# tj12323/GeoPurify

Hardware: AMD Instinct MI355X
Metric: scenes/sec (ScanNet-val shape) + pooled-feature GB/s vs HBM peak (higher is better)
Workload: dtype f32 (student convolutions and pooling: f16 hi/lo split operands, 3 MFMAs per product, fp32 accumulate)

## Files before the change

geopurify_amd/_lib.py:

```python
import ctypes
import os
from ctypes import POINTER, c_char_p, c_double, c_float, c_int32, c_int64, c_size_t, c_uint32, c_void_p

_HERE = os.path.dirname(os.path.abspath(__file__))
LIB_PATH = os.environ.get("GP_LIB") or os.path.join(_HERE, "libgeopurify_hip.so")

_P = c_void_p
GP_KNN_MAX_K = 127

SIGNATURES = {
    "gp_version": (c_int32, []),
    "gp_last_error": (c_char_p, []),
    "gp_debug_set": (c_int32, [c_int32, c_int32]),
    "gp_debug_ptr": (c_int32, [c_int32, _P, c_size_t]),
    "gp_voxelize_workspace_bytes": (c_size_t, [c_int64]),
    "gp_voxelize_f64": (c_int32, [_P, c_int64, POINTER(c_double), _P, _P, _P, _P, _P, _P, _P, c_size_t, _P]),
    "gp_fnv_hash_f64": (c_int32, [_P, c_int64, _P, _P]),
    "gp_project_points_f64": (c_int32, [_P, c_int64, POINTER(c_double), c_double, c_double, c_double,
                                        c_double, _P, c_int32, c_int32, c_int32, c_double, _P, _P, _P]),
    "gp_render_depth_f64": (c_int32, [_P, c_int64, POINTER(c_double), c_double, c_double, c_double, c_double,
                                      c_int32, c_int32, c_int32, _P, _P]),
    "gp_minmax_i32": (c_int32, [_P, c_int64, _P, _P]),
    "gp_morton_order_workspace_bytes": (c_size_t, [c_int64]),
    "gp_morton_order": (c_int32, [_P, c_int64, _P, _P, _P, c_size_t, _P]),
    "gp_grid_bytes": (c_size_t, [c_int64, POINTER(c_int32)]),
    "gp_grid_build": (c_int32, [_P, c_int64, POINTER(c_int32), POINTER(c_int32), _P, c_size_t, _P]),
    "gp_scatter_mean_csr": (c_int32, [_P, c_int64, c_int32, _P, _P, c_int64, _P, _P, c_int64, c_int32, _P]),
    "gp_gather_rows": (c_int32, [_P, c_int64, c_int32, _P, c_int64, _P, _P, c_int64, _P]),
    "gp_kernel_map_build": (c_int32, [_P, _P, c_int64, _P, _P]),
    "gp_coords_order_batched_workspace_bytes": (c_size_t, [c_int64]),
    "gp_coords_order_batched": (c_int32, [_P, c_int64, _P, _P, _P, _P, _P, c_size_t, _P]),
    "gp_kernel_map_sorted": (c_int32, [_P, c_int64, _P, _P]),
    "gp_quantize_batched_workspace_bytes": (c_size_t, [c_int64]),
    "gp_quantize_batched": (c_int32, [_P, c_int64, _P, _P, _P, _P, _P, _P, _P, c_size_t, _P]),
    "gp_segment_labels": (c_int32, [_P, c_int64, _P, _P, _P, c_int64, c_int64, c_int32, _P, _P]),
    "gp_sparse_conv": (c_int32, [_P, c_int64, _P, c_int64, _P, c_int32, c_int32, c_int32, _P, _P, _P,
                                 c_int64, c_int32, _P, c_int64, _P]),
    "gp_conv_pairs_workspace_bytes": (c_size_t, [c_int64, c_int32]),
    "gp_conv_pairs_build": (c_int32, [_P, c_int64, c_int32, c_int32, _P, _P, _P, _P, _P, _P, _P, c_size_t, _P]),
    "gp_conv_chunk_plan_workspace_bytes": (c_size_t, [c_int64, c_int32]),
    "gp_conv_chunk_plan": (c_int32, [_P, c_int64, c_int32, c_int32, c_int32, c_int32, c_int32, _P, _P, _P, c_size_t, _P]),
    "gp_conv_weights_split": (c_int32, [_P, c_int32, c_int32, c_int32, c_float, _P, _P, _P]),
    "gp_split_f16": (c_int32, [_P, c_int64, c_int32, c_int64, _P, _P, c_int64, _P]),
    "gp_sparse_conv_f16x3": (c_int32, [_P, c_int64, _P, _P, c_int64, _P, _P, _P, _P, _P, c_int32, c_int64, c_int64, c_int32, _P, _P,
                                       c_int32, c_int32, _P, _P, _P, _P, c_int64, c_int32, _P, c_int64, _P, _P,
                                       c_int64, c_int32, POINTER(c_int32), POINTER(c_int32), POINTER(c_int32), _P, _P,
                                       _P, _P, c_int64, _P, c_int32, c_int32, _P]),
    "gp_conv_weights_split_blocked": (c_int32, [_P, c_int32, c_int32, c_int32, c_float, _P, _P, c_int32, _P]),
    "gp_pow2_scale": (c_int32, [_P, c_int64, c_int32, c_int64, _P, _P, c_size_t, _P]),
    "gp_split_f16_scaled": (c_int32, [_P, c_int64, c_int32, c_int64, _P, _P, c_int64, _P, _P, _P, _P]),
    "gp_rcb_order": (c_int32, [_P, c_int64, c_int32, c_int32, _P, _P, _P]),
    "gp_rows_renumber_i32": (c_int32, [_P, c_int64, c_int32, _P, _P, _P, _P]),
    "gp_l2norm_rows": (c_int32, [_P, c_int64, c_int32, c_int64, _P]),
    "gp_embed_head_f16x3": (c_int32, [_P, _P, c_int64, _P, _P, _P, c_int64, c_int32, c_int32, c_float, c_int32, _P, c_int64, _P, _P, c_float, _P, _P]),
    "gp_knn_workspace_bytes": (c_size_t, [c_int64]),
    "gp_knn_lattice": (c_int32, [_P, _P, _P, c_int64, c_int32, _P, _P, c_size_t, _P]),
    "gp_knn_batched_workspace_bytes": (c_size_t, [c_int64]),
    "gp_knn_batched": (c_int32, [_P, _P, c_int64, c_int32, _P, _P, _P, c_size_t, _P]),
    "gp_affinity_softmax": (c_int32, [_P, c_int64, c_int32, _P, c_int32, c_int64, c_float, _P, _P]),
    "gp_affinity_softmax_scatter": (c_int32, [_P, c_int64, c_int32, _P, c_int32, c_int64, c_float, _P, _P, _P, _P, _P]),
    "gp_pool_ell": (c_int32, [_P, c_int64, _P, _P, c_int32, c_int64, c_int32, _P, c_int64, _P]),
    "gp_pool_transpose_workspace_bytes": (c_size_t, [c_int64, c_int32]),
    "gp_pool_transpose_build": (c_int32, [_P, c_int64, c_int32, _P, _P, _P, c_size_t, _P]),
    "gp_pool_ell_transpose": (c_int32, [_P, c_int64, _P, _P, _P, c_int32, c_int64, c_int32, _P, c_int64, _P]),
    "gp_pool_ell_wgrad": (c_int32, [_P, c_int64, _P, c_int64, _P, c_int32, c_int64, c_int32, _P, c_int32, _P]),
    "gp_affinity_softmax_backward_workspace_bytes": (c_size_t, [c_int64, c_int32]),
    "gp_affinity_softmax_backward": (c_int32, [_P, c_int64, c_int32, _P, _P, _P, c_int32, c_int64, c_float, _P, _P, _P, c_int64, _P,
                                               c_size_t, _P]),
    "gp_l2norm_rows_backward": (c_int32, [_P, c_int64, _P, c_int64, c_int32, c_int64, _P, c_int64, _P]),
    "gp_pool_tiles_workspace_bytes": (c_size_t, [c_int64, c_int32]),
    "gp_pool_tiles_count": (c_int32, [_P, c_int64, c_int32, c_int32, _P, _P, c_size_t, _P]),
    "gp_pool_tiles_fill": (c_int32, [_P, _P, c_int64, c_int32, c_int32, _P, _P, _P, _P]),
    "gp_pool_tiles_apply": (c_int32, [_P, c_int64, _P, _P, _P, c_int32, c_int64, c_int32, _P, c_int64, _P]),
    "gp_pool_mfma_workspace_bytes": (c_size_t, [c_int64, c_int32]),
    "gp_pool_mfma_count": (c_int32, [_P, c_int64, c_int32, c_int32, c_int32, _P, _P, _P, c_size_t, _P]),
    "gp_pool_mfma_fill": (c_int32, [_P, _P, c_int64, c_int32, c_int32, _P, _P, c_int64, _P, _P, _P, _P]),
    "gp_pool_mfma_apply": (c_int32, [_P, _P, c_int64, _P, _P, _P, _P, c_int64, c_int32, c_int32, _P, _P, c_int64, _P, c_int64, _P, _P]),
    "gp_pool_mfma_apply_persistent": (c_int32, [_P, _P, c_int64, _P, _P, _P, _P, c_int64, c_int32, c_int32, c_int32, _P, _P, c_int64,
                                                _P, c_int64, c_int64, _P, _P, _P]),
    "gp_pool_cs_workspace_bytes": (c_size_t, [c_int64, c_int32]),
    "gp_pool_cs_count": (c_int32, [_P, c_int64, c_int32, c_int32, _P, _P, _P, _P, c_size_t, _P]),
    "gp_pool_cs_fill": (c_int32, [_P, _P, c_int64, c_int32, c_int32, _P, c_int64, c_int32, _P, _P, _P, _P, _P]),
    "gp_pool_cs_structure": (c_int32, [_P, c_int64, c_int32, c_int32, _P, c_int64, c_int32, _P, _P, _P, _P, _P, _P]),
    "gp_pool_cs_structure_valid": (c_int32, [_P, c_int64, c_int32, c_int32, _P, c_int64, c_int32, _P, _P, _P, _P]),
    "gp_affinity_cs_fragments": (c_int32, [_P, _P, c_int64, c_int32, c_int32, c_float, _P, _P, _P, _P, c_int32, _P, _P, _P]),
    "gp_pool_cs_apply": (c_int32, [_P, _P, c_int64, _P, _P, _P, _P, _P, c_int64, c_int32, c_int32, _P, _P, c_int64, _P, c_int64, _P, _P]),
    "gp_pool_cs_deps": (c_int32, [_P, _P, c_int64, c_int32, _P, _P, _P]),
    "gp_pool_cs_chain_flag_words": (c_size_t, [c_int64, c_int32]),
    "gp_pool_cs_chain_flag_words_d": (c_size_t, [c_int64, c_int32, c_int32]),
    "gp_pool_cs_apply_chain": (c_int32, [_P, _P, _P, _P, c_int64, _P, _P, _P, _P, _P, c_int64, c_int32, c_int32, c_int32, _P, c_int64, _P, _P, _P,
                                         c_uint32, _P]),
    "gp_lift_dense_accum": (c_int32, [_P, c_int32, c_int32, c_int32, _P, _P, _P, c_int64, _P, c_int64, _P, _P]),
    "gp_lift_dense_bilinear_accum": (c_int32, [_P, c_int32, c_int32, c_int32, c_int32, c_int32, _P, _P, _P, c_int64, _P,
                                               c_int64, _P, _P]),
    "gp_lift_dense_finish": (c_int32, [_P, c_int64, c_int32, _P, c_int64, _P, _P]),
    "gp_lift_masks_workspace_bytes": (c_size_t, [c_int32, c_int32, c_int32]),
    "gp_lift_masks_view": (c_int32, [_P, c_int32, c_int32, c_int32, _P, _P, _P, _P, _P, c_int32, c_int32,
                                     _P, _P, c_int64, _P, _P, _P, c_size_t, _P]),
    "gp_pv_count": (c_int32, [_P, c_int64, _P, _P]),
    "gp_scan_workspace_bytes": (c_size_t, [c_int64]),
    "gp_exclusive_scan_i64": (c_int32, [_P, c_int64, _P, _P, c_size_t, _P]),
    "gp_pv_fill": (c_int32, [_P, _P, c_int64, c_int32, _P, _P, _P, _P, _P]),
    "gp_segment_tables": (c_int32, [_P, c_int32, c_int32, _P, c_int32, c_float, _P, _P, _P]),
    "gp_fuse_views_top3": (c_int32, [_P, _P, _P, c_int64, _P, _P, c_int32, c_int32, c_int32, _P, c_int64, _P, _P]),
    "gp_nn1_workspace_bytes": (c_size_t, [c_int64, c_int64]),
    "gp_nn1_f64": (c_int32, [_P, c_int64, _P, c_int64, _P, _P, c_size_t, _P]),
    "gp_nn1_masked_workspace_bytes": (c_size_t, [c_int64]),
    "gp_nn1_masked_f64": (c_int32, [_P, c_int64, _P, _P, _P, _P, c_size_t, _P]),
    "gp_visible_lists_workspace_bytes": (c_size_t, [c_int64]),
    "gp_visible_lists": (c_int32, [_P, c_int64, _P, _P, _P, _P, _P, c_size_t, _P]),
    "gp_views_visible_lists_workspace_bytes": (c_size_t, [c_int64, c_int32]),
    "gp_views_visible_lists": (c_int32, [_P, c_int64, _P, _P, c_int32, c_int32, c_int32, c_int32, c_double, c_int64, c_int64,
                                         _P, _P, _P, _P, _P, _P, _P, c_size_t, _P]),
    "gp_lift_masks_views_workspace_bytes": (c_size_t, [c_int32, c_int32, c_int32, c_int32, c_int64, c_int64, c_int64]),
    "gp_lift_masks_views": (c_int32, [_P, c_int32, c_int32, c_int32, c_int32, _P, _P, _P, _P, _P, c_int32, c_int32, _P, c_int64,
                                      _P, _P, _P, _P, _P, _P, c_int32, c_int64, c_int64, _P, _P, _P, _P, _P, c_size_t, _P]),
    "gp_classify_argmax": (c_int32, [_P, c_int64, c_int32, c_int64, _P, c_int32, c_float, _P, _P, _P]),
    "gp_gather_rows_classify": (c_int32, [_P, c_int64, c_int32, _P, c_int64, _P, _P, c_int64, _P, c_int32, c_float, _P, _P, _P]),
    "gp_rows_argmax": (c_int32, [_P, c_int64, c_int32, c_int64, _P, c_int64, c_int32, _P, _P, _P]),
    "gp_col_stats_workspace_bytes": (c_size_t, [c_int64, c_int32]),
    "gp_col_stats": (c_int32, [_P, c_int64, c_int64, c_int32, _P, _P, _P, c_size_t, _P]),
    "gp_bn_train_apply": (c_int32, [_P, c_int64, c_int64, c_int32, _P, _P, _P, _P, c_float, _P, c_int64, c_int32, _P, c_int64,
                                    _P, _P, c_int64, c_float, _P, _P, _P]),
    "gp_bn_train_backward_workspace_bytes": (c_size_t, [c_int64, c_int32]),
    "gp_bn_train_backward": (c_int32, [_P, c_int64, _P, c_int64, _P, c_int64, _P, _P, c_float, _P, _P, c_int64, c_int32, _P, c_int64,
                                       _P, c_int64, _P, _P, _P, _P, _P, c_int64, _P, c_size_t, _P]),
    "gp_col_sums_f64": (c_int32, [_P, c_int64, c_int64, c_int32, _P, _P, _P, c_size_t, _P]),
    "gp_bn_bwd_sums_f64": (c_int32, [_P, c_int64, _P, c_int64, _P, c_int64, _P, _P, c_float, _P, _P, c_int64, c_int32, _P, _P, c_size_t, _P]),
    "gp_bn_bwd_apply": (c_int32, [_P, c_int64, _P, c_int64, _P, c_int64, _P, _P, c_float, _P, _P, _P, c_int64, c_int64, c_int32, _P, c_int64,
                                  _P, c_int64, _P, _P]),
    "gp_infonce_workspace_bytes": (c_size_t, [c_int64, c_int32]),
    "gp_infonce_fwd_bwd": (c_int32, [_P, c_int64, c_int64, c_int32, _P, c_int64, _P, c_int64, c_int32, c_float, _P, _P, c_int64,
                                     _P, c_size_t, _P]),
    "gp_infonce_weighted_fwd_bwd": (c_int32, [_P, c_int64, c_int64, c_int32, _P, c_int64, _P, c_int64, c_int32, c_float, _P, _P, _P, _P, c_int64,
                                              _P, c_size_t, _P]),
    "gp_conv_wgrad_workspace_bytes": (c_size_t, [c_int64, c_int32, c_int32]),
    "gp_conv_wgrad_f16x3": (c_int32, [_P, _P, c_int64, _P, _P, c_int64, _P, _P, _P, c_int64, _P, c_int32, c_int32, c_int32, c_int32,
                                      _P, _P, _P, c_size_t, _P]),
    "gp_adamw_step": (c_int32, [_P, _P, _P, _P, c_int64, c_float, c_float, c_float, c_float, c_float, c_int64, _P]),
    "gp_knn_points_f32": (c_int32, [_P, c_int64, _P, c_int64, c_int32, _P, _P, _P]),
    "gp_sampler_select": (c_int32, [_P, c_int64, c_int64, c_int64, _P, c_int32, _P, _P, _P]),
    "gp_sim_segments_f16x3": (c_int32, [_P, _P, c_int64, c_int32, _P, _P, _P, _P, c_int64, c_int64, _P, _P]),
    "gp_sampler_select_segments": (c_int32, [_P, _P, _P, _P, c_int64, c_int64, _P, c_int32, _P, _P, _P]),
    "gp_sampler_micro_segments": (c_int32, [_P, _P, _P, _P, _P, c_int64, c_int32, _P, c_int64, c_int32, _P, _P]),
    "gp_normalize_split_f16": (c_int32, [_P, c_int64, c_int32, c_int64, c_int64, c_float, _P, _P, c_int64, _P]),
    "gp_iou_hist_i64": (c_int32, [_P, _P, c_int64, c_int32, POINTER(c_int64), c_int32, _P, _P]),
    "gp_nn1_batched_workspace_bytes": (c_size_t, [c_int64]),
    "gp_nn1_batched": (c_int32, [_P, _P, _P, _P, c_int64, c_int32, _P, _P, _P, c_size_t, _P]),
    "gp_iou_hist_batched_i64": (c_int32, [_P, _P, c_int64, _P, _P, c_int64, c_int32, c_int32, POINTER(c_int64), c_int32, _P, _P]),
    "gp_sparse_conv_tiles": (c_int32, [POINTER(c_int32)]),
    "gp_segment_loss_col_step": (c_int32, []),
    "gp_segment_loss_unit_rows": (c_int32, [_P, c_int64, c_int32, c_int64, _P, c_int64, c_int32, _P, _P]),
    "gp_segment_loss_items_workspace_bytes": (c_size_t, [c_int64, c_int64]),
    "gp_segment_loss_items": (c_int32, [_P, _P, c_int64, _P, _P, c_int64, c_int32, POINTER(c_int64), c_int32, c_int32, _P, _P, _P, _P, _P, _P,
                                        _P, c_size_t, _P]),
    "gp_segment_loss_rows": (c_int32, [_P, c_int64, c_int64, c_int32, c_int32, _P, _P, _P, _P, _P, _P, _P, c_int64, _P, _P, _P]),
    "gp_segment_loss_reduce_workspace_bytes": (c_size_t, [c_int64, c_int32]),
    "gp_segment_loss_reduce": (c_int32, [_P, _P, c_int64, _P, c_int32, c_int32, _P, _P, _P, c_size_t, _P]),
    "gp_fused_decode_workspace_bytes": (c_size_t, [c_int64, c_int64]),
    "gp_fused_decode": (c_int32, [_P, c_int64, _P, _P, c_int64, c_int64, _P, c_int64, c_int32, _P, _P, _P, _P, c_size_t, _P]),
    "gp_lift_batched_col_chunk": (c_int32, []),
    "gp_lift_batched_transpose": (c_int32, [_P, c_int32, c_int32, c_int64, _P, _P]),
    "gp_lift_batched_workspace_bytes": (c_size_t, [c_int64, c_int32]),
    "gp_lift_batched": (c_int32, [_P, c_int64, _P, c_int32, c_int32, c_int32, _P, _P, _P, _P, c_int32, c_int32, c_int32, c_int32, c_int32,
                                  c_double, c_int64, c_int64, c_int32, _P, c_int64, _P, _P, _P, _P, _P, _P, _P, c_size_t, _P]),
    "gp_lift_masks_batched_lists_workspace_bytes": (c_size_t, [c_int64, c_int32]),
    "gp_lift_masks_batched_lists": (c_int32, [_P, c_int64, _P, _P, _P, _P, c_int32, c_int32, c_int32, c_int32, c_double, c_int64, c_int64,
                                              c_int64, _P, _P, _P, _P, _P, _P, _P, _P, _P, c_size_t, _P]),
    "gp_lift_masks_batched_workspace_bytes": (c_size_t, [c_int64, c_int32, c_int32, c_int32, c_int32, c_int32, c_int32, c_int64, c_int32,
                                                         c_int64]),
    "gp_lift_masks_batched": (c_int32, [_P, c_int64, _P, c_int32, _P, c_int32, c_int32, c_int32, _P, _P, _P, _P, _P, c_int32, c_int32,
                                        _P, _P, _P, _P, _P, _P, c_int64, c_int32, c_int64, _P, _P, c_int32, c_int32, c_int32,
                                        _P, c_int64, _P, _P, _P, _P, _P, _P, c_size_t, _P]),
}

_lib = None


class GeoPurifyHipError(RuntimeError):
    pass


def load(path=None):
    global _lib
    if _lib is not None:
        return _lib
    import torch
    p = path or LIB_PATH
    if not os.path.exists(p):
        raise GeoPurifyHipError(
            f"{p} not found: build it with `python -c 'import __graft_entry__ as g; g.build()'` "
            "(or `make -C geopurify_amd/csrc`).  There is no CPU fallback.")
    lib = ctypes.CDLL(p)
    missing = []
    for name, (res, args) in SIGNATURES.items():
        try:
            fn = getattr(lib, name)
        except AttributeError:
            missing.append(name)
            continue
        fn.restype = res
        fn.argtypes = args
    if missing:
        raise GeoPurifyHipError(f"{p} does not export {missing}; rebuild the library")
    _lib = lib
    return lib


def check(rc, what):
    if rc != 0:
        msg = load().gp_last_error()
        raise GeoPurifyHipError(f"{what} failed (rc={rc}): {msg.decode() if msg else ''}")


def exported_symbols():
    return list(SIGNATURES.keys())
```

geopurify_amd/csrc/knn.hip:

```cpp
#include "gp_grid.h"

namespace {

constexpr int KNN_MAXSEL = 128;
constexpr int KNN_MAXTIE = 256;

template <int R>
struct KnnCfg {
    static constexpr int B = (8 * R + 1) * (8 * R + 1);
    static constexpr int HB = (B + 63) / 64 * 64;
};

template <int R, int WAVES>
__global__ void __launch_bounds__(WAVES * 64)
knn_ring_kernel(const void *grid, const int32_t *__restrict__ coords, const int32_t *__restrict__ ids, int64_t nv,
                int k, int32_t *__restrict__ nbr, const int32_t *__restrict__ qlist,
                const int32_t *__restrict__ qcount, int32_t *__restrict__ fail_list, int32_t *__restrict__ fail_count) {
    constexpr int B = KnnCfg<R>::B, HB = KnnCfg<R>::HB;
    __shared__ int s_hist[WAVES][HB];
    __shared__ unsigned long long s_selkey[WAVES][KNN_MAXSEL];
    __shared__ int s_selrow[WAVES][KNN_MAXSEL];
    __shared__ int s_tieid[WAVES][KNN_MAXTIE];
    __shared__ int s_tierow[WAVES][KNN_MAXTIE];
    __shared__ int s_cnt[WAVES][2];
    __shared__ int s_cstart[WAVES][(2 * R + 1) * (2 * R + 1) * (2 * R + 1)], s_coff[WAVES][(2 * R + 1) * (2 * R + 1) * (2 * R + 1) + 1];

    const int wv = threadIdx.x >> 6, lane = threadIdx.x & 63;
    int64_t widx = (int64_t)blockIdx.x * WAVES + wv;
    int64_t total = qlist ? (int64_t)*qcount : nv;
    if (widx >= total) return;
    const int qi = __builtin_amdgcn_readfirstlane(qlist ? qlist[widx] : (int)widx);
    GpGridView g(grid);
    const int qx = coords[(int64_t)qi * 3], qy = coords[(int64_t)qi * 3 + 1], qz = coords[(int64_t)qi * 3 + 2];
    const int cx0 = (qx - g.h->origin[0]) >> 3, cy0 = (qy - g.h->origin[1]) >> 3, cz0 = (qz - g.h->origin[2]) >> 3;
    int *hist = s_hist[wv];
    for (int b = lane; b < HB; b += 64) hist[b] = 0;
    if (lane < 2) s_cnt[wv][lane] = 0;
    constexpr int SIDE = 2 * R + 1, NC = SIDE * SIDE * SIDE;
    int *cstart = s_cstart[wv], *coff = s_coff[wv];
    int total_c = 0;
    for (int c0 = 0; c0 < NC; c0 += 64) {
        const int c = c0 + lane;
        int start = 0, cnt = 0;
        if (c < NC) {
            const int dx = c % SIDE - R, dy = (c / SIDE) % SIDE - R, dz = c / (SIDE * SIDE) - R;
            const int slot = g.cell_slot(cx0 + dx, cy0 + dy, cz0 + dz);
            if (slot >= 0) { start = g.recs[slot].start; cnt = g.recs[slot].count; }
        }
        int incl = cnt;
#pragma unroll
        for (int o = 1; o < 64; o <<= 1) {
            int t = __shfl_up(incl, o, 64);
            if (lane >= o) incl += t;
        }
        if (c < NC) { cstart[c] = start; coff[c] = total_c + incl - cnt; }
        total_c += __shfl(incl, 63, 64);
    }
    if (lane == 0) coff[NC] = total_c;
    gp_wave_sync();
    auto row_of = [&](int j) {
        int lo = 0, hi = NC - 1;
        while (lo < hi) {
            const int mid = (lo + hi + 1) >> 1;
            if (coff[mid] <= j) lo = mid; else hi = mid - 1;
        }
        return cstart[lo] + (j - coff[lo]);
    };

    for (int j0 = 0; j0 < total_c; j0 += 128) {
        const int ja = j0 + lane, jb = j0 + 64 + lane;
        const bool va = ja < total_c, vb = jb < total_c;
        const int64_t ra = va ? row_of(ja) : 0, rb = vb ? row_of(jb) : 0;
        const int ax = coords[ra * 3], ay = coords[ra * 3 + 1], az = coords[ra * 3 + 2];
        const int bx = coords[rb * 3], by = coords[rb * 3 + 1], bz = coords[rb * 3 + 2];
        const int da = (ax - qx) * (ax - qx) + (ay - qy) * (ay - qy) + (az - qz) * (az - qz);
        const int db = (bx - qx) * (bx - qx) + (by - qy) * (by - qy) + (bz - qz) * (bz - qz);
        if (va && da < B) atomicAdd(&hist[da], 1);
        if (vb && db < B) atomicAdd(&hist[db], 1);
    }
    gp_wave_sync();

    constexpr int CH = HB / 64;
    int loc = 0;
#pragma unroll
    for (int c = 0; c < CH; ++c) loc += hist[lane * CH + c];
    int incl = loc;
#pragma unroll
    for (int o = 1; o < 64; o <<= 1) {
        int t = __shfl_up(incl, o, 64);
        if (lane >= o) incl += t;
    }
    int tot = __shfl(incl, 63, 64);
    const int need = k + 1;
    bool fail = tot < need;
    int T = 0, c_lt = 0;
    if (!fail) {
        int excl = incl - loc;
        unsigned long long m = __ballot(incl >= need);
        int owner = __ffsll((long long)m) - 1;
        int myT = 0, mylt = 0;
        if (lane == owner) {
            int run = excl;
            for (int c = 0; c < CH; ++c) {
                int h = hist[lane * CH + c];
                if (run + h >= need) { myT = lane * CH + c; mylt = run; break; }
                run += h;
            }
        }
        T = __shfl(myT, owner, 64);
        c_lt = __shfl(mylt, owner, 64);
        if (hist[T] > KNN_MAXTIE) fail = true;
    }
    if (fail) {
        if (lane == 0) {
            int p = atomicAdd(fail_count, 1);
            fail_list[p] = qi;
        }
        return;
    }

    for (int j0 = 0; j0 < total_c; j0 += 64) {
        const int j = j0 + lane;
        if (j < total_c) {
            const int64_t r = row_of(j);
            int ex = coords[r * 3] - qx, ey = coords[r * 3 + 1] - qy, ez = coords[r * 3 + 2] - qz;
            int d2 = ex * ex + ey * ey + ez * ez;
            if (d2 < T) {
                int id = ids ? ids[r] : (int)r;
                int p = atomicAdd(&s_cnt[wv][0], 1);
                s_selkey[wv][p] = ((unsigned long long)(unsigned)d2 << 32) | (unsigned)id;
                s_selrow[wv][p] = (int)r;
            } else if (d2 == T) {
                int id = ids ? ids[r] : (int)r;
                int p = atomicAdd(&s_cnt[wv][1], 1);
                s_tieid[wv][p] = id;
                s_tierow[wv][p] = (int)r;
            }
        }
    }
    gp_wave_sync();
    const int m_tie = s_cnt[wv][1];
    const int take = need - c_lt;
    for (int t = lane; t < m_tie; t += 64) {
        int id = s_tieid[wv][t];
        int rank = 0;
        for (int u = 0; u < m_tie; ++u) rank += (s_tieid[wv][u] < id);
        if (rank < take) {
            s_selkey[wv][c_lt + rank] = ((unsigned long long)(unsigned)T << 32) | (unsigned)id;
            s_selrow[wv][c_lt + rank] = s_tierow[wv][t];
        }
    }
    gp_wave_sync();

    for (int t = lane; t < need; t += 64) {
        unsigned long long key = s_selkey[wv][t];
        int rank = 0;
        for (int u = 0; u < need; ++u) rank += (s_selkey[wv][u] < key);
        if (rank > 0) nbr[(int64_t)qi * k + rank - 1] = s_selrow[wv][t];
    }
}

__global__ void __launch_bounds__(256)
knn_exhaustive_kernel(const int32_t *__restrict__ coords, const int32_t *__restrict__ ids, int64_t nv, int k,
                      int32_t *__restrict__ nbr, const int32_t *__restrict__ qlist, const int32_t *__restrict__ qcount) {
    __shared__ int s_red[4];
    __shared__ unsigned long long s_selkey[KNN_MAXSEL];
    __shared__ int s_selrow[KNN_MAXSEL];
    __shared__ int s_n;
    const int total = *qcount;
    for (int w = blockIdx.x; w < total; w += gridDim.x) {
        const int qi = qlist[w];
        const int qx = coords[(int64_t)qi * 3], qy = coords[(int64_t)qi * 3 + 1], qz = coords[(int64_t)qi * 3 + 2];
        const int need = k + 1;
        auto keyof = [&](int64_t r) {
            long long ex = coords[r * 3] - qx, ey = coords[r * 3 + 1] - qy, ez = coords[r * 3 + 2] - qz;
            unsigned long long d2 = (unsigned long long)(ex * ex + ey * ey + ez * ez);
            unsigned id = (unsigned)(ids ? ids[r] : (int)r);
            return (d2 << 32) | id;
        };
        unsigned long long lo = 0, hi = ~0ull;
        while (lo < hi) {
            unsigned long long mid = lo + ((hi - lo) >> 1);
            int c = 0;
            for (int64_t r = threadIdx.x; r < nv; r += 256) c += (keyof(r) <= mid);
            c = gp_wave_sum_i(c);
            __syncthreads();
            if ((threadIdx.x & 63) == 0) s_red[threadIdx.x >> 6] = c;
            __syncthreads();
            int tot = s_red[0] + s_red[1] + s_red[2] + s_red[3];
            if (tot >= need) hi = mid; else lo = mid + 1;
        }
        if (threadIdx.x == 0) s_n = 0;
        __syncthreads();
        for (int64_t r = threadIdx.x; r < nv; r += 256) {
            unsigned long long key = keyof(r);
            if (key <= lo) {
                int p = atomicAdd(&s_n, 1);
                if (p < KNN_MAXSEL) { s_selkey[p] = key; s_selrow[p] = (int)r; }
            }
        }
        __syncthreads();
        for (int t = threadIdx.x; t < need; t += 256) {
            unsigned long long key = s_selkey[t];
            int rank = 0;
            for (int u = 0; u < need; ++u) rank += (s_selkey[u] < key);
            if (rank > 0) nbr[(int64_t)qi * k + rank - 1] = s_selrow[t];
        }
        __syncthreads();
    }
}

__global__ void zero2_kernel(int32_t *a, int32_t *b) {
    if (threadIdx.x == 0) { *a = 0; *b = 0; }
}

}

extern "C" size_t gp_knn_workspace_bytes(int64_t nv) {
    GpCarver cv(nullptr, 0);
    cv.take<int32_t>(64);
    cv.take<int32_t>(nv);
    cv.take<int32_t>(nv);
    return cv.off;
}

extern "C" int gp_knn_lattice(const void *grid, const int32_t *coords, const int32_t *ids, int64_t nv, int32_t k,
                              int32_t *nbr, void *workspace, size_t workspace_bytes, void *stream_) {
    GP_CHECK_ARG(grid && coords && nbr && workspace, "gp_knn_lattice: null argument");
    GP_CHECK_ARG(k >= 1 && k <= GP_KNN_MAX_K, "gp_knn_lattice: k=%d not in 1..%d", k, GP_KNN_MAX_K);
    GP_CHECK_ARG(nv > k, "gp_knn_lattice: need more than k voxels (nv=%lld, k=%d)", (long long)nv, k);
    GpCarver cv(workspace, workspace_bytes);
    int32_t *counts = cv.take<int32_t>(64);
    int32_t *list_a = cv.take<int32_t>(nv);
    int32_t *list_b = cv.take<int32_t>(nv);
    if (!cv.ok()) { gp_set_error("gp_knn_lattice: workspace too small (%zu < %zu)", workspace_bytes, cv.off); return GP_ENOMEM; }
    hipStream_t s = gp_stream(stream_);
    zero2_kernel<<<1, 64, 0, s>>>(counts, counts + 1);
    constexpr int W1 = 4, W3 = 2;
    knn_ring_kernel<1, W1><<<(int)((nv + W1 - 1) / W1), W1 * 64, 0, s>>>(grid, coords, ids, nv, k, nbr, nullptr, nullptr,
                                                                      list_a, counts);
    knn_ring_kernel<3, W3><<<(int)((nv + W3 - 1) / W3), W3 * 64, 0, s>>>(grid, coords, ids, nv, k, nbr, list_a, counts,
                                                                      list_b, counts + 1);
    knn_exhaustive_kernel<<<1024, 256, 0, s>>>(coords, ids, nv, k, nbr, list_b, counts + 1);
    GP_CHECK_LAUNCH();
    return GP_OK;
}
```

geopurify_amd/csrc/lift.hip:

```cpp
#include <cstring>
#include <rocprim/device/device_scan.hpp>

#include "gp_common.h"
#include "gp_project.h"

namespace {

__global__ void lift_dense_accum_kernel(const float *__restrict__ feat2d, int d, int H, int W,
                                        const int64_t *__restrict__ pt, const int64_t *__restrict__ x,
                                        const int64_t *__restrict__ y, int64_t n_v, float *__restrict__ sum,
                                        int64_t ld_sum, float *__restrict__ cnt) {
    int64_t i = (blockIdx.x * (int64_t)blockDim.x + threadIdx.x) >> 6;
    if (i >= n_v) return;
    int lane = gp_lane();
    int64_t p = pt[i];
    int64_t pix = x[i] * W + y[i];
    int64_t plane = (int64_t)H * W;
    for (int c = lane; c < d; c += 64) sum[p * ld_sum + c] += feat2d[c * plane + pix];
    if (lane == 0) cnt[p] += 1.0f;
}

__global__ void lift_dense_bilinear_accum_kernel(const float *__restrict__ feat, int d, int h, int w, float scale_h,
                                                 float scale_w, const int64_t *__restrict__ pt,
                                                 const int64_t *__restrict__ x, const int64_t *__restrict__ y, int64_t n_v,
// ... 25 lines not shown
    if (c == 0.f) c = 1e-6f;
    for (int k = lane; k < d; k += 64) sum[p * ld_sum + k] = sum[p * ld_sum + k] / c;
    if (lane == 0) seen[p] = c > 1e-5f ? 1 : 0;
}

__global__ void transpose_kernel(const float *__restrict__ src, int rows, int cols, float *__restrict__ dst) {
    __shared__ float tile[64][65];
    int bx = blockIdx.x * 64, by = blockIdx.y * 64;
    int tx = threadIdx.x & 63, ty = threadIdx.x >> 6;
    for (int r = ty; r < 64; r += 4) {
        int row = by + r, col = bx + tx;
        tile[r][tx] = (row < rows && col < cols) ? src[(int64_t)row * cols + col] : 0.f;
    }
    __syncthreads();
    for (int r = ty; r < 64; r += 4) {
        int orow = bx + r, ocol = by + tx;
        if (orow < cols && ocol < rows) dst[(int64_t)orow * rows + ocol] = tile[tx][r];
    }
}

__device__ __forceinline__ void lift_masks_point(const float *__restrict__ mt , int Q, int h, int w,
                                                 const float *__restrict__ scores, const int32_t *__restrict__ tx0,
                                                 const float *__restrict__ twx, const int32_t *__restrict__ ty0,
                                                 const float *__restrict__ twy, int out_h, int out_w, int row, int col, int lane,
                                                 int &seg_out, float &logit_out) {
    bool inb = (unsigned)row < (unsigned)out_h && (unsigned)col < (unsigned)out_w;
    float best = -1.f, best_logit = 0.f;
    int best_q = -1;
    if (inb) {
        int x0 = tx0[col], y0 = ty0[row];
        float wx[4], wy[4];
#pragma unroll
        for (int t = 0; t < 4; ++t) { wx[t] = twx[col * 4 + t]; wy[t] = twy[row * 4 + t]; }
        for (int q = lane; q < Q; q += 64) {
            float sc = scores[q];
            float hr[4];
#pragma unroll
            for (int j = 0; j < 4; ++j) {
                int yy = min(y0 + j, h - 1);
                const float *r = mt + ((int64_t)yy * w) * Q + q;
                float t = __fmul_rn(r[(int64_t)min(x0, w - 1) * Q], wx[0]);
#pragma unroll
                for (int a = 1; a < 4; ++a) t = fmaf(r[(int64_t)min(x0 + a, w - 1) * Q], wx[a], t);
                hr[j] = t;
            }
            float v = __fmul_rn(hr[0], wy[0]);
#pragma unroll
            for (int j = 1; j < 4; ++j) v = fmaf(hr[j], wy[j], v);
            if (sc > 0.f) {
                float sg = 1.f / (1.f + expf(-v));
                float pr = __fmul_rn(sc, sg);
                if (pr > best) { best = pr; best_q = q; best_logit = v; }
            }
        }
    }
#pragma unroll
    for (int o = 32; o > 0; o >>= 1) {
        float ob = __shfl_xor(best, o, 64);
        int oq = __shfl_xor(best_q, o, 64);
        float ol = __shfl_xor(best_logit, o, 64);
        bool take = (oq >= 0) && (best_q < 0 || ob > best || (ob == best && oq < best_q));
        if (take) { best = ob; best_q = oq; best_logit = ol; }
    }
    float sg = 1.f / (1.f + expf(-best_logit));
    seg_out = (best_q >= 0 && sg >= 0.5f) ? best_q : -1;
    logit_out = best_logit;
}
__global__ void lift_masks_kernel(const float *__restrict__ mt , int Q, int h, int w,
                                  const float *__restrict__ scores, const int32_t *__restrict__ tx0,
                                  const float *__restrict__ twx, const int32_t *__restrict__ ty0,
                                  const float *__restrict__ twy, int out_h, int out_w,
                                  const int64_t *__restrict__ px, const int64_t *__restrict__ py, int64_t n_v,
                                  int32_t *__restrict__ seg, float *__restrict__ seg_logit) {
    int64_t i = (blockIdx.x * (int64_t)blockDim.x + threadIdx.x) >> 6;
    if (i >= n_v) return;
    int lane = gp_lane();
    int sg;
    float lg;
    lift_masks_point(mt, Q, h, w, scores, tx0, twx, ty0, twy, out_h, out_w, (int)px[i], (int)py[i], lane, sg, lg);
    if (lane == 0) {
        seg[i] = sg;
        if (seg_logit) seg_logit[i] = lg;
    }
}

}

#include "gp_lift_masks.h"

namespace {

__global__ void pv_mask_kernel(const int64_t *__restrict__ ent_pt, const int32_t *__restrict__ ent_view, const uint8_t *__restrict__ keep,
                               int64_t total, unsigned long long *__restrict__ vmask) {
    int64_t e = blockIdx.x * (int64_t)blockDim.x + threadIdx.x;
    if (e >= total) return;
    const int v = ent_view[e];
    if (keep[v]) atomicOr(&vmask[ent_pt[e] * 2 + (v >> 6)], 1ull << (v & 63));
}
__global__ void pv_cnt_kernel(const unsigned long long *__restrict__ vmask, int64_t n, int64_t *__restrict__ cnt ) {
    int64_t p = blockIdx.x * (int64_t)blockDim.x + threadIdx.x;
    if (p < n) cnt[p] = __popcll(vmask[2 * p]) + __popcll(vmask[2 * p + 1]);
    else if (p == n) cnt[p] = 0;
}
__global__ void pv_fill_views_kernel(const int64_t *__restrict__ ent_pt, const int32_t *__restrict__ ent_view,
                                     const uint8_t *__restrict__ keep, const int32_t *__restrict__ seg, int64_t total,
                                     const unsigned long long *__restrict__ vmask, const int64_t *__restrict__ start,
                                     int32_t *__restrict__ pv_view, int32_t *__restrict__ pv_seg) {
    int64_t e = blockIdx.x * (int64_t)blockDim.x + threadIdx.x;
    if (e >= total) return;
    const int v = ent_view[e];
    if (!keep[v]) return;
    const int64_t p = ent_pt[e];
    const unsigned long long m0 = vmask[2 * p], m1 = vmask[2 * p + 1];
    const int rank = v < 64 ? __popcll(m0 & ((1ull << v) - 1ull)) : __popcll(m0) + __popcll(m1 & ((1ull << (v - 64)) - 1ull));
    const int64_t s_ = start[p] + rank;
    pv_view[s_] = v;
    pv_seg[s_] = seg[e];
}

__global__ void segment_tables_kernel(const float *__restrict__ emb, int Q, int d, const float *__restrict__ text,
                                      int C, float scale, float *__restrict__ fseg, float *__restrict__ lseg) {
    int q = (blockIdx.x * blockDim.x + threadIdx.x) >> 6;
    if (q >= Q) return;
    int lane = gp_lane();
    float ss = 0.f;
    for (int c = lane; c < d; c += 64) { float v = emb[(int64_t)q * d + c]; ss += v * v; }
    ss = gp_wave_sum(ss);
    float nrm = fmaxf(sqrtf(ss), 1e-12f);
    for (int c = lane; c < d; c += 64) fseg[(int64_t)q * d + c] = emb[(int64_t)q * d + c] / nrm;
    for (int k = 0; k < C; ++k) {
        float dot = 0.f;
        for (int c = lane; c < d; c += 64) dot += (emb[(int64_t)q * d + c] / nrm) * text[(int64_t)k * d + c];
        dot = gp_wave_sum(dot);
        if (lane == 0) lseg[(int64_t)q * C + k] = scale * dot;
    }
}

__global__ void pv_count_kernel(const int64_t *__restrict__ pt, int64_t n_v, int64_t *__restrict__ cnt) {
    int64_t i = blockIdx.x * (int64_t)blockDim.x + threadIdx.x;
    if (i < n_v) cnt[pt[i]] += 1;
}
__global__ void pv_fill_kernel(const int64_t *__restrict__ pt, const int32_t *__restrict__ seg, int64_t n_v, int view,
                               const int64_t *__restrict__ start, int32_t *__restrict__ cursor,
                               int32_t *__restrict__ pv_view, int32_t *__restrict__ pv_seg) {
    int64_t i = blockIdx.x * (int64_t)blockDim.x + threadIdx.x;
    if (i >= n_v) return;
    int64_t p = pt[i];
    int64_t s = start[p] + cursor[p];
    cursor[p] += 1;
    pv_view[s] = view;
    pv_seg[s] = seg[i];
}

__global__ void fuse_top3_kernel(const int64_t *__restrict__ start, const int32_t *__restrict__ pv_view,
                                 const int32_t *__restrict__ pv_seg, int64_t n, const float *__restrict__ fseg,
                                 const float *__restrict__ lseg, int Q, int d, int C, float *__restrict__ out,
                                 int64_t ld_out, uint8_t *__restrict__ seen) {
    int64_t p = (blockIdx.x * (int64_t)blockDim.x + threadIdx.x) >> 6;
    if (p >= n) return;
    int lane = gp_lane();
    int64_t b = start[p], e = start[p + 1];
    int M = (int)(e - b);
    if (lane == 0 && seen) seen[p] = M > 0 ? 1 : 0;
    if (M == 0) {
        for (int c = lane * 4; c < d; c += 256) *reinterpret_cast<float4 *>(out + p * ld_out + c) = make_float4(0, 0, 0, 0);
        return;
    }
    const bool in_regs = M <= 64;
    int my_sg = -1, my_v = 0;
    if (in_regs && lane < M) { my_sg = pv_seg[b + lane]; my_v = pv_view[b + lane]; }
    float bestv = -INFINITY;
    int bestc = 0x7fffffff;
    for (int c0 = 0; c0 < C; c0 += 64) {
        const int c = c0 + lane;
        float sum = 0.f;
        if (in_regs) {
            for (int j0 = 0; j0 < M; j0 += 4) {
                float t[4];
#pragma unroll
                for (int u = 0; u < 4; ++u) {
                    const int j = j0 + u;
                    const int sg = __shfl(my_sg, j < M ? j : 0, 64), vw = __shfl(my_v, j < M ? j : 0, 64);
                    t[u] = (j < M && sg >= 0 && c < C) ? lseg[((int64_t)vw * Q + sg) * C + c] : 0.f;
                }
#pragma unroll
                for (int u = 0; u < 4; ++u)
                    if (j0 + u < M) sum += t[u];
            }
        } else if (c < C) {
            for (int64_t j = b; j < e; ++j) { int sg = pv_seg[j]; sum += sg >= 0 ? lseg[((int64_t)pv_view[j] * Q + sg) * C + c] : 0.f; }
        }
        if (c < C) {
            sum = sum / (float)M;
            if (sum > bestv) { bestv = sum; bestc = c; }
        }
    }
#pragma unroll
    for (int o = 32; o > 0; o >>= 1) {
        float ov = __shfl_xor(bestv, o, 64);
        int oc = __shfl_xor(bestc, o, 64);
        if (ov > bestv || (ov == bestv && oc < bestc)) { bestv = ov; bestc = oc; }
    }
    float s0 = -INFINITY, s1 = -INFINITY, s2 = -INFINITY;
    int64_t j0 = -1, j1 = -1, j2 = -1;
    if (in_regs) {
        const float my_s = (lane < M && my_sg >= 0) ? lseg[((int64_t)my_v * Q + my_sg) * C + bestc] : 0.f;
        for (int jj = 0; jj < M; ++jj) {
            const float sc = __shfl(my_s, jj, 64);
            const int64_t j = b + jj;
            if (sc > s0) { s2 = s1; j2 = j1; s1 = s0; j1 = j0; s0 = sc; j0 = j; }
            else if (sc > s1) { s2 = s1; j2 = j1; s1 = sc; j1 = j; }
            else if (sc > s2) { s2 = sc; j2 = j; }
        }
    } else {
        for (int64_t j = b; j < e; ++j) {
            int sg = pv_seg[j];
            float sc = sg >= 0 ? lseg[((int64_t)pv_view[j] * Q + sg) * C + bestc] : 0.f;
            if (sc > s0) { s2 = s1; j2 = j1; s1 = s0; j1 = j0; s0 = sc; j0 = j; }
            else if (sc > s1) { s2 = s1; j2 = j1; s1 = sc; j1 = j; }
            else if (sc > s2) { s2 = sc; j2 = j; }
        }
    }
    float e0 = 1.f, e1 = (j1 >= 0) ? expf(s1 - s0) : 0.f, e2 = (j2 >= 0) ? expf(s2 - s0) : 0.f;
    float den = e0 + e1 + e2;
    float w0 = e0 / den, w1 = e1 / den, w2 = e2 / den;
    if (pv_seg[j0] < 0) w0 = 0.f;
    if (j1 >= 0 && pv_seg[j1] < 0) { w1 = 0.f; }
    if (j2 >= 0 && pv_seg[j2] < 0) { w2 = 0.f; }
    auto frow = [&](int64_t j) { int sg = pv_seg[j] < 0 ? 0 : pv_seg[j]; return fseg + ((int64_t)pv_view[j] * Q + sg) * d; };
    const float *f0 = frow(j0);
    const float *f1 = j1 >= 0 ? frow(j1) : f0;
    const float *f2 = j2 >= 0 ? frow(j2) : f0;
    for (int c = lane * 4; c < d; c += 256) {
        float4 a = *reinterpret_cast<const float4 *>(f0 + c);
        float4 r = make_float4(a.x * w0, a.y * w0, a.z * w0, a.w * w0);
        if (j1 >= 0) {
            float4 t = *reinterpret_cast<const float4 *>(f1 + c);
            r.x += t.x * w1; r.y += t.y * w1; r.z += t.z * w1; r.w += t.w * w1;
        }
        if (j2 >= 0) {
            float4 t = *reinterpret_cast<const float4 *>(f2 + c);
            r.x += t.x * w2; r.y += t.y * w2; r.z += t.z * w2; r.w += t.w * w2;
        }
        *reinterpret_cast<float4 *>(out + p * ld_out + c) = r;
    }
}

}

extern "C" int gp_lift_dense_accum(const float *feat2d, int32_t d, int32_t height, int32_t width, const int64_t *pt,
                                   const int64_t *x, const int64_t *y, int64_t n_v, float *sum, int64_t ld_sum,
                                   float *cnt, void *stream_) {
    GP_CHECK_ARG(feat2d && pt && x && y && sum && cnt, "gp_lift_dense_accum: null argument");
    if (n_v == 0) return GP_OK;
    lift_dense_accum_kernel<<<(int)((n_v * 64 + 255) / 256), 256, 0, gp_stream(stream_)>>>(feat2d, d, height, width, pt,
                                                                                            x, y, n_v, sum, ld_sum, cnt);
    GP_CHECK_LAUNCH();
    return GP_OK;
}

extern "C" int gp_lift_dense_bilinear_accum(const float *feat, int32_t d, int32_t h, int32_t w, int32_t out_h, int32_t out_w,
                                            const int64_t *pt, const int64_t *x, const int64_t *y, int64_t n_v, float *sum,
                                            int64_t ld_sum, float *cnt, void *stream_) {
    GP_CHECK_ARG(feat && pt && x && y && sum && cnt, "gp_lift_dense_bilinear_accum: null argument");
    GP_CHECK_ARG(d > 0 && h > 0 && w > 0 && out_h > 0 && out_w > 0, "gp_lift_dense_bilinear_accum: bad shape");
    if (n_v == 0) return GP_OK;
    const float sh = out_h > 1 ? (float)(h - 1) / (float)(out_h - 1) : 0.f;
    const float sw = out_w > 1 ? (float)(w - 1) / (float)(out_w - 1) : 0.f;
    lift_dense_bilinear_accum_kernel<<<(int)((n_v * 64 + 255) / 256), 256, 0, gp_stream(stream_)>>>(feat, d, h, w, sh, sw, pt, x, y,
                                                                                                     n_v, sum, ld_sum, cnt);
    GP_CHECK_LAUNCH();
    return GP_OK;
}

extern "C" int gp_lift_dense_finish(float *sum, int64_t ld_sum, int32_t d, const float *cnt, int64_t n, uint8_t *seen,
                                    void *stream_) {
    GP_CHECK_ARG(sum && cnt && seen && n > 0, "gp_lift_dense_finish: null/empty argument");
    lift_dense_finish_kernel<<<(int)((n * 64 + 255) / 256), 256, 0, gp_stream(stream_)>>>(sum, ld_sum, d, cnt, n, seen);
    GP_CHECK_LAUNCH();
    return GP_OK;
}

extern "C" size_t gp_lift_masks_workspace_bytes(int32_t q, int32_t h, int32_t w) {
    return gp_align_up((size_t)q * h * w * sizeof(float), 256);
}

extern "C" int gp_lift_masks_view(const float *pred_masks, int32_t q, int32_t h, int32_t w, const float *scores,
                                  const int32_t *tap_x0, const float *tap_wx, const int32_t *tap_y0,
                                  const float *tap_wy, int32_t out_h, int32_t out_w, const int64_t *x,
                                  const int64_t *y, int64_t n_v, int32_t *seg, float *seg_logit, void *workspace,
                                  size_t workspace_bytes, void *stream_) {
    GP_CHECK_ARG(pred_masks && scores && tap_x0 && tap_wx && tap_y0 && tap_wy && x && y && seg && workspace,
                 "gp_lift_masks_view: null argument");
    GP_CHECK_ARG(q > 0 && h > 0 && w > 0, "gp_lift_masks_view: bad mask shape");
    if (workspace_bytes < gp_lift_masks_workspace_bytes(q, h, w)) { gp_set_error("gp_lift_masks_view: workspace too small"); return GP_ENOMEM; }
    if (n_v == 0) return GP_OK;
    hipStream_t s = gp_stream(stream_);
    float *mt = static_cast<float *>(workspace);
    int hw = h * w;
    dim3 tg((hw + 63) / 64, (q + 63) / 64);
    transpose_kernel<<<tg, 256, 0, s>>>(pred_masks, q, hw, mt);
    lift_masks_kernel<<<(int)((n_v * 64 + 255) / 256), 256, 0, s>>>(mt, q, h, w, scores, tap_x0, tap_wx, tap_y0, tap_wy,
                                                                    out_h, out_w, x, y, n_v, seg, seg_logit);
    GP_CHECK_LAUNCH();
    return GP_OK;
}

static size_t lv_scan32_tmp(int64_t n) {
    size_t t = 0;
    (void)rocprim::exclusive_scan(nullptr, t, (int32_t *)nullptr, (int32_t *)nullptr, (int32_t)0, (size_t)n, rocprim::plus<int32_t>(), 0);
    return t;
}
static size_t lv_scan64_tmp(int64_t n) {
    size_t t = 0;
    (void)rocprim::exclusive_scan(nullptr, t, (int64_t *)nullptr, (int64_t *)nullptr, (int64_t)0, (size_t)n, rocprim::plus<int64_t>(), 0);
    return t;
}
struct LvWork {
    float *mt; int32_t *cov, *rs, *rent, *qent; float *rxyz; double *part_d; int32_t *part_i; unsigned long long *vmask; int4 *tab;
    int64_t *cnt; char *tmp; size_t tmp_bytes;
    int32_t *order; float *sscore;
};
static size_t lv_carve(void *ws, size_t bytes, int32_t nsrc, int32_t q, int32_t h, int32_t w, int64_t total, int64_t n, int64_t fill_cap,
                       LvWork &k) {
    GpCarver cv(ws, bytes);
    k.mt = cv.take<float>((size_t)nsrc * q * h * w);
    k.order = cv.take<int32_t>((size_t)nsrc * q);
    k.sscore = cv.take<float>((size_t)nsrc * q);
    k.cov = cv.take<int32_t>(total + 1);
    k.rs = cv.take<int32_t>(total + 1);
    k.rent = cv.take<int32_t>(total);
    k.qent = cv.take<int32_t>(total);
    k.rxyz = cv.take<float>(total * 3);
    k.part_d = cv.take<double>((size_t)FV_CHUNKS * fill_cap);
    k.part_i = cv.take<int32_t>((size_t)FV_CHUNKS * fill_cap);
    k.vmask = cv.take<unsigned long long>(n * 2);
    k.cnt = cv.take<int64_t>(n + 1);
    k.tab = cv.take<int4>(130);
    size_t a = lv_scan32_tmp(total + 1), b = lv_scan64_tmp(n + 1);
    k.tmp_bytes = a > b ? a : b;
    k.tmp = cv.take<char>(k.tmp_bytes);
    return cv.off;
}
extern "C" size_t gp_lift_masks_views_workspace_bytes(int32_t nsrc, int32_t q, int32_t h, int32_t w, int64_t total, int64_t n,
                                                      int64_t fill_cap) {
    if (nsrc <= 0 || q <= 0 || h <= 0 || w <= 0 || total <= 0 || n <= 0 || fill_cap < 0 || fill_cap > total) return 0;
    LvWork k;
    return lv_carve(nullptr, 0, nsrc, q, h, w, total, n, fill_cap ? fill_cap : total, k);
}
extern "C" int gp_lift_masks_views(const float *pred_masks, int32_t nsrc, int32_t q, int32_t h, int32_t w, const float *scores,
                                   const int32_t *tap_x0, const float *tap_wx, const int32_t *tap_y0, const float *tap_wy,
                                   int32_t out_h, int32_t out_w, const float *xyz, int64_t n, const int64_t *ent_pt,
                                   const int64_t *ent_x, const int64_t *ent_y, const int32_t *ent_view, const int64_t *view_off,
                                   const uint8_t *keep, int32_t nviews, int64_t total, int64_t fill_cap, int32_t *seg,
                                   int64_t *pv_start, int32_t *pv_view, int32_t *pv_seg, void *workspace, size_t workspace_bytes,
                                   void *stream_) {
    GP_CHECK_ARG(pred_masks && scores && tap_x0 && tap_wx && tap_y0 && tap_wy && xyz && ent_pt && ent_x && ent_y && ent_view && view_off &&
                     keep && seg && pv_start && pv_view && pv_seg && workspace,
                 "gp_lift_masks_views: null argument");
    GP_CHECK_ARG(q > 0 && h > 0 && w > 0 && n > 0 && total > 0, "gp_lift_masks_views: empty shape");
    GP_CHECK_ARG(q <= 1024, "gp_lift_masks_views: %d queries (the score sort holds 1024)", q);
    GP_CHECK_ARG(nviews > 0 && nviews <= 128 && nviews <= nsrc, "gp_lift_masks_views: %d views (1..128, <= %d mask sets)", nviews, nsrc);
    GP_CHECK_ARG(total < (int64_t)INT32_MAX, "gp_lift_masks_views: too many entries");
    GP_CHECK_ARG(fill_cap >= 0 && fill_cap <= total, "gp_lift_masks_views: fill_cap=%lld outside 0..total", (long long)fill_cap);
    if (fill_cap == 0) fill_cap = total;
    LvWork k;
    if (lv_carve(workspace, workspace_bytes, nsrc, q, h, w, total, n, fill_cap, k) > workspace_bytes) {
        gp_set_error("gp_lift_masks_views: workspace too small");
        return GP_ENOMEM;
    }
    hipStream_t s = gp_stream(stream_);
    const int hw = h * w;
    lv_sort_scores_kernel<<<nviews, 256, 0, s>>>(scores, q, k.order, k.sscore);
    transpose_views_kernel<<<dim3((hw + 63) / 64, (q + 63) / 64, nviews), 256, 0, s>>>(pred_masks, q, hw, k.mt, k.order);
    lift_masks_views_kernel<<<(unsigned)((total * 64 + 255) / 256), 256, 0, s>>>(k.mt, q, h, w, k.sscore, k.order, tap_x0, tap_wx, tap_y0,
                                                                               tap_wy, out_h, out_w, ent_x, ent_y, ent_view, keep, total, seg);
    const unsigned eb = (unsigned)((total + 1 + 255) / 256);
    fill_flags_kernel<<<eb, 256, 0, s>>>(seg, total, k.cov);
    size_t tb = k.tmp_bytes;
    GP_CHECK_HIP(rocprim::exclusive_scan(k.tmp, tb, k.cov, k.rs, (int32_t)0, (size_t)(total + 1), rocprim::plus<int32_t>(), s));
    fill_compact_kernel<<<eb, 256, 0, s>>>(xyz, ent_pt, seg, k.rs, total, k.rxyz, k.rent, k.qent);
    const unsigned qb = (unsigned)(total / 256 + nviews + 1);
    fill_table_kernel<<<1, 64, 0, s>>>(view_off, k.rs, nviews, k.tab);
    fill_part_kernel<<<dim3(qb, FV_CHUNKS), 256, 0, s>>>(xyz, ent_pt, k.tab, nviews, k.rxyz, k.qent, k.part_d, k.part_i, fill_cap,
                                                         k.rent, seg);
    fill_reduce_kernel<<<qb, 256, 0, s>>>(k.tab, nviews, k.part_d, k.part_i, fill_cap, k.rent, k.qent, seg);
    GP_CHECK_HIP(hipMemsetAsync(k.vmask, 0, (size_t)n * 2 * sizeof(unsigned long long), s));
    pv_mask_kernel<<<eb, 256, 0, s>>>(ent_pt, ent_view, keep, total, k.vmask);
    pv_cnt_kernel<<<(unsigned)((n + 1 + 255) / 256), 256, 0, s>>>(k.vmask, n, k.cnt);
    tb = k.tmp_bytes;
    GP_CHECK_HIP(rocprim::exclusive_scan(k.tmp, tb, k.cnt, pv_start, (int64_t)0, (size_t)(n + 1), rocprim::plus<int64_t>(), s));
    pv_fill_views_kernel<<<eb, 256, 0, s>>>(ent_pt, ent_view, keep, seg, total, k.vmask, pv_start, pv_view, pv_seg);
    GP_CHECK_LAUNCH();
    return GP_OK;
}

extern "C" int gp_segment_tables(const float *mask_embed, int32_t q, int32_t d, const float *text_norm, int32_t c,
                                 float logit_scale, float *f_seg, float *logit_seg, void *stream_) {
    GP_CHECK_ARG(mask_embed && text_norm && f_seg && logit_seg && q > 0 && d > 0 && c > 0, "gp_segment_tables: null/empty argument");
    segment_tables_kernel<<<(q * 64 + 255) / 256, 256, 0, gp_stream(stream_)>>>(mask_embed, q, d, text_norm, c, logit_scale,
                                                                              f_seg, logit_seg);
    GP_CHECK_LAUNCH();
    return GP_OK;
}

extern "C" int gp_pv_count(const int64_t *pt, int64_t n_v, int64_t *cnt, void *stream_) {
    GP_CHECK_ARG(pt && cnt, "gp_pv_count: null argument");
    if (n_v == 0) return GP_OK;
    pv_count_kernel<<<(int)((n_v + 255) / 256), 256, 0, gp_stream(stream_)>>>(pt, n_v, cnt);
    GP_CHECK_LAUNCH();
    return GP_OK;
}

extern "C" size_t gp_scan_workspace_bytes(int64_t n) {
    size_t t = 0;
    (void)rocprim::exclusive_scan(nullptr, t, (int64_t *)nullptr, (int64_t *)nullptr, (int64_t)0, (size_t)n, rocprim::plus<int64_t>(), 0);
    return gp_align_up(t, 256);
}

extern "C" int gp_exclusive_scan_i64(const int64_t *in, int64_t n, int64_t *out, void *workspace, size_t workspace_bytes,
                                     void *stream_) {
    GP_CHECK_ARG(in && out && n > 0, "gp_exclusive_scan_i64: null/empty argument");
    size_t t = workspace_bytes;
    GP_CHECK_HIP(rocprim::exclusive_scan(workspace, t, in, out, (int64_t)0, (size_t)n, rocprim::plus<int64_t>(), gp_stream(stream_)));
    return GP_OK;
}

extern "C" int gp_pv_fill(const int64_t *pt, const int32_t *seg, int64_t n_v, int32_t view, const int64_t *pv_start,
                          int32_t *cursor, int32_t *pv_view, int32_t *pv_seg, void *stream_) {
    GP_CHECK_ARG(pt && seg && pv_start && cursor && pv_view && pv_seg, "gp_pv_fill: null argument");
    if (n_v == 0) return GP_OK;
    pv_fill_kernel<<<(int)((n_v + 255) / 256), 256, 0, gp_stream(stream_)>>>(pt, seg, n_v, view, pv_start, cursor, pv_view, pv_seg);
    GP_CHECK_LAUNCH();
    return GP_OK;
}

extern "C" int gp_fuse_views_top3(const int64_t *pv_start, const int32_t *pv_view, const int32_t *pv_seg, int64_t n,
                                  const float *f_seg, const float *logit_seg, int32_t q, int32_t d, int32_t c,
                                  float *out, int64_t ld_out, uint8_t *seen, void *stream_) {
    GP_CHECK_ARG(pv_start && pv_view && pv_seg && f_seg && logit_seg && out && n > 0, "gp_fuse_views_top3: null/empty argument");
    GP_CHECK_ARG(d % 4 == 0 && ld_out % 4 == 0, "gp_fuse_views_top3: d and ld_out must be multiples of 4");
    fuse_top3_kernel<<<(int)((n * 64 + 255) / 256), 256, 0, gp_stream(stream_)>>>(pv_start, pv_view, pv_seg, n, f_seg,
                                                                                logit_seg, q, d, c, out, ld_out, seen);
    GP_CHECK_LAUNCH();
    return GP_OK;
}
```

geopurify_amd/ops.py:

```python
import ctypes

import numpy as np
import torch

from . import _lib
from ._lib import check


def _ptr(t):
    return ctypes.c_void_p(t.data_ptr()) if t is not None else None


def _stream():
    return ctypes.c_void_p(torch.cuda.current_stream().cuda_stream)


def _ws(nbytes, device):
    return torch.empty(max(int(nbytes), 256), dtype=torch.uint8, device=device)


def _chk(t, dtype, name):
    if t.dtype != dtype or not t.is_cuda or not t.is_contiguous():
        raise ValueError(f"{name}: expected contiguous CUDA {dtype}, got {t.dtype} cuda={t.is_cuda} contig={t.is_contiguous()}")
    return t
# ... 68 lines not shown


def minmax_i32(coords):
    lib = _lib.load()
    _chk(coords, torch.int32, "coords")
    mm = torch.empty(6, dtype=torch.int32, device=coords.device)
    check(lib.gp_minmax_i32(_ptr(coords), coords.shape[0], _ptr(mm), _stream()), "gp_minmax_i32")
    return mm


def morton_order(coords_i32):
    lib = _lib.load()
    _chk(coords_i32, torch.int32, "coords")
    nv = coords_i32.shape[0]
    dev = coords_i32.device
    ws = _ws(lib.gp_morton_order_workspace_bytes(nv), dev)
    perm = torch.empty(nv, dtype=torch.int32, device=dev)
    rank = torch.empty(nv, dtype=torch.int32, device=dev)
    check(lib.gp_morton_order(_ptr(coords_i32), nv, _ptr(perm), _ptr(rank), _ptr(ws), ws.numel(), _stream()),
          "gp_morton_order")
    return perm, rank


class Grid:

    def __init__(self, buf, origin, extent, nv):
        self.buf, self.origin, self.extent, self.nv = buf, origin, extent, nv

    def status(self):
        return int(self.buf[36:40].view(torch.int32).item())


def grid_build(coords_sorted, origin=None, extent=None):
    lib = _lib.load()
    _chk(coords_sorted, torch.int32, "coords")
    nv = coords_sorted.shape[0]
    if origin is None or extent is None:
        lo = coords_sorted.amin(0)
        hi = coords_sorted.amax(0)
        lohi = torch.stack([lo, hi]).cpu().tolist()
        origin = lohi[0]
        extent = [lohi[1][a] - lohi[0][a] + 1 for a in range(3)]
    o = (ctypes.c_int32 * 3)(*[int(v) for v in origin])
    e = (ctypes.c_int32 * 3)(*[int(v) for v in extent])
    nbytes = lib.gp_grid_bytes(nv, e)
    if nbytes == 0:
        raise _lib.GeoPurifyHipError("gp_grid_bytes: invalid extent")
    buf = _ws(nbytes, coords_sorted.device)
    check(lib.gp_grid_build(_ptr(coords_sorted), nv, o, e, _ptr(buf), buf.numel(), _stream()), "gp_grid_build")
    return Grid(buf, list(origin), list(extent), nv)


def kernel_map_build(grid, coords_sorted):
    lib = _lib.load()
    nv = coords_sorted.shape[0]
    nm = torch.empty((27, nv), dtype=torch.int32, device=coords_sorted.device)
    check(lib.gp_kernel_map_build(_ptr(grid.buf), _ptr(coords_sorted), nv, _ptr(nm), _stream()), "gp_kernel_map_build")
    return nm


def coords_order_batched(coords_b):
    lib = _lib.load()
    _chk(coords_b, torch.int32, "coords")
    if coords_b.dim() != 2 or coords_b.shape[1] != 4:
        raise ValueError(f"coords_order_batched: expected [nv, 4], got {list(coords_b.shape)}")
    nv = coords_b.shape[0]
    dev = coords_b.device
    ws = _ws(lib.gp_coords_order_batched_workspace_bytes(nv), dev)
    perm = torch.empty(nv, dtype=torch.int32, device=dev)
    rank = torch.empty(nv, dtype=torch.int32, device=dev)
    keys = torch.empty(nv, dtype=torch.int64, device=dev)
    status = torch.empty(3, dtype=torch.int32, device=dev)
    check(lib.gp_coords_order_batched(_ptr(coords_b), nv, _ptr(perm), _ptr(rank), _ptr(keys), _ptr(status), _ptr(ws), ws.numel(),
                                      _stream()), "gp_coords_order_batched")
    return perm, rank, keys, status


def kernel_map_sorted(keys_sorted):
    lib = _lib.load()
    _chk(keys_sorted, torch.int64, "keys")
    nv = keys_sorted.shape[0]
    nm = torch.empty((27, nv), dtype=torch.int32, device=keys_sorted.device)
    check(lib.gp_kernel_map_sorted(_ptr(keys_sorted), nv, _ptr(nm), _stream()), "gp_kernel_map_sorted")
    return nm


class QuantizedIndex:

    def __init__(self, n, nv, coordinates, unique_index, inverse, order, seg_start, bad_batch, bad_axes):
        self.n, self.nv, self.coordinates, self.unique_index, self.inverse = n, nv, coordinates, unique_index, inverse
        self.order, self.seg_start, self.bad_batch, self.bad_axes = order, seg_start, bad_batch, bad_axes
        self.counts = seg_start[1:] - seg_start[:-1]


QUANTIZE_OUTPUTS = {"vox_coords": (torch.int32, lambda n: (n, 4)), "unique_index": (torch.int64, lambda n: (n,)),
                    "inverse": (torch.int64, lambda n: (n,)), "order": (torch.int64, lambda n: (n,)),
                    "seg_start": (torch.int64, lambda n: (n + 1,)), "status": (torch.int32, lambda n: (3,))}


def quantize_batched(coords_b, buffers=None):
    lib = _lib.load()
    _chk(coords_b, torch.int32, "coords")
    if coords_b.dim() != 2 or coords_b.shape[1] != 4:
        raise ValueError(f"quantize_batched: expected [n, 4], got {list(coords_b.shape)}")
    n = coords_b.shape[0]
    if not 0 < n < 2 ** 31:
        raise ValueError(f"quantize_batched: n={n} out of range (1 .. 2^31 - 1)")
    dev = coords_b.device
    b = {}
    for name, (dtype, shape) in QUANTIZE_OUTPUTS.items():
        t = (buffers or {}).get(name)
        if t is None:
            t = torch.empty(shape(n), dtype=dtype, device=dev)
        elif _chk(t, dtype, name).shape != shape(n) or t.device != dev:
            raise ValueError(f"quantize_batched: buffer {name} must be {list(shape(n))} on {dev}, got {list(t.shape)} on {t.device}")
        b[name] = t
    ws = _ws(lib.gp_quantize_batched_workspace_bytes(n), dev)
    check(lib.gp_quantize_batched(_ptr(coords_b), n, _ptr(b["vox_coords"]), _ptr(b["unique_index"]), _ptr(b["inverse"]),
                                  _ptr(b["order"]), _ptr(b["seg_start"]), _ptr(b["status"]), _ptr(ws), ws.numel(), _stream()),
          "gp_quantize_batched")
    nv, bad_batch, bad_axes = readback(b["status"])
    return QuantizedIndex(n, nv, b["vox_coords"][:nv], b["unique_index"][:nv], b["inverse"], b["order"], b["seg_start"][:nv + 1],
                     bad_batch, bad_axes)


SEGMENT_LABEL_RULES = {"first": 0, "differ": 1, "count": 2}


def segment_labels(labels, q, ignore_label, rule, out=None):
    lib = _lib.load()
    if rule not in SEGMENT_LABEL_RULES:
        raise ValueError(f"segment_labels: rule={rule!r}, expected one of {sorted(SEGMENT_LABEL_RULES)}")
    _chk(labels, torch.int64, "labels")
    if labels.dim() != 1 or labels.shape[0] != q.n:
        raise ValueError(f"segment_labels: expected labels [{q.n}], got {list(labels.shape)}")
    if labels.device != q.order.device:
        raise ValueError(f"segment_labels: labels on {labels.device}, the quantisation on {q.order.device}")
    if out is None:
        out = torch.empty(q.nv, dtype=torch.int64, device=labels.device)
    elif _chk(out, torch.int64, "out").shape != (q.nv,) or out.device != labels.device:
        raise ValueError(f"segment_labels: expected out [{q.nv}], got {list(out.shape)}")
    check(lib.gp_segment_labels(_ptr(labels), q.n, _ptr(q.order), _ptr(q.seg_start), _ptr(q.unique_index), q.nv, int(ignore_label),
                                SEGMENT_LABEL_RULES[rule], _ptr(out), _stream()), "gp_segment_labels")
    return out


def scatter_mean_csr(src, d, order, seg_start, nv, out, col0=0, row_map=None):
    lib = _lib.load()
    _chk(src, torch.float32, "src")
    check(lib.gp_scatter_mean_csr(_ptr(src), src.stride(0), int(d), _ptr(order), _ptr(seg_start), int(nv),
                                  _ptr(row_map), _ptr(out), out.stride(0), int(col0), _stream()),
          "gp_scatter_mean_csr")
    return out


def gather_rows(src, d, index, out=None, row_map=None):
    lib = _lib.load()
    n = index.shape[0]
    if out is None:
        out = torch.empty((n, d), dtype=torch.float32, device=src.device)
    check(lib.gp_gather_rows(_ptr(src), src.stride(0), int(d), _ptr(index), n, _ptr(row_map), _ptr(out),
                             out.stride(0), _stream()), "gp_gather_rows")
    return out


def gather_rows_classify(src, d, index, text_norm, logit_scale, row_map=None):
    lib = _lib.load()
    n = index.shape[0]
    out = torch.empty((n, d), dtype=torch.float32, device=src.device)
    pred = torch.empty(n, dtype=torch.int64, device=src.device)
    zero = torch.empty(n, dtype=torch.uint8, device=src.device)
    check(lib.gp_gather_rows_classify(_ptr(src), src.stride(0), int(d), _ptr(index), n, _ptr(row_map), _ptr(out), out.stride(0),
                                      _ptr(text_norm), int(text_norm.shape[0]), float(logit_scale), _ptr(pred), _ptr(zero), _stream()),
          "gp_gather_rows_classify")
    return out, pred, zero


def can_gather_rows_classify(d, num_classes):
    return d % 64 == 0 and d <= 1024 and num_classes * d * 4 <= 64 * 1024


def pool_cs_width_ok(d):
    return d % 256 == 0 and 256 <= d <= 1024


def sparse_conv(x, nbr_map, w, scale=None, shift=None, residual=None, relu=False, out=None):
    lib = _lib.load()
    nv = x.shape[0]
    if w.dim() == 3:
        kv, cin, cout = w.shape
    else:
        kv, (cin, cout) = 1, w.shape
    _chk(w, torch.float32, "w")
    if out is None:
        out = torch.empty((nv, cout), dtype=torch.float32, device=x.device)
    check(lib.gp_sparse_conv(_ptr(x), x.stride(0), _ptr(nbr_map) if kv > 1 else None, nv, _ptr(w), int(kv),
                             int(cin), int(cout), _ptr(scale), _ptr(shift), _ptr(residual),
                             residual.stride(0) if residual is not None else 0, int(bool(relu)), _ptr(out),
                             out.stride(0), _stream()), "gp_sparse_conv")
    return out


class ConvPairs:

    def __init__(self, pair_in, pair_pos, seg_off, tile_start, nseg, num_pairs, nv):
        self.pair_in, self.pair_pos, self.pair_off, self.tile_start = pair_in, pair_pos, seg_off, tile_start
        self.nseg, self.num_pairs, self.nv = nseg, num_pairs, nv
        self.partial = None
        self.num_chunks, self.chunk_row_off, self.chunk_tile_off, self.chunk_pair_off = 0, None, None, None

    def _set_chunks(self, rows, tiles, pairs):
        n = len(rows) - 1
        self.num_chunks = n
        self.chunk_row_off = (ctypes.c_int32 * (n + 1))(*rows)
        self.chunk_tile_off = (ctypes.c_int32 * (n + 1))(*tiles)
        self.chunk_pair_off = (ctypes.c_int32 * (n + 1))(*pairs)
        self.max_chunk_pairs = max(pairs[i + 1] - pairs[i] for i in range(n))

    def regroup(self, g):
        g = max(1, min(int(g), max(self.num_chunks, 1)))
        cp = ConvPairs(self.pair_in, self.pair_pos, self.pair_off, self.tile_start, self.nseg, self.num_pairs, self.nv)
        cp.tile_desc = self.tile_desc
        n = self.num_chunks
        idx = list(range(0, n, g)) + [n]
        ro, po, to = list(self.chunk_row_off), list(self.chunk_pair_off), list(self.chunk_tile_off)
        cp._set_chunks([ro[i] for i in idx], [to[i] for i in idx], [po[i] for i in idx])
        return cp


CONV_TARGET_TILES = None


def conv_pairs_build(nbr_map, chunk_rows="balanced", col_tiles=2):
    lib = _lib.load()
    kv, nv = nbr_map.shape
    dev = nbr_map.device
    if isinstance(chunk_rows, str):
        if chunk_rows != "balanced":
            raise ValueError(f"conv_pairs_build: chunk_rows={chunk_rows!r}")
    if isinstance(chunk_rows, str):
        granule = 256
        max_chunks = (nv + granule - 1) // granule
        plan = torch.empty(max_chunks + 2, dtype=torch.int32, device=dev)
        ws = _ws(lib.gp_conv_chunk_plan_workspace_bytes(nv, granule), dev)
        target = CONV_TARGET_TILES or 3 * torch.cuda.get_device_properties(dev).multi_processor_count - 16
        check(lib.gp_conv_chunk_plan(_ptr(nbr_map), nv, kv, granule, int(col_tiles), int(target), max_chunks, _ptr(plan),
                                     _ptr(plan[max_chunks + 1:]), _ptr(ws), ws.numel(), _stream()), "gp_conv_chunk_plan")
        host = readback(plan)
        nchunks = host[max_chunks + 1]
        rows = host[:nchunks + 1]
        row_off = plan[:nchunks + 1]
    else:
        ch = nv if chunk_rows is None else max(int(chunk_rows), 256)
        rows = list(range(0, nv, ch)) + [nv]
        nchunks = len(rows) - 1
        row_off = torch.tensor(rows, dtype=torch.int32, device=dev)
    nseg = nchunks * kv
    ws = _ws(lib.gp_conv_pairs_workspace_bytes(nv, kv), dev)
    pair_in = torch.empty(kv * nv, dtype=torch.int32, device=dev)
    pair_pos = torch.empty((kv, nv), dtype=torch.int32, device=dev)
    seg_off = torch.empty(nseg + 1, dtype=torch.int32, device=dev)
    tile_start = torch.empty(nseg + 1, dtype=torch.int32, device=dev)
    tile_desc = torch.empty(((kv * nv) // 256 + nseg + 1, 4), dtype=torch.int32, device=dev)
    check(lib.gp_conv_pairs_build(_ptr(nbr_map), nv, kv, nchunks, _ptr(row_off), _ptr(pair_in), _ptr(pair_pos), _ptr(seg_off),
                                  _ptr(tile_start), _ptr(tile_desc), _ptr(ws), ws.numel(), _stream()), "gp_conv_pairs_build")
    bounds = readback(torch.stack([seg_off[::kv], tile_start[::kv]]))
    num_pairs = bounds[0][-1]
    cp = ConvPairs(pair_in, pair_pos, seg_off, tile_start, nseg, num_pairs, nv)
    cp.tile_desc = tile_desc
    cp._set_chunks(rows, bounds[1], bounds[0])
    return cp


def conv_weights_split(w, scale_pow2, blocked=None, transpose_flip=False):
    lib = _lib.load()
    kv, cin, cout = w.shape
    if transpose_flip:
        if cout % 32 == 0 and cin % 256 == 0 and blocked is not False:
            hi = torch.empty((kv, cin // 256, cout // 32, 256, 32), dtype=torch.float16, device=w.device)
            lo = torch.empty_like(hi)
            check(lib.gp_conv_weights_split_blocked(_ptr(w), kv, cout, cin, float(scale_pow2), _ptr(hi), _ptr(lo), 1, _stream()),
                  "gp_conv_weights_split_blocked")
            return hi, lo
        return conv_weights_split(w.flip(0).transpose(1, 2).contiguous(), scale_pow2, blocked)
    if blocked is None:
        blocked = cin % 32 == 0 and cout % 256 == 0
    if blocked:
        hi = torch.empty((kv, cout // 256, cin // 32, 256, 32), dtype=torch.float16, device=w.device)
        lo = torch.empty_like(hi)
        check(lib.gp_conv_weights_split_blocked(_ptr(w), kv, cin, cout, float(scale_pow2), _ptr(hi), _ptr(lo), 0, _stream()),
              "gp_conv_weights_split_blocked")
        return hi, lo
    hi = torch.empty((kv, cout, cin), dtype=torch.float16, device=w.device)
    lo = torch.empty((kv, cout, cin), dtype=torch.float16, device=w.device)
    check(lib.gp_conv_weights_split(_ptr(w), kv, cin, cout, float(scale_pow2), _ptr(hi), _ptr(lo), _stream()),
          "gp_conv_weights_split")
    return hi, lo


def conv_weights_shape(w_hi):
    if w_hi.dim() == 5:
        return int(w_hi.shape[0]), int(w_hi.shape[1]) * 256, int(w_hi.shape[2]) * 32
    return tuple(int(v) for v in w_hi.shape)


def split_f16(x, d=None, scale=None, per_row=False, interleaved=False, dst_row=None, extra_zero_rows=0):
    lib = _lib.load()
    d = x.shape[1] if d is None else d
    if interleaved:
        assert per_row and d % 32 == 0, "interleaved rows are the row-scaled operand of the convolution"
        rows = torch.empty((x.shape[0], 2 * d), dtype=torch.float16, device=x.device)
        rinv = torch.empty(x.shape[0], dtype=torch.float32, device=x.device)
        check(lib.gp_split_f16_scaled(_ptr(x), x.stride(0), int(d), x.shape[0], _ptr(rows), None, rows.stride(0), None, _ptr(rinv),
                                      _ptr(dst_row), _stream()), "gp_split_f16_scaled")
        return rows, None, rinv
    hi = torch.empty((x.shape[0] + extra_zero_rows, d), dtype=torch.float16, device=x.device)
    lo = torch.empty((x.shape[0] + extra_zero_rows, d), dtype=torch.float16, device=x.device)
    if extra_zero_rows:
        hi[x.shape[0]:].zero_()
        lo[x.shape[0]:].zero_()
    if scale is None and not per_row:
        if dst_row is not None:
            raise ValueError("split_f16: dst_row needs a scaled form (scale= or per_row=True)")
        check(lib.gp_split_f16(_ptr(x), x.stride(0), int(d), x.shape[0], _ptr(hi), _ptr(lo), hi.stride(0), _stream()),
              "gp_split_f16")
        return hi, lo
    rinv = torch.empty(x.shape[0], dtype=torch.float32, device=x.device) if per_row else None
    check(lib.gp_split_f16_scaled(_ptr(x), x.stride(0), int(d), x.shape[0], _ptr(hi), _ptr(lo), hi.stride(0), _ptr(scale),
                                  _ptr(rinv), _ptr(dst_row), _stream()), "gp_split_f16_scaled")
    return (hi, lo, rinv) if per_row else (hi, lo)


def rcb_order(coords_sorted, chunk_rows=1024, leaf_rows=128):
    lib = _lib.load()
    _chk(coords_sorted, torch.int32, "coords")
    nv = coords_sorted.shape[0]
    sigma = torch.empty(nv, dtype=torch.int32, device=coords_sorted.device)
    rho = torch.empty(nv, dtype=torch.int32, device=coords_sorted.device)
    check(lib.gp_rcb_order(_ptr(coords_sorted), nv, int(chunk_rows), int(leaf_rows), _ptr(sigma), _ptr(rho), _stream()), "gp_rcb_order")
    return sigma, rho


def rows_renumber(nbr, sigma, rho):
    lib = _lib.load()
    nv, k = nbr.shape
    out = torch.empty_like(nbr)
    check(lib.gp_rows_renumber_i32(_ptr(nbr), nv, int(k), _ptr(sigma), _ptr(rho), _ptr(out), _stream()), "gp_rows_renumber_i32")
    return out


def pow2_scale(x, d=None):
    lib = _lib.load()
    d = x.shape[1] if d is None else d
    out = torch.empty(2, dtype=torch.float32, device=x.device)
    ws = _ws(256, x.device)
    check(lib.gp_pow2_scale(_ptr(x), x.stride(0), int(d), x.shape[0], _ptr(out), _ptr(ws), ws.numel(), _stream()), "gp_pow2_scale")
    return out


def sparse_conv_f16x3(x, pairs, w_hi, w_lo, scale=None, shift=None, residual=None, relu=False, out=None,
                      x_split=None, out_split=None, x_row_inv=None, out_row_inv=None, want_f32=True, fp32_partials=False, dense_single_offset=False,
                      reference_walk=False):
    lib = _lib.load()
    res_planes = residual if isinstance(residual, (tuple, list)) else None
    if res_planes is not None:
        residual = None
    rh, rl, ri = (tuple(res_planes) + (None,))[:3] if res_planes is not None else (None, None, None)
    kv, cout, cin = conv_weights_shape(w_hi)
    w_blocked = int(w_hi.dim() == 5)
    nv = pairs.nv
    dev = w_hi.device
    if dense_single_offset:
        partial = torch.empty(64, dtype=torch.float32, device=dev)
    else:
        if pairs.partial is None or pairs.partial.shape[1] < cout or pairs.partial.shape[0] < max(pairs.max_chunk_pairs, 1):
            pairs.partial = torch.empty((max(pairs.max_chunk_pairs, 1), cout), dtype=torch.float32, device=dev)
        partial = pairs.partial
    if out is None and (want_f32 or out_split is None):
        out = torch.empty((nv, cout), dtype=torch.float32, device=dev)
    xh, xl = x_split if x_split is not None else (None, None)
    yh, yl = out_split if out_split is not None else (None, None)
    plane_flags = (1 if (xh is not None and xl is None) else 0) | (2 if (yh is not None and yl is None) else 0) | \
                  (4 if (rh is not None and rl is None) else 0) | (8 if fp32_partials else 0) | (16 if dense_single_offset else 0) | (32 if reference_walk else 0)
    check(lib.gp_sparse_conv_f16x3(_ptr(x), x.stride(0) if x is not None else 0, _ptr(xh), _ptr(xl),
                                   xh.stride(0) if xh is not None else 0, _ptr(pairs.pair_in), _ptr(pairs.pair_pos),
                                   _ptr(pairs.pair_off), _ptr(pairs.tile_start), _ptr(pairs.tile_desc), pairs.nseg, pairs.num_pairs, nv, kv, _ptr(w_hi), _ptr(w_lo), cin, cout,
                                   _ptr(partial), _ptr(scale), _ptr(shift), _ptr(residual),
                                   residual.stride(0) if residual is not None else 0, int(bool(relu)), _ptr(out),
                                   out.stride(0) if out is not None else 0, _ptr(yh), _ptr(yl), yh.stride(0) if yh is not None else 0,
                                   int(pairs.num_chunks), pairs.chunk_row_off, pairs.chunk_tile_off, pairs.chunk_pair_off,
                                   _ptr(x_row_inv), _ptr(out_row_inv), _ptr(rh), _ptr(rl), rh.stride(0) if rh is not None else 0, _ptr(ri),
                                   w_blocked, plane_flags, _stream()),
          "gp_sparse_conv_f16x3")
    return out


def interleave_planes(hi, lo):
    n, c = hi.shape
    return torch.stack([hi.reshape(n, c // 32, 32), lo.reshape(n, c // 32, 32)], dim=2).reshape(n, 2 * c).contiguous()


def deinterleave_planes(t):
    n, c2 = t.shape
    v = t.reshape(n, c2 // 64, 2, 32)
    return v[:, :, 0].reshape(n, c2 // 2).contiguous(), v[:, :, 1].reshape(n, c2 // 2).contiguous()


def l2norm_rows_(x, d=None):
    lib = _lib.load()
    d = x.shape[1] if d is None else d
    check(lib.gp_l2norm_rows(_ptr(x), x.stride(0), int(d), x.shape[0], _stream()), "gp_l2norm_rows")
    return x


def embed_head_f16x3(x_split, w_hi, w_lo, out_scale, x_row_inv=None, normalize=True, out=None, planes=False, want_f32=True, plane_rows=None):
    lib = _lib.load()
    hi, lo = x_split
    cout, cin = w_hi.shape[-2:]
    nv = hi.shape[0]
    _chk(hi, torch.float16, "x_hi"), _chk(lo, torch.float16, "x_lo")
    if hi.stride(0) != lo.stride(0) or hi.shape[1] < cin:
        raise ValueError("embed_head_f16x3: the hi / lo planes must share a row stride and hold cin channels")
    if out is None and (want_f32 or not planes):
        out = torch.empty((nv, cout), dtype=torch.float32, device=hi.device)
    eh = el = None
    if planes:
        eh = torch.empty((nv, cout), dtype=torch.float16, device=hi.device)
        el = torch.empty((nv, cout), dtype=torch.float16, device=hi.device)
    check(lib.gp_embed_head_f16x3(_ptr(hi), _ptr(lo), hi.stride(0), _ptr(x_row_inv), _ptr(w_hi), _ptr(w_lo), nv, int(cin), int(cout),
                                  float(out_scale), int(bool(normalize)), _ptr(out), out.stride(0) if out is not None else 0, _ptr(eh), _ptr(el),
                                  AFFINITY_PLANE_SCALE, _ptr(plane_rows) if planes else None, _stream()), "gp_embed_head_f16x3")
    return (out, (eh, el)) if planes else out


def knn_lattice(grid, coords_sorted, ids, k):
    lib = _lib.load()
    nv = coords_sorted.shape[0]
    dev = coords_sorted.device
    ws = _ws(lib.gp_knn_workspace_bytes(nv), dev)
    nbr = torch.empty((nv, k), dtype=torch.int32, device=dev)
    check(lib.gp_knn_lattice(_ptr(grid.buf), _ptr(coords_sorted), _ptr(ids), nv, int(k), _ptr(nbr), _ptr(ws),
                             ws.numel(), _stream()), "gp_knn_lattice")
    return nbr


def knn_batched(keys_sorted, ids, k, nbr=None, status=None, workspace=None):
    lib = _lib.load()
    _chk(keys_sorted, torch.int64, "keys")
    _chk(ids, torch.int32, "ids")
    nv, k = keys_sorted.shape[0], int(k)
    if keys_sorted.dim() != 1 or ids.shape != (nv,):
        raise ValueError(f"knn_batched: expected keys [nv] and ids [nv], got {list(keys_sorted.shape)} and {list(ids.shape)}")
    dev = keys_sorted.device
    if nbr is None:
        nbr = torch.empty((nv, max(k, 0)), dtype=torch.int32, device=dev)
    elif _chk(nbr, torch.int32, "nbr").shape != (nv, k):
        raise ValueError(f"knn_batched: expected nbr [{nv}, {k}], got {list(nbr.shape)}")
    if status is None:
        status = torch.empty(4, dtype=torch.int32, device=dev)
    elif _chk(status, torch.int32, "status").shape != (4,):
        raise ValueError(f"knn_batched: expected status [4], got {list(status.shape)}")
    ws = _ws(lib.gp_knn_batched_workspace_bytes(nv), dev) if workspace is None else _chk(workspace, torch.uint8, "workspace")
    check(lib.gp_knn_batched(_ptr(keys_sorted), _ptr(ids), nv, k, _ptr(nbr), _ptr(status), _ptr(ws), ws.numel(), _stream()),
          "gp_knn_batched")
    return nbr, status


def affinity_softmax(e, nbr, sharpen=20.0, d=None, into=None):
    lib = _lib.load()
    nv, k = nbr.shape
    d = e.shape[1] if d is None else d
    w = torch.empty((nv, k), dtype=torch.float32, device=e.device)
    if into is not None:
        if into.dst is None or into.nv != nv or tuple(into.dst.shape) != (nv, k):
            raise ValueError("affinity_softmax: `into` needs a PoolCs structure built from these neighbour lists")
        check(lib.gp_affinity_softmax_scatter(_ptr(e), e.stride(0), int(d), _ptr(nbr), int(k), nv, float(sharpen), _ptr(w),
                                              _ptr(into.dst), _ptr(into.wa_hi), _ptr(into.wa_lo), _stream()),
              "gp_affinity_softmax_scatter")
        into.filled = True
        return w
    check(lib.gp_affinity_softmax(_ptr(e), e.stride(0), int(d), _ptr(nbr), int(k), nv, float(sharpen), _ptr(w),
                                  _stream()), "gp_affinity_softmax")
    return w


_E_SCALE = {}
AFFINITY_PLANE_SCALE = 1024.0


def affinity_cs_fragments(e, sharpen, op, planes=None):
    lib = _lib.load()
    if op.valid is None:
        raise ValueError("affinity_cs_fragments: the operator needs pool_cs_plan(structure='valid')")
    if planes is not None:
        eh, el = planes
    else:
        key = str(e.device)
        if key not in _E_SCALE:
            _E_SCALE[key] = torch.tensor([AFFINITY_PLANE_SCALE], dtype=torch.float32, device=e.device)
        eh, el = split_f16(e, 128, scale=_E_SCALE[key])
    check(lib.gp_affinity_cs_fragments(_ptr(eh), _ptr(el), op.nv, 128, int(op.k), float(sharpen), _ptr(op.bu_off), _ptr(op.bu_row),
                                       _ptr(op.bu_mask), _ptr(op.valid), int(op.block_rows), _ptr(op.wa_hi), _ptr(op.wa_lo), _stream()),
          "gp_affinity_cs_fragments")
    op.filled = True
    return op


def pool_ell(x, nbr, w, d, out):
    lib = _lib.load()
    nv, k = nbr.shape
    check(lib.gp_pool_ell(_ptr(x), x.stride(0), _ptr(nbr), _ptr(w), int(k), nv, int(d), _ptr(out), out.stride(0),
                          _stream()), "gp_pool_ell")
    return out


def _flat_nk(t, dtype, nv, k, name):
    if _chk(t, dtype, name).shape != (nv, k):
        raise ValueError(f"{name}: expected [{nv}, {k}], got {list(t.shape)}")
    return t


def _rows(t, name, n=None, d=None):
    if t.dtype != torch.float32 or not t.is_cuda or t.dim() != 2 or t.stride(1) != 1:
        raise ValueError(f"{name}: expected CUDA fp32 rows with unit column stride, got {t.dtype} {list(t.shape)} strides {t.stride()}")
    if (n is not None and t.shape[0] != n) or (d is not None and t.shape[1] != d):
        raise ValueError(f"{name}: expected [{n}, {d}], got {list(t.shape)}")
    return t


def pool_transpose_build(nbr, tr_off=None, tr_slot=None, workspace=None):
    lib = _lib.load()
    _chk(nbr, torch.int32, "nbr")
    if nbr.dim() != 2:
        raise ValueError(f"pool_transpose_build: expected nbr [nv, k], got {list(nbr.shape)}")
    nv, k = nbr.shape
    dev = nbr.device
    if tr_off is None:
        tr_off = torch.empty(nv + 1, dtype=torch.int64, device=dev)
    elif _chk(tr_off, torch.int64, "tr_off").shape != (nv + 1,):
        raise ValueError(f"pool_transpose_build: expected tr_off [{nv + 1}], got {list(tr_off.shape)}")
    if tr_slot is None:
        tr_slot = torch.empty(nv * k, dtype=torch.int32, device=dev)
    elif _chk(tr_slot, torch.int32, "tr_slot").shape != (nv * k,):
        raise ValueError(f"pool_transpose_build: expected tr_slot [{nv * k}], got {list(tr_slot.shape)}")
    ws = _ws(lib.gp_pool_transpose_workspace_bytes(nv, int(k)), dev) if workspace is None else _chk(workspace, torch.uint8, "workspace")
    check(lib.gp_pool_transpose_build(_ptr(nbr), nv, int(k), _ptr(tr_off), _ptr(tr_slot), _ptr(ws), ws.numel(), _stream()),
          "gp_pool_transpose_build")
    return tr_off, tr_slot


def pool_ell_transpose(g, tr_off, tr_slot, w, k, out):
    lib = _lib.load()
    nv, d = _rows(g, "g").shape
    _rows(out, "out", nv, d)
    _chk(tr_off, torch.int64, "tr_off"), _chk(tr_slot, torch.int32, "tr_slot"), _chk(w, torch.float32, "w")
    if tr_off.shape != (nv + 1,) or tr_slot.numel() != w.numel():
        raise ValueError(f"pool_ell_transpose: expected tr_off [{nv + 1}] and one slot per weight, got {list(tr_off.shape)} / "
                         f"{tr_slot.numel()} / {w.numel()}")
    check(lib.gp_pool_ell_transpose(_ptr(g), g.stride(0), _ptr(tr_off), _ptr(tr_slot), _ptr(w), int(k), nv, int(d), _ptr(out),
                                    out.stride(0), _stream()), "gp_pool_ell_transpose")
    return out


def pool_ell_wgrad(g, x_prev, nbr, dw, accumulate):
    lib = _lib.load()
    nv, d = _rows(g, "g").shape
    _rows(x_prev, "x_prev", nv, d)
    _chk(nbr, torch.int32, "nbr")
    k = nbr.shape[1] if nbr.dim() == 2 else -1
    _flat_nk(nbr, torch.int32, nv, k, "nbr"), _flat_nk(dw, torch.float32, nv, k, "dw")
    check(lib.gp_pool_ell_wgrad(_ptr(g), g.stride(0), _ptr(x_prev), x_prev.stride(0), _ptr(nbr), int(k), nv, int(d), _ptr(dw),
                                int(bool(accumulate)), _stream()), "gp_pool_ell_wgrad")
    return dw


def affinity_softmax_backward(e_unit, nbr, w, dw, sharpen, tr_off, tr_slot, out=None, workspace=None):
    lib = _lib.load()
    nv, d = _rows(e_unit, "e_unit").shape
    _chk(nbr, torch.int32, "nbr")
    k = nbr.shape[1] if nbr.dim() == 2 else -1
    _flat_nk(nbr, torch.int32, nv, k, "nbr"), _flat_nk(w, torch.float32, nv, k, "w"), _flat_nk(dw, torch.float32, nv, k, "dw")
    _chk(tr_off, torch.int64, "tr_off"), _chk(tr_slot, torch.int32, "tr_slot")
    if tr_off.shape != (nv + 1,) or tr_slot.numel() != nv * k:
        raise ValueError(f"affinity_softmax_backward: expected tr_off [{nv + 1}] and tr_slot [{nv * k}], got {list(tr_off.shape)} / "
                         f"{list(tr_slot.shape)}")
    out = torch.empty((nv, d), dtype=torch.float32, device=e_unit.device) if out is None else _rows(out, "out", nv, d)
    ws = (_ws(lib.gp_affinity_softmax_backward_workspace_bytes(nv, int(k)), e_unit.device) if workspace is None
          else _chk(workspace, torch.uint8, "workspace"))
    check(lib.gp_affinity_softmax_backward(_ptr(e_unit), e_unit.stride(0), int(d), _ptr(nbr), _ptr(w), _ptr(dw), int(k), nv, float(sharpen),
                                           _ptr(tr_off), _ptr(tr_slot), _ptr(out), out.stride(0), _ptr(ws), ws.numel(), _stream()),
          "gp_affinity_softmax_backward")
    return out


def l2norm_rows_backward(e_raw, de_unit, out=None):
# ... 151 lines not shown
    xh, xl = x_split
    assert xh.stride(0) == xl.stride(0)
    yh, yl = out_split if out_split is not None else (None, None)
    check(lib.gp_pool_cs_apply(_ptr(xh), _ptr(xl), xh.stride(0), _ptr(op.bu_off), _ptr(op.bu_row), _ptr(op.bu_mask), _ptr(op.wa_hi),
                               _ptr(op.wa_lo), op.nv, int(d), int(op.block_rows), _ptr(yh), _ptr(yl), yh.stride(0) if yh is not None else 0,
                               _ptr(out_f32), out_f32.stride(0) if out_f32 is not None else 0, _ptr(out_scale), _stream()),
          "gp_pool_cs_apply")
    return out_f32 if out_f32 is not None else out_split


def pool_cs_deps(op, d=512):
    lib = _lib.load()
    words = _pool_cs_flag_words(op, d)
    dev = op.bu_row.device
    nb = op.bu_off.numel() - 1
    op.dep = torch.empty(nb * 64, dtype=torch.int32, device=dev)
    scratch = torch.empty(nb, dtype=torch.int32, device=dev)
    check(lib.gp_pool_cs_deps(_ptr(op.bu_off), _ptr(op.bu_row), op.nv, int(op.block_rows), _ptr(op.dep), _ptr(scratch), _stream()),
          "gp_pool_cs_deps")
    op.flags = torch.zeros(words, dtype=torch.int32, device=dev)
    op.epoch = 0
    return op


def _pool_cs_flag_words(op, d):
    words = _lib.load().gp_pool_cs_chain_flag_words_d(op.nv, int(op.block_rows), int(d))
    if words == 0:
        raise ValueError(f"pool_cs: d={d} (the column-sliced kernels take d = 256, 512, 768 or 1024)")
    return words


def pool_cs_apply_chain(x_split, pong, op, d, applications, out_f32, out_scale=None):
    lib = _lib.load()
    if getattr(op, "dep", None) is None:
        pool_cs_deps(op, d)
    elif op.flags is None or op.flags.numel() < _pool_cs_flag_words(op, d):
        op.flags = torch.zeros(_pool_cs_flag_words(op, d), dtype=torch.int32, device=op.bu_row.device)
        op.epoch = 0
    xh, xl = x_split
    ph, pl_ = pong
    assert xh.stride(0) == xl.stride(0) == ph.stride(0) == pl_.stride(0)
    check(lib.gp_pool_cs_apply_chain(_ptr(xh), _ptr(xl), _ptr(ph), _ptr(pl_), xh.stride(0), _ptr(op.bu_off), _ptr(op.bu_row),
                                     _ptr(op.bu_mask), _ptr(op.wa_hi), _ptr(op.wa_lo), op.nv, int(d), int(op.block_rows),
                                     int(applications), _ptr(out_f32), out_f32.stride(0), _ptr(out_scale), _ptr(op.dep), _ptr(op.flags),
                                     op.epoch & 0xFFFFFFFF, _stream()), "gp_pool_cs_apply_chain")
    op.epoch += int(applications)
    op.chain_done = torch.cuda.Event()
    op.chain_done.record(torch.cuda.current_stream(xh.device))
    return out_f32


def pool_cs_chain_check(op):
    if getattr(op, "flags", None) is None:
        return
    ev = getattr(op, "chain_done", None)
    if ev is not None:
        ev.synchronize()
    if int(op.flags[0].item()) != 0:
        raise _lib.GeoPurifyHipError("gp_pool_cs_apply_chain: a workgroup waited 2 s for a dependency; the pooled features are invalid")


def pool_mfma_apply_persistent(x_split, op, d, out_split=None, out_f32=None, out_scale=None, dynamic=True):
    lib = _lib.load()
    xh, xl = x_split
    assert xh.stride(0) == xl.stride(0)
    yh, yl = out_split if out_split is not None else (None, None)
    rows = (yh if yh is not None else out_f32).shape[0]
    check(lib.gp_pool_mfma_apply_persistent(_ptr(xh), _ptr(xl), xh.stride(0), _ptr(op.bu_off), _ptr(op.bu_row), _ptr(op.wa_hi),
                                            _ptr(op.wa_lo), op.nv, int(d), int(op.block_rows), int(op.min_steps), _ptr(yh), _ptr(yl),
                                            yh.stride(0) if yh is not None else 0, _ptr(out_f32),
                                            out_f32.stride(0) if out_f32 is not None else 0, int(rows), _ptr(out_scale),
                                            _ptr(op.queue) if dynamic else None, _stream()),
          "gp_pool_mfma_apply_persistent")
    return out_f32 if out_f32 is not None else out_split


def lift_dense_accum(feat2d, pt, x, y, sum_, cnt):
    lib = _lib.load()
    d, H, W = feat2d.shape
    check(lib.gp_lift_dense_accum(_ptr(feat2d), d, H, W, _ptr(pt), _ptr(x), _ptr(y), pt.shape[0], _ptr(sum_),
                                  sum_.stride(0), _ptr(cnt), _stream()), "gp_lift_dense_accum")


def lift_dense_bilinear_accum(feat_lo, out_h, out_w, pt, x, y, sum_, cnt):
    lib = _lib.load()
    d, h, w = feat_lo.shape
    check(lib.gp_lift_dense_bilinear_accum(_ptr(feat_lo), d, h, w, int(out_h), int(out_w), _ptr(pt), _ptr(x), _ptr(y),
                                           pt.shape[0], _ptr(sum_), sum_.stride(0), _ptr(cnt), _stream()),
          "gp_lift_dense_bilinear_accum")


def lift_dense_finish(sum_, d, cnt):
    lib = _lib.load()
    n = sum_.shape[0]
    seen = torch.empty(n, dtype=torch.uint8, device=sum_.device)
    check(lib.gp_lift_dense_finish(_ptr(sum_), sum_.stride(0), int(d), _ptr(cnt), n, _ptr(seen), _stream()),
          "gp_lift_dense_finish")
    return seen


def lift_masks_view(pred_masks, scores, taps, out_hw, x, y, want_logit=False, workspace=None):
    lib = _lib.load()
    Q, h, w = pred_masks.shape
    n_v = x.shape[0]
    dev = pred_masks.device
    need = lib.gp_lift_masks_workspace_bytes(Q, h, w)
    if workspace is None or workspace.numel() < need:
        workspace = _ws(need, dev)
    seg = torch.empty(n_v, dtype=torch.int32, device=dev)
    lg = torch.empty(n_v, dtype=torch.float32, device=dev) if want_logit else None
    tx0, twx, ty0, twy = taps
    check(lib.gp_lift_masks_view(_ptr(pred_masks), Q, h, w, _ptr(scores), _ptr(tx0), _ptr(twx), _ptr(ty0), _ptr(twy),
                                 int(out_hw[0]), int(out_hw[1]), _ptr(x), _ptr(y), n_v, _ptr(seg), _ptr(lg),
                                 _ptr(workspace), workspace.numel(), _stream()), "gp_lift_masks_view")
    return (seg, lg) if want_logit else seg


def segment_tables(mask_embed, text_norm, logit_scale, f_seg, logit_seg):
    lib = _lib.load()
    Q, d = mask_embed.shape
    C = text_norm.shape[0]
    check(lib.gp_segment_tables(_ptr(mask_embed), Q, d, _ptr(text_norm), C, float(logit_scale), _ptr(f_seg),
                                _ptr(logit_seg), _stream()), "gp_segment_tables")


def pv_count(pt, cnt):
    lib = _lib.load()
    check(lib.gp_pv_count(_ptr(pt), pt.shape[0], _ptr(cnt), _stream()), "gp_pv_count")


def exclusive_scan_i64(x):
    lib = _lib.load()
    n = x.shape[0]
    out = torch.empty_like(x)
    ws = _ws(lib.gp_scan_workspace_bytes(n), x.device)
    check(lib.gp_exclusive_scan_i64(_ptr(x), n, _ptr(out), _ptr(ws), ws.numel(), _stream()), "gp_exclusive_scan_i64")
    return out


def pv_fill(pt, seg, view, pv_start, cursor, pv_view, pv_seg):
    lib = _lib.load()
    check(lib.gp_pv_fill(_ptr(pt), _ptr(seg), pt.shape[0], int(view), _ptr(pv_start), _ptr(cursor), _ptr(pv_view),
                         _ptr(pv_seg), _stream()), "gp_pv_fill")


def fuse_views_top3(pv_start, pv_view, pv_seg, n, f_seg, logit_seg, out):
    lib = _lib.load()
    V, Q, d = f_seg.shape
    C = logit_seg.shape[2]
    seen = torch.empty(n, dtype=torch.uint8, device=out.device)
    check(lib.gp_fuse_views_top3(_ptr(pv_start), _ptr(pv_view), _ptr(pv_seg), int(n), _ptr(f_seg), _ptr(logit_seg),
                                 Q, d, C, _ptr(out), out.stride(0), _ptr(seen), _stream()), "gp_fuse_views_top3")
    return seen


def nn1(ref_xyz, query_xyz):
    lib = _lib.load()
    _chk(ref_xyz, torch.float32, "ref_xyz")
    _chk(query_xyz, torch.float32, "query_xyz")
    nr, nq = ref_xyz.shape[0], query_xyz.shape[0]
    nn = torch.empty(nq, dtype=torch.int64, device=ref_xyz.device)
    if nq == 0:
        return nn
    ws = _ws(lib.gp_nn1_workspace_bytes(nr, nq), ref_xyz.device)
    check(lib.gp_nn1_f64(_ptr(ref_xyz), nr, _ptr(query_xyz), nq, _ptr(nn), _ptr(ws), ws.numel(), _stream()), "gp_nn1_f64")
    return nn


def nn1_masked(xyz, ref_mask, query_mask, workspace=None):
    lib = _lib.load()
    _chk(xyz, torch.float32, "xyz")
    n = xyz.shape[0]
    nn = torch.empty(n, dtype=torch.int64, device=xyz.device)
    need = lib.gp_nn1_masked_workspace_bytes(n)
    if workspace is None or workspace.numel() < need:
        workspace = _ws(need, xyz.device)
    check(lib.gp_nn1_masked_f64(_ptr(xyz), n, _ptr(ref_mask), _ptr(query_mask), _ptr(nn), _ptr(workspace),
                                workspace.numel(), _stream()), "gp_nn1_masked_f64")
    return nn


def visible_lists(mapping, pt, x, y, count_dev, workspace=None):
    lib = _lib.load()
    n = mapping.shape[0]
    need = lib.gp_visible_lists_workspace_bytes(n)
    if workspace is None or workspace.numel() < need:
        workspace = _ws(need, mapping.device)
    check(lib.gp_visible_lists(_ptr(mapping), n, _ptr(pt), _ptr(x), _ptr(y), _ptr(count_dev), _ptr(workspace),
                               workspace.numel(), _stream()), "gp_visible_lists")


def views_visible_lists(coords, params, depth_all, width, height, cut_bound, vis_thres, min_visible, val_keep):
    lib = _lib.load()
    _chk(coords, torch.float64, "coords")
    _chk(params, torch.float64, "params")
    n, nv = coords.shape[0], params.shape[0]
    dev = coords.device
    if depth_all is not None:
        _chk(depth_all, torch.float64, "depth_all")
        assert depth_all.shape == (nv, height, width)
    ent = {"pt": torch.empty(nv * n, dtype=torch.int64, device=dev), "x": torch.empty(nv * n, dtype=torch.int64, device=dev),
           "y": torch.empty(nv * n, dtype=torch.int64, device=dev), "view": torch.empty(nv * n, dtype=torch.int32, device=dev),
           "view_off": torch.empty(nv + 1, dtype=torch.int64, device=dev), "keep": torch.empty(nv, dtype=torch.uint8, device=dev)}
    ws = _ws(lib.gp_views_visible_lists_workspace_bytes(n, nv), dev)
    check(lib.gp_views_visible_lists(_ptr(coords), n, _ptr(params), _ptr(depth_all), nv, int(width), int(height), int(cut_bound),
                                     float(vis_thres), int(min_visible), int(val_keep), _ptr(ent["pt"]), _ptr(ent["x"]), _ptr(ent["y"]),
                                     _ptr(ent["view"]), _ptr(ent["view_off"]), _ptr(ent["keep"]), _ptr(ws), ws.numel(), _stream()),
          "gp_views_visible_lists")
    return ent


def lift_masks_views(pred_masks, scores, taps, out_hw, xyz, ent, total, nviews, fill_cap=None):
    lib = _lib.load()
    _chk(pred_masks, torch.float32, "pred_masks")
    _chk(scores, torch.float32, "scores")
    _chk(xyz, torch.float32, "xyz")
    nsrc, Q, h, w = pred_masks.shape
    n = xyz.shape[0]
    dev = xyz.device
    seg = torch.empty(total, dtype=torch.int32, device=dev)
    start = torch.empty(n + 1, dtype=torch.int64, device=dev)
    pvv = torch.empty(total, dtype=torch.int32, device=dev)
    pvs = torch.empty(total, dtype=torch.int32, device=dev)
    if fill_cap is None:
        fill_cap = min(int(total), max(int(total) // 4, 65536))
    ws = _ws(lib.gp_lift_masks_views_workspace_bytes(nsrc, Q, h, w, total, n, int(fill_cap)), dev)
    tx0, twx, ty0, twy = taps
    check(lib.gp_lift_masks_views(_ptr(pred_masks), nsrc, Q, h, w, _ptr(scores), _ptr(tx0), _ptr(twx), _ptr(ty0), _ptr(twy),
                                  int(out_hw[0]), int(out_hw[1]), _ptr(xyz), n, _ptr(ent["pt"]), _ptr(ent["x"]), _ptr(ent["y"]),
                                  _ptr(ent["view"]), _ptr(ent["view_off"]), _ptr(ent["keep"]), int(nviews), int(total), int(fill_cap), _ptr(seg),
                                  _ptr(start), _ptr(pvv), _ptr(pvs), _ptr(ws), ws.numel(), _stream()), "gp_lift_masks_views")
    return seg, start, pvv, pvs


def classify_argmax(feat, text_norm, logit_scale, d=None):
    lib = _lib.load()
    n = feat.shape[0]
    d = feat.shape[1] if d is None else d
    C = text_norm.shape[0]
    pred = torch.empty(n, dtype=torch.int64, device=feat.device)
    zero = torch.empty(n, dtype=torch.uint8, device=feat.device)
    check(lib.gp_classify_argmax(_ptr(feat), feat.stride(0), int(d), n, _ptr(text_norm), C, float(logit_scale),
                                 _ptr(pred), _ptr(zero), _stream()), "gp_classify_argmax")
    return pred, zero


def classify_argmax_gemm(feat, text_norm, d=None):
    lib = _lib.load()
    n = feat.shape[0]
    d = feat.shape[1] if d is None else d
    C = text_norm.shape[0]
    cpad = (C + 127) // 128 * 128
    w = torch.zeros((d, cpad), dtype=torch.float32, device=feat.device)
    w[:, :C] = text_norm.t()
    logits = sparse_conv(feat, None, w)
    pred = torch.empty(n, dtype=torch.int64, device=feat.device)
    zero = torch.empty(n, dtype=torch.uint8, device=feat.device)
    check(lib.gp_rows_argmax(_ptr(logits), logits.stride(0), C, n, _ptr(feat), feat.stride(0), int(d), _ptr(pred),
                             _ptr(zero), _stream()), "gp_rows_argmax")
    return pred, zero


def iou_hist(pred, target, num_classes, ignore_ids, counts):
    lib = _lib.load()
    ig = (ctypes.c_int64 * max(len(ignore_ids), 1))(*[int(v) for v in ignore_ids])
    check(lib.gp_iou_hist_i64(_ptr(pred), _ptr(target), pred.shape[0], int(num_classes), ig, len(ignore_ids),
                              _ptr(counts), _stream()), "gp_iou_hist_i64")
    return counts


def nn1_batched(keys_sorted, ids, ref_mask, query_mask, axes=7, nn=None, status=None, workspace=None):
    lib = _lib.load()
    _chk(keys_sorted, torch.int64, "keys")
    nv = keys_sorted.shape[0]
    if keys_sorted.dim() != 1:
        raise ValueError(f"nn1_batched: expected keys [nv], got {list(keys_sorted.shape)}")
    for t, dtype, name in ((ids, torch.int32, "ids"), (ref_mask, torch.uint8, "ref_mask"), (query_mask, torch.uint8, "query_mask")):
        if t is not None and _chk(t, dtype, name).shape != (nv,):
            raise ValueError(f"nn1_batched: expected {name} [{nv}], got {list(t.shape)}")
    dev = keys_sorted.device
    if nn is None:
        nn = torch.empty(nv, dtype=torch.int32, device=dev)
    elif _chk(nn, torch.int32, "nn").shape != (nv,):
        raise ValueError(f"nn1_batched: expected nn [{nv}], got {list(nn.shape)}")
    if status is None:
        status = torch.empty(4, dtype=torch.int32, device=dev)
    elif _chk(status, torch.int32, "status").shape != (4,):
        raise ValueError(f"nn1_batched: expected status [4], got {list(status.shape)}")
    ws = _ws(lib.gp_nn1_batched_workspace_bytes(nv), dev) if workspace is None else _chk(workspace, torch.uint8, "workspace")
    check(lib.gp_nn1_batched(_ptr(keys_sorted), _ptr(ids), _ptr(ref_mask), _ptr(query_mask), nv, int(axes), _ptr(nn), _ptr(status),
                             _ptr(ws), ws.numel(), _stream()), "gp_nn1_batched")
    return nn, status


def iou_hist_batched(pred, coords, target, num_batches, num_classes, ignore_ids, counts, index=None):
    lib = _lib.load()
    _chk(pred, torch.int64, "pred")
    _chk(coords, torch.int32, "coords")
    _chk(target, torch.int64, "target")
    _chk(counts, torch.int64, "counts")
    rows, n = pred.shape[0], target.shape[0]
    if pred.dim() != 1 or coords.shape != (rows, 4) or target.dim() != 1:
        raise ValueError(f"iou_hist_batched: expected pred [rows], coords [rows, 4], target [n], got {list(pred.shape)}, "
                         f"{list(coords.shape)}, {list(target.shape)}")
    if index is not None and _chk(index, torch.int64, "index").shape != (n,):
        raise ValueError(f"iou_hist_batched: expected index [{n}], got {list(index.shape)}")
# ... 603 lines not shown
```

geopurify_amd/pipeline.py:

```python
from dataclasses import dataclass, field
from typing import List, Optional

import numpy as np
import torch

from . import ops
from .bicubic import aa_bicubic_taps

GEO_DIM = 6
CONV_PAD = 32


def _pad_to(v, m):
    return (v + m - 1) // m * m


class StudentWeights:

    def __init__(self, state_dict, device, eps=1e-5, mode="f16x3", residual_from_planes=True, interleaved_rows=True, blocked_weights=True,
                 head="f16x3"):
        sd = {k: v.detach() for k, v in state_dict.items()}
        self.mode = mode
        self.residual_from_planes = bool(residual_from_planes)
        self.interleaved_rows = bool(interleaved_rows)
        self.blocked_weights = bool(blocked_weights)
        w0 = sd["input_layer.0.kernel"].float()
        self.cin = w0.shape[1]
        self.cin_pad = _pad_to(self.cin, CONV_PAD)
        self.hidden = w0.shape[2]
        w0p = torch.zeros((27, self.cin_pad, self.hidden), dtype=torch.float32)
        w0p[:, :self.cin] = w0
        self.layers = []
        self._add_layer(w0p, self._fold(sd, "input_layer.1", eps), device)
        self.num_blocks = 0
        while f"res_blocks.{self.num_blocks}.conv1.kernel" in sd:
            i = self.num_blocks
            self._add_layer(sd[f"res_blocks.{i}.conv1.kernel"].float(), self._fold(sd, f"res_blocks.{i}.norm1", eps), device)
            self._add_layer(sd[f"res_blocks.{i}.conv2.kernel"].float(), self._fold(sd, f"res_blocks.{i}.norm2", eps), device)
            self.num_blocks += 1
        self.w_out = sd["output_layer.kernel"].float().to(device).contiguous()
        self.embed = self.w_out.shape[1]
        self.head = None
        if (mode == "f16x3" and self.embed == 128 and self.hidden % 64 == 0 and all(l[0] == "f16x3" for l in self.layers)
                and head != "f32"):
            amax = float(self.w_out.abs().max().item())
            p2 = 2.0 ** int(np.floor(np.log2(16384.0 / amax))) if amax > 0 else 1.0
            hi, lo = ops.conv_weights_split(self.w_out.reshape(1, self.hidden, self.embed), p2, blocked=False)
            self.head = (hi, lo, 1.0 / p2)

    @staticmethod
    def _fold(sd, prefix, eps):
        s = sd[prefix + ".bn.weight"].float() / torch.sqrt(sd[prefix + ".bn.running_var"].float() + eps)
        b = sd[prefix + ".bn.bias"].float() - sd[prefix + ".bn.running_mean"].float() * s
        return s, b

    def _add_layer(self, w, bn, device):
        w = w.to(device).contiguous()
        scale, shift = bn[0].to(device).contiguous(), bn[1].to(device).contiguous()
        use_fast = self.mode == "f16x3" and w.shape[2] % 256 == 0
        if use_fast:
            amax = float(w.abs().max().item())
            p2 = 2.0 ** int(np.floor(np.log2(16384.0 / amax))) if amax > 0 else 1.0
            hi, lo = ops.conv_weights_split(w, p2, blocked=None if self.blocked_weights else False)
            self.layers.append(("f16x3", (hi, lo), (scale / p2).contiguous(), shift))
        else:
            self.layers.append(("f32", w, scale, shift))

    def _conv(self, li, x, ctx, residual=None, x_split=None, want_split=False, want_f32=True, il=False):
        kind, w, scale, shift = self.layers[li]
        if kind == "f16x3":
            out_split = None
            if want_split:
                nv, cout = ctx["pairs"].nv, ops.conv_weights_shape(w[0])[1]
                dev = w[0].device
                if il:
                    out_split = (torch.empty((nv, 2 * cout), dtype=torch.float16, device=dev), None, torch.empty(nv, dtype=torch.float32, device=dev))
                else:
                    out_split = (torch.empty((nv, cout), dtype=torch.float16, device=dev), torch.empty((nv, cout), dtype=torch.float16, device=dev),
                                 torch.empty(nv, dtype=torch.float32, device=dev))
            y = ops.sparse_conv_f16x3(x, ctx["pairs"], w[0], w[1], scale, shift, residual=residual, relu=True,
                                      x_split=x_split[:2] if x_split is not None else None,
                                      out_split=out_split[:2] if out_split is not None else None,
                                      x_row_inv=x_split[2] if x_split is not None else None,
                                      out_row_inv=out_split[2] if out_split is not None else None, want_f32=want_f32)
            return y, out_split
        return ops.sparse_conv(x, ctx["nbr_map"], w, scale, shift, residual=residual, relu=True), None

    @property
    def fast(self):
        return all(l[0] == "f16x3" for l in self.layers)

    def split_input(self, x):
        if not self.fast:
            return None
        return ops.split_f16(x, self.cin_pad, per_row=True, interleaved=self.residual_from_planes and self.interleaved_rows)

    def forward(self, x, nbr_map, pairs=None, x_split=None, mark=None, planes=False, plane_rows=None, raw=False):
        if raw and planes:
            raise ValueError("StudentWeights.forward: raw=True returns fp32 rows, not planes")
        ctx = {"nbr_map": nbr_map, "pairs": pairs}
        fast = self.fast
        if pairs is None and any(l[0] == "f16x3" for l in self.layers):
            ctx["pairs"] = ops.conv_pairs_build(nbr_map, col_tiles=max(1, self.hidden // 256))
        xs = (x_split if x_split is not None else self.split_input(x)) if fast else None
        planes_res = fast and self.residual_from_planes
        il = planes_res and self.interleaved_rows
        h, hs = self._conv(0, x, ctx, x_split=xs, want_split=fast, want_f32=not planes_res, il=il)
        for b in range(self.num_blocks):
            t, ts = self._conv(1 + 2 * b, h, ctx, x_split=hs, want_split=fast, want_f32=not fast, il=il)
            last = b == self.num_blocks - 1
            head = last and fast and self.head is not None
            h, hs = self._conv(2 + 2 * b, t, ctx, residual=hs if planes_res else h, x_split=ts, want_split=fast and (not last or head),
                               want_f32=not (head or (planes_res and not last)), il=il and not last)
        self.last_pairs = ctx["pairs"]
        if mark is not None:
            mark("student convolutions")
        if fast and self.head is not None and hs is not None:
            if raw:
                return ops.embed_head_f16x3(hs[:2], self.head[0], self.head[1], self.head[2], x_row_inv=hs[2], normalize=False)
            if planes:
                return ops.embed_head_f16x3(hs[:2], self.head[0], self.head[1], self.head[2], x_row_inv=hs[2], normalize=True,
                                            planes=True, want_f32=False, plane_rows=plane_rows)[1]
            return ops.embed_head_f16x3(hs[:2], self.head[0], self.head[1], self.head[2], x_row_inv=hs[2], normalize=True)
        e = ops.sparse_conv(h, None, self.w_out)
        if raw:
            return e
        e = ops.l2norm_rows_(e)
        if planes:
            return ops.split_f16(e, self.embed, scale=torch.tensor([ops.AFFINITY_PLANE_SCALE], dtype=torch.float32, device=e.device),
                                 dst_row=plane_rows)
        return e

    def flops(self, num_pairs, nv):
        per_pair = self.cin * self.hidden + 2 * self.num_blocks * self.hidden * self.hidden
        return 2.0 * num_pairs * per_pair + 2.0 * nv * self.hidden * self.embed


@dataclass
class ViewLists:
    pt: torch.Tensor
    x: torch.Tensor
    y: torch.Tensor
    src_view: int


@dataclass
class SceneBatch:
    scene_coords: torch.Tensor
    scene_coords_3d: torch.Tensor
    scene_inds_reconstruct: torch.Tensor
    scene_label: torch.Tensor
    scene_gauss_features: torch.Tensor
    views: List[ViewLists] = field(default_factory=list)
    order: Optional[torch.Tensor] = None
    seg_start: Optional[torch.Tensor] = None
    extent: Optional[list] = None
    imgs: Optional[torch.Tensor] = None
    ent: Optional[dict] = None

    def as_tuple(self):
        dev = self.scene_coords.device
        N = self.scene_coords.shape[0]
        e = torch.empty(0, device=dev)
        V = len(self.views)
        ori = torch.cat([torch.cat([torch.full((len(v.pt), 1), float(i), device=dev),
                                    self.scene_coords[v.pt]], 1) for i, v in enumerate(self.views)]) if V else e
        mask = torch.zeros((V, N), dtype=torch.long, device=dev)
        for i, v in enumerate(self.views):
            mask[i, v.pt] = 1
        vid = torch.arange(V, device=dev).repeat_interleave(N)
        mask_2ds = torch.stack([vid, mask.reshape(-1)], 1)
        xl = torch.cat([v.x for v in self.views]) if V else e.long()
        yl = torch.cat([v.y for v in self.views]) if V else e.long()
        imgs = self.imgs if self.imgs is not None else e
        return (self.scene_coords, self.scene_coords_3d, self.scene_inds_reconstruct, self.scene_label, ori,
                e, e, e, e, e, e, imgs, xl, yl, mask_2ds, e, e, e, (None,) * V, self.scene_gauss_features)


def _view_matrices(cfg, views):
    from .synthetic import mapper_intrinsics
    out = []
    for v in views:
        K = mapper_intrinsics(cfg, v.K)
        if cfg.dataset == "scannet":
            w2c = np.asarray(v.pose).T.astype(np.float64)
        else:
            w2c = np.linalg.inv(np.asarray(v.pose))
        out.append((w2c, K))
    return out


def _voxel_extent(vox):
    ci = vox["coords_aug"].to(torch.int32)
    return ops.minmax_i32(ci.contiguous())[3:6].to(torch.int64) + 1


def build_scene_batch(scene, rigid, device="cuda", val_keep=10_000_000, batch_views=True, mark=None):
    from .synthetic import mapper_intrinsics
    cfg = scene.cfg
    dev = torch.device(device)
    coords64 = scene.coords_dev if hasattr(scene, "coords_dev") else torch.from_numpy(scene.coords).to(dev)
    N = coords64.shape[0]
    vox = ops.voxelize(coords64, rigid)
    if mark is not None:
        mark("voxelize")
    W, H = cfg.image_dim
    V = len(scene.views)
    gauss = scene.gauss_dev if hasattr(scene, "gauss_dev") else torch.from_numpy(
        np.concatenate([scene.colors, scene.normals], 1).astype(np.float32)).to(dev)
    labels = scene.labels_dev if hasattr(scene, "labels_dev") else torch.from_numpy(scene.labels).to(dev)
    if batch_views and V and getattr(scene, "depth_all_dev", None) is not None and V * N < 2 ** 31:
        mats = _view_matrices(cfg, scene.views)
        params = np.stack([np.concatenate([m.reshape(16), [K[0, 0], K[1, 1], K[0, 2], K[1, 2]]]) for m, K in mats]).astype(np.float64)
        ent = ops.views_visible_lists(coords64, torch.from_numpy(params).to(dev), scene.depth_all_dev, W, H, cfg.cut_bound,
                                      cfg.vis_thres, cfg.min_visible, val_keep)
        tail = torch.cat([ent["view_off"], _voxel_extent(vox)])
        host = ops.readback(tail)
        views = []
        for i in range(V):
            o, n_v = host[i], host[i + 1] - host[i]
            if n_v == 0 or n_v < cfg.min_visible or n_v > val_keep:
                continue
            views.append(ViewLists(ent["pt"][o:o + n_v], ent["x"][o:o + n_v], ent["y"][o:o + n_v], i))
        ent["total"] = host[V]
        ent["max_nv"] = max([host[i + 1] - host[i] for i in range(V)] + [0])
        ent["sum_nv2"] = float(sum((host[i + 1] - host[i]) ** 2 for i in range(V)))
        ent["num_views"] = V
        if mark is not None:
            mark("project+lists")
        return SceneBatch(coords64.float(), vox["coords_aug"].float(), vox["inds_reconstruct"], labels, gauss, views,
                          vox["order"], vox["seg_start"], host[V + 1:V + 4], ent=ent)
    depth_dev = scene.depth_dev if hasattr(scene, "depth_dev") else [torch.from_numpy(v.depth).to(dev) for v in scene.views]
    pt = torch.empty((V, N), dtype=torch.int64, device=dev)
    xs = torch.empty((V, N), dtype=torch.int64, device=dev)
    ys = torch.empty((V, N), dtype=torch.int64, device=dev)
    counts = torch.zeros(V + 3, dtype=torch.int64, device=dev)
    ws = None
    for i, (w2c, K) in enumerate(_view_matrices(cfg, scene.views)):
        mapping = ops.project_points(coords64, w2c, K[0, 0], K[1, 1], K[0, 2], K[1, 2], depth_dev[i], W, H,
                                     cfg.cut_bound, cfg.vis_thres)
        if ws is None:
            ws = torch.empty(ops._lib.load().gp_visible_lists_workspace_bytes(N), dtype=torch.uint8, device=dev)
        ops.visible_lists(mapping, pt[i], xs[i], ys[i], counts[i:i + 1], ws)
    counts[V:V + 3] = _voxel_extent(vox)
    host = counts.cpu().tolist()
    views = []
    for i in range(V):
        n_v = host[i]
# ... 44 lines not shown
    def __init__(self, feat_maps, text_embed, logit_scale, device="cuda"):
        dev = torch.device(device)
        self.feat = torch.as_tensor(feat_maps).to(dev)
        self.text_embed = torch.as_tensor(text_embed).to(dev)
        self.logit_scale = float(logit_scale)


class LSegFeatureVLM:

    def __init__(self, feat_lo, image_shape, text_embed, logit_scale, device="cuda"):
        dev = torch.device(device)
        self.feat_lo = torch.as_tensor(feat_lo).to(dev).contiguous()
        self.image_shape = tuple(int(v) for v in image_shape)
        self.text_embed = torch.as_tensor(text_embed).to(dev)
        self.logit_scale = float(logit_scale)


POOL_MODES = {"auto": None, "mfma_cs": "cs", "mfma_chain": "chain", "mfma": "mfma", "mfma_persist": "mfma_persist", "tiles": "tiles",
              "ell": "ell"}


def _known_pool_mode(mode):
    if mode not in POOL_MODES:
        raise ValueError(f"pool_mode={mode!r}: one of {', '.join(POOL_MODES)}")
    return mode


def resolve_pool_mode(mode, D, K, num_iters, tile_rows, block_rows):
    family = POOL_MODES[_known_pool_mode(mode)]
    mfma_ok = D == 512 and block_rows * K <= 16384 and num_iters >= 1
    cs_ok = D % 256 == 0 and 256 <= D <= 1024 and 128 * K <= 12288 and num_iters >= 1
    tiles_ok = num_iters > 1 and tile_rows * K <= 1536 and (D % 512 == 0 or (D == 64 and tile_rows in (4, 8)))
    if family is None:
        if (cs_ok or mfma_ok) and num_iters >= 3 and D in (256, 512, 768):
            return "cs" if cs_ok else "mfma"
        return "tiles" if tiles_ok else "ell"
    if family in ("cs", "chain"):
        if not cs_ok:
            raise ValueError(f"pool_mode='{mode}' needs D in (256, 512, 768, 1024) and K <= 96 (D={D}, K={K})")
        return "chain" if family == "chain" and num_iters >= 2 else "cs"
    if family in ("mfma", "mfma_persist") and not mfma_ok:
        raise ValueError(f"pool_mode='mfma' needs D == 512 and block_rows*K <= 16384 (D={D}, K={K})")
    if family == "tiles" and not tiles_ok:
        return "ell"
    return family


class HotPath:

    def __init__(self, student: StudentWeights, mask_shape, K=96, sharpen=20.0, num_iters=19, device="cuda",
                 pool_mode="auto", pool_tile_rows=8, pool_block_rows=64, batch_views=True, pool_structure_ahead=True, affinity_mfma=True,
                 all_views_max_pairs=2e11, pool_row_order="rcb"):
        self.student = student
        self.batch_views = batch_views
        self.all_views_max_pairs = float(all_views_max_pairs)
        self.pool_mode, self.pool_tile_rows, self.pool_block_rows = _known_pool_mode(pool_mode), pool_tile_rows, pool_block_rows
        self.pool_structure_ahead = bool(pool_structure_ahead)
        self.affinity_mfma = bool(affinity_mfma)
        self.pool_row_order = pool_row_order
        self.mask_shape = tuple(mask_shape)
        self.K, self.sharpen, self.num_iters = K, sharpen, num_iters
        self.device = torch.device(device)
        self._taps = {}
        self.stats = {}
        self.stage_mark = None
        self._chain_ops = []
        self.keep_lifted, self.last_lifted = False, None

    def _tap_tables(self, h, w):
        key = (h, w)
        if key not in self._taps:
            H, W = self.mask_shape
            tx0, twx = aa_bicubic_taps(w, W)
            ty0, twy = aa_bicubic_taps(h, H)
            d = self.device
            self._taps[key] = tuple(torch.from_numpy(a).to(d) for a in (tx0, twx, ty0, twy))
        return self._taps[key]

    def lift_masks(self, batch: SceneBatch, vlm):
        dev = self.device
        N = batch.scene_coords.shape[0]
        V = len(batch.views)
        has_img = batch.imgs is not None and batch.imgs.numel() > 0
        batched = ((not has_img or getattr(vlm, "ignores_image", False)) and torch.is_tensor(getattr(vlm, "mask_embed", None))
                   and vlm.mask_embed.dim() == 3 and vlm.mask_embed.is_contiguous())
        outs = None
        if batched:
            text_embed, logit_scale = vlm.text_embed, float(vlm.logit_scale)
            Q, D = vlm.mask_embed.shape[1:]
        else:
            outs = [vlm(v.src_view, image=batch.imgs[v.src_view]) if has_img else vlm(v.src_view) for v in batch.views]
            if V:
                text_embed, logit_scale = outs[0]["text_embed"].to(dev), float(outs[0]["logit_scale"])
                Q, D = outs[0]["mask_embed"].shape
            else:
                text_embed, logit_scale = vlm.text_embed, float(vlm.logit_scale)
                Q, D = 1, text_embed.shape[1]
        text_norm = torch.nn.functional.normalize(text_embed, dim=-1).contiguous()
        C = text_norm.shape[0]
        n_tab = vlm.mask_embed.shape[0] if batched else max(V, 1)
        f_seg = torch.empty((n_tab, Q, D), dtype=torch.float32, device=dev)
        l_seg = torch.empty((n_tab, Q, C), dtype=torch.float32, device=dev)
        if batched:
            ops.segment_tables(vlm.mask_embed.view(n_tab * Q, D), text_norm, logit_scale,
                               f_seg.view(n_tab * Q, D), l_seg.view(n_tab * Q, C))
        scores_all = None
        if batched and getattr(vlm, "pred_logits", None) is not None and vlm.pred_logits.dim() == 3:
            scores_all = torch.softmax(vlm.pred_logits, dim=-1)[..., :-1].max(-1).values.contiguous()
        ent = batch.ent
        pm_all = getattr(vlm, "pred_masks", None)
        all_views = (self.batch_views and batched and scores_all is not None and ent is not None and ent["total"] > 0
                     and ent["num_views"] <= 128 and ent.get("sum_nv2", float(ent["max_nv"]) ** 2 * ent["num_views"]) / 4 <= self.all_views_max_pairs
                     and torch.is_tensor(pm_all) and pm_all.dim() == 4 and pm_all.is_contiguous()
                     and pm_all.shape[0] >= ent["num_views"] and pm_all.shape[1] <= 1024)
        if all_views:
            _, start, pvv, pvs = ops.lift_masks_views(pm_all, scores_all, self._tap_tables(pm_all.shape[2], pm_all.shape[3]),
                                                      self.mask_shape, batch.scene_coords, ent, ent["total"], ent["num_views"])
            return self._fuse_and_fill(batch, start, pvv, pvs, f_seg, l_seg, D, text_norm, logit_scale)
        cnt = torch.zeros(N + 1, dtype=torch.int64, device=dev)
        segs = []
        ws_m = ws_n = None
        for i, v in enumerate(batch.views):
            out = vlm(v.src_view) if batched else outs[i]
            pm = out["pred_masks"].to(dev).contiguous()
            scores = scores_all[v.src_view] if scores_all is not None else \
                torch.softmax(out["pred_logits"].to(dev), dim=-1)[..., :-1].max(-1).values.contiguous()
            if ws_m is None:
                lib = ops._lib.load()
                ws_m = torch.empty(lib.gp_lift_masks_workspace_bytes(*pm.shape), dtype=torch.uint8, device=dev)
                ws_n = torch.empty(lib.gp_nn1_masked_workspace_bytes(N), dtype=torch.uint8, device=dev)
            seg = ops.lift_masks_view(pm, scores, self._tap_tables(pm.shape[1], pm.shape[2]), self.mask_shape,
                                      v.x, v.y, workspace=ws_m)
            xyz = batch.scene_coords[v.pt].contiguous()
            covered = (seg >= 0).to(torch.uint8)
            nn = ops.nn1_masked(xyz, covered, 1 - covered, workspace=ws_n)
            seg = torch.where(nn >= 0, seg[nn.clamp(min=0)], seg)
            if not batched:
                ops.segment_tables(out["mask_embed"].to(dev).contiguous(), text_norm, logit_scale, f_seg[i], l_seg[i])
            ops.pv_count(v.pt, cnt)
            segs.append(seg)
        start = ops.exclusive_scan_i64(cnt)
        total = sum(len(v.pt) for v in batch.views)
        cursor = torch.zeros(N, dtype=torch.int32, device=dev)
        pvv = torch.empty(max(total, 1), dtype=torch.int32, device=dev)
        pvs = torch.empty(max(total, 1), dtype=torch.int32, device=dev)
        for i, v in enumerate(batch.views):
            ops.pv_fill(v.pt, segs[i], v.src_view if batched else i, start, cursor, pvv, pvs)
        return self._fuse_and_fill(batch, start, pvv, pvs, f_seg, l_seg, D, text_norm if V else text_embed, logit_scale)

    def _fuse_and_fill(self, batch, start, pvv, pvs, f_seg, l_seg, D, text, logit_scale):
        dev = self.device
        N = batch.scene_coords.shape[0]
        F = torch.empty((N, D), dtype=torch.float32, device=dev)
        seen = ops.fuse_views_top3(start, pvv, pvs, N, f_seg, l_seg, F)
        nn = ops.nn1_masked(batch.scene_coords, seen, 1 - seen)
        src = torch.where(nn >= 0, nn, torch.arange(N, device=dev))
        F = ops.gather_rows(F, D, src)
        return F, text, logit_scale

    def lift_dense(self, batch: SceneBatch, vlm: DenseFeatureVLM):
        dev = self.device
        N = batch.scene_coords.shape[0]
        D = vlm.feat.shape[1]
        s = torch.zeros((N, D), dtype=torch.float32, device=dev)
        cnt = torch.zeros(N, dtype=torch.float32, device=dev)
        for v in batch.views:
            ops.lift_dense_accum(vlm.feat[v.src_view], v.pt, v.x, v.y, s, cnt)
        seen = ops.lift_dense_finish(s, D, cnt)
        nn = ops.nn1_masked(batch.scene_coords, seen, 1 - seen)
        src = torch.where(nn >= 0, nn, torch.arange(N, device=dev))
        return ops.gather_rows(s, D, src), vlm.text_embed, vlm.logit_scale

    def lift_lseg(self, batch: SceneBatch, vlm: LSegFeatureVLM):
        dev = self.device
        N = batch.scene_coords.shape[0]
        D = vlm.feat_lo.shape[1]
        H, W = vlm.image_shape
        s = torch.zeros((N, D), dtype=torch.float32, device=dev)
        cnt = torch.zeros(N, dtype=torch.float32, device=dev)
        for v in batch.views:
            ops.lift_dense_bilinear_accum(vlm.feat_lo[v.src_view], H, W, v.pt, v.x, v.y, s, cnt)
        seen = ops.lift_dense_finish(s, D, cnt)
        nn = ops.nn1_masked(batch.scene_coords, seen, 1 - seen)
        src = torch.where(nn >= 0, nn, torch.arange(N, device=dev))
        return ops.gather_rows(s, D, src), vlm.text_embed, vlm.logit_scale

    def prepare(self, batch: SceneBatch, F):
        dev = self.device
        N, D = F.shape
        st = self.student
        assert st.cin == D + GEO_DIM, f"student expects {st.cin} input channels, lift gives {D}+{GEO_DIM}"
        coords = batch.scene_coords_3d.floor().to(torch.int32).contiguous()
        Nv = coords.shape[0]
        perm, rank = ops.morton_order(coords)
        cs = coords[perm.long()].contiguous()
        mark = self.stage_mark if self.stage_mark is not None else (lambda name: None)
        mark("morton order")
        if batch.order is None:
            order = torch.sort(batch.scene_inds_reconstruct, stable=True).indices
            segc = torch.zeros(Nv + 1, dtype=torch.int64, device=dev)
            segc[1:] = torch.bincount(batch.scene_inds_reconstruct, minlength=Nv).cumsum(0)
            batch.order, batch.seg_start = order, segc
        X = torch.zeros((Nv, st.cin_pad), dtype=torch.float32, device=dev)
        ops.scatter_mean_csr(F, D, batch.order, batch.seg_start, Nv, X, col0=0, row_map=rank)
        ops.scatter_mean_csr(batch.scene_gauss_features, GEO_DIM, batch.order, batch.seg_start, Nv, X, col0=D,
                             row_map=rank)
        mark("scatter_mean")
        if batch.extent is not None:
            grid = ops.grid_build(cs, [0, 0, 0], batch.extent)
        else:
            grid = ops.grid_build(cs)
        nbr_map = ops.kernel_map_build(grid, cs)
        pairs = ops.conv_pairs_build(nbr_map, col_tiles=max(1, st.hidden // 256)) if any(l[0] == "f16x3" for l in st.layers) else None
        mark("grid+kernel_map")
        nbr = ops.knn_lattice(grid, cs, perm, self.K)
        mark("kNN")
        state = {"X": X, "rank": rank, "nbr_map": nbr_map, "pairs": pairs, "nbr": nbr, "Nv": Nv, "D": D, "pool": None,
                 "xs": st.split_input(X)}
        family = self._pool_family(D)
        if family in ("cs", "chain"):
            sc = ops.pow2_scale(X, D)
            how = self.pool_structure_ahead
            if how and self.affinity_mfma and self.K <= 96 and self.student is not None and self.student.embed == 128:
                how = "valid"
            rho = None
            nbr_op = nbr
            if how == "valid" and self.pool_row_order == "rcb" and Nv > 1024:
                sigma, rho = ops.rcb_order(cs, 1024, 128)
                nbr_op = ops.rows_renumber(nbr, sigma, rho)
                state["rank_pool"] = rho[rank.long()].contiguous()
            state["pool"] = {"op": ops.pool_cs_plan(nbr_op, structure=how), "sc": sc, "rho": rho, "nbr": nbr_op,
                             "x_split": ops.split_f16(X, D, scale=sc[0:1], dst_row=rho),
                             "pong": tuple(torch.empty((Nv, D), dtype=torch.float16, device=dev) for _ in range(2))}
            if family == "chain" and (state["pool"]["op"].dst is not None or state["pool"]["op"].valid is not None):
                ops.pool_cs_deps(state["pool"]["op"], D)
            mark("pool plan+split")
        return state

    def refine(self, batch: SceneBatch, F, after_student=None, prepared=None, classify_text=None):
        p = prepared if prepared is not None else self.prepare(batch, F)
        X, rank, nbr, Nv, D = p["X"], p["rank"], p["nbr"], p["Nv"], p["D"]
        mark = self.stage_mark if self.stage_mark is not None else (lambda name: None)
        op = p["pool"]["op"] if p["pool"] is not None else None
        mfma_aff = op is not None and op.valid is not None
        rho = p["pool"]["rho"] if (p["pool"] is not None and mfma_aff) else None
        E = self.student.forward(X, p["nbr_map"], p["pairs"], x_split=p.get("xs"), mark=self.stage_mark, planes=mfma_aff, plane_rows=rho)
        mark("embed head" if self.stage_mark is not None else "student")
        if after_student is not None:
            after_student()
        if mfma_aff:
            ops.affinity_cs_fragments(None, self.sharpen, op, planes=E)
            w = None
        else:
            w = ops.affinity_softmax(E, nbr, self.sharpen, into=op if op is not None and op.dst is not None else None)
        mark("affinity")
        self._last_E, self._last_E_rho = E, rho
        self._last_pool_inputs = (X, nbr, w, Nv, D)
        self._last_pool_plan = p["pool"]
        out = self._pool(X, nbr, w, Nv, D, plan=p["pool"])
        mark("pooling")
        self._fused_pred = None
        if classify_text is not None and ops.can_gather_rows_classify(D, classify_text[0].shape[0]) and classify_text[0].shape[0] <= 32:
            text_norm = torch.nn.functional.normalize(classify_text[0], dim=-1).contiguous()
            out, pred, zero = ops.gather_rows_classify(out, D, batch.scene_inds_reconstruct, text_norm, classify_text[1],
                                                       row_map=p.get("rank_pool", rank))
            self._fused_pred = (out, classify_text[0], pred, zero)
        else:
            out = ops.gather_rows(out, D, batch.scene_inds_reconstruct, row_map=p.get("rank_pool", rank))
        mark("gather")
        self.stats = {"Nv": Nv, "nbr_map": p["nbr_map"], "pool_bytes_per_iter": Nv * (2 * D * 4 + self.K * 8),
                      "pool_kernel": self._pool_kernel}
        return out

    def _pool_family(self, D):
        return resolve_pool_mode(self.pool_mode, D, self.K, self.num_iters, self.pool_tile_rows, self.pool_block_rows)

    def _pool(self, X, nbr, w, Nv, D, plan=None):
        dev = X.device
        family = self._pool_family(D)
        if w is None and (plan is None or not plan["op"].filled):
            E = self._last_E
            if isinstance(E, tuple):
                E = (E[0].float() + E[1].float()) / ops.AFFINITY_PLANE_SCALE
                if getattr(self, "_last_E_rho", None) is not None:
                    E = E[self._last_E_rho.long()]
            w = ops.affinity_softmax(E.contiguous(), nbr, self.sharpen)
        if self.num_iters == 0:
            out = torch.empty((Nv, D), dtype=torch.float32, device=dev)
            out.copy_(X[:, :D])
            self._pool_kernel = "none"
            return out
        if family in ("cs", "chain"):
            if plan is None:
                sc = ops.pow2_scale(X, D)
                plan = {"op": ops.pool_cs_plan(nbr), "sc": sc, "x_split": ops.split_f16(X, D, scale=sc[0:1]),
                        "pong": tuple(torch.empty((Nv, D), dtype=torch.float16, device=dev) for _ in range(2))}
            op = plan["op"] if plan["op"].filled else ops.pool_cs_fill(plan["op"], nbr, w)
            out = torch.empty((Nv, D), dtype=torch.float32, device=dev)
            sc = plan["sc"]
            sp = [plan["x_split"], plan["pong"]]
            if self.stage_mark is not None:
                self.stage_mark("pool operator fill")
            if family == "chain":
                if op.dep is None:
                    ops.pool_cs_deps(op, D)
                ops.pool_cs_apply_chain(sp[0], sp[1], op, D, self.num_iters, out, out_scale=sc[1:2])
                if op not in self._chain_ops:
                    self._chain_ops.append(op)
                self._pool_kernel = "cs_chain_kernel" if D == 512 else "cs_chain_ns_kernel"
                return out
            src = sp[0]
            for t in range(self.num_iters):
                last = t == self.num_iters - 1
                dst = None if last else sp[(t + 1) % 2]
                ops.pool_cs_apply(src, op, D, out_split=dst, out_f32=out if last else None, out_scale=sc[1:2] if last else None)
                src = dst
            self._pool_kernel = "cs_pool_kernel" if D == 512 else "cs_pool_ns_kernel"
            return out
        if family in ("mfma", "mfma_persist"):
            op = ops.pool_mfma_build(nbr, w, self.pool_block_rows, min_steps=9 if family == "mfma_persist" else 0)
            persistent = family == "mfma_persist" and op.min_steps >= 9 and self.pool_block_rows == 64
            rows = op.rows_padded if persistent else Nv
            out = torch.empty((rows, D), dtype=torch.float32, device=dev)
            sc = ops.pow2_scale(X, D)
            sp = [ops.split_f16(X, D, scale=sc[0:1]), tuple(torch.empty((rows, D), dtype=torch.float16, device=dev) for _ in range(2))]
            if persistent and self.num_iters > 1:
                sp.append(tuple(torch.empty((rows, D), dtype=torch.float16, device=dev) for _ in range(2)))
            apply = ops.pool_mfma_apply_persistent if persistent else ops.pool_mfma_apply
            src = sp[0]
            for t in range(self.num_iters):
                last = t == self.num_iters - 1
                dst = None if last else sp[1 + (t % 2)] if persistent else sp[(t + 1) % 2]
                apply(src, op, D, out_split=dst, out_f32=out if last else None, out_scale=sc[1:2] if last else None)
                src = dst
            self._pool_kernel = "pool_mfma_persist_kernel" if persistent else "pool_mfma_kernel"
            return out[:Nv]
        use_tiles = family == "tiles"
        tiles = ops.pool_tiles_build(nbr, w, self.pool_tile_rows) if use_tiles else None
        bufs = [torch.empty((Nv, D), dtype=torch.float32, device=dev) for _ in range(2)]
        cur = X
        for t in range(self.num_iters):
            if use_tiles:
                ops.pool_tiles_apply(cur, tiles, D, bufs[t % 2])
            else:
                ops.pool_ell(cur, nbr, w, D, bufs[t % 2])
            cur = bufs[t % 2]
        self._pool_kernel = ("pool_tiles64_kernel" if D == 64 else "pool_tiles_kernel") if use_tiles else "pool_ell_kernel"
        return cur

    def evaluate_scene(self, batch: SceneBatch, vlm):
        if isinstance(vlm, LSegFeatureVLM):
            F, text, scale = self.lift_lseg(batch, vlm)
        elif isinstance(vlm, DenseFeatureVLM):
            F, text, scale = self.lift_dense(batch, vlm)
        else:
            F, text, scale = self.lift_masks(batch, vlm)
        if self.keep_lifted:
            self.last_lifted = F
        feats = self.refine(batch, F)
        if self._chain_ops:
            self.pool_chain_check()
        return {"scene_features": feats, "text_features": text, "logit_scale": scale}

    def pool_chain_check(self, block=True):
        keep = []
        while self._chain_ops:
            op = self._chain_ops[0]
            ev = getattr(op, "chain_done", None)
            if not block and ev is not None and not ev.query():
                keep.append(self._chain_ops.pop(0))
                continue
            ops.pool_cs_chain_check(op)
            self._chain_ops.pop(0)
        self._chain_ops = keep
# ... 55 lines not shown
```

include/geopurify_hip.h:

```cpp
#ifndef GEOPURIFY_HIP_H
#define GEOPURIFY_HIP_H

#include <stddef.h>
#include <stdint.h>

#ifdef __cplusplus
extern "C" {
#endif

#define GP_OK 0
#define GP_EINVAL (-22)
#define GP_ENOMEM (-12)
#define GP_EHIP (-5)
#define GP_ERANGE (-34)

#define GP_KNN_MAX_K 127

int gp_version(void);
int gp_debug_set(int32_t key, int32_t value);
int gp_debug_ptr(int32_t key, void *device_buffer, size_t bytes);
const char *gp_last_error(void);

size_t gp_voxelize_workspace_bytes(int64_t n);
int gp_voxelize_f64(const double *coords, int64_t n, const double *rigid_host,
                    double *coords_aug, int64_t *inds, int64_t *inds_reconstruct, int64_t *nv_dev,
                    int64_t *order, int64_t *seg_start,
                    void *workspace, size_t workspace_bytes, void *stream);
int gp_fnv_hash_f64(const double *coords, int64_t n, uint64_t *hash, void *stream);

int gp_project_points_f64(const double *coords, int64_t n, const double *w2c_host,
                          double fx, double fy, double cx, double cy,
                          const double *depth, int32_t width, int32_t height,
                          int32_t cut_bound, double vis_thres,
                          int64_t *mapping, double *weight, void *stream);
int gp_render_depth_f64(const double *coords, int64_t n, const double *w2c_host,
                        double fx, double fy, double cx, double cy, int32_t width, int32_t height,
                        int32_t cut_bound, double *depth, void *stream);

int gp_minmax_i32(const int32_t *coords, int64_t nv, int32_t *mm, void *stream);
size_t gp_morton_order_workspace_bytes(int64_t nv);
int gp_morton_order(const int32_t *coords, int64_t nv, int32_t *perm, int32_t *rank,
                    void *workspace, size_t workspace_bytes, void *stream);
size_t gp_grid_bytes(int64_t nv, const int32_t *extent_host);
int gp_grid_build(const int32_t *coords, int64_t nv, const int32_t *origin_host,
                  const int32_t *extent_host, void *grid, size_t grid_bytes, void *stream);

int gp_scatter_mean_csr(const float *src, int64_t ld_src, int32_t d, const int64_t *order,
                        const int64_t *seg_start, int64_t nv, const int32_t *row_map,
                        float *out, int64_t ld_out, int32_t col0, void *stream);
int gp_gather_rows(const float *src, int64_t ld_src, int32_t d, const int64_t *index, int64_t n,
                   const int32_t *row_map, float *out, int64_t ld_out, void *stream);

int gp_kernel_map_build(const void *grid, const int32_t *coords, int64_t nv, int32_t *nbr_map,
                        void *stream);
size_t gp_coords_order_batched_workspace_bytes(int64_t nv);
int gp_coords_order_batched(const int32_t *coords, int64_t nv, int32_t *perm, int32_t *rank, uint64_t *keys_sorted,
                            int32_t *status, void *workspace, size_t workspace_bytes, void *stream);
size_t gp_quantize_batched_workspace_bytes(int64_t n);
int gp_quantize_batched(const int32_t *coords, int64_t n, int32_t *vox_coords, int64_t *unique_index, int64_t *inverse,
                        int64_t *order, int64_t *seg_start, int32_t *status, void *workspace, size_t workspace_bytes,
                        void *stream);
int gp_segment_labels(const int64_t *labels, int64_t n, const int64_t *order, const int64_t *seg_start,
                      const int64_t *unique_index, int64_t nv, int64_t ignore_label, int32_t rule, int64_t *out, void *stream);
int gp_kernel_map_sorted(const uint64_t *keys_sorted, int64_t nv, int32_t *nbr_map, void *stream);
int gp_sparse_conv(const float *x, int64_t ld_x, const int32_t *nbr_map, int64_t nv,
                   const float *w, int32_t kv, int32_t cin, int32_t cout,
                   const float *scale, const float *shift, const float *residual, int64_t ld_res,
                   int32_t relu, float *y, int64_t ld_y, void *stream);
int gp_sparse_conv_tiles(int32_t *tiles);
size_t gp_conv_pairs_workspace_bytes(int64_t nv, int32_t kv);
int gp_conv_pairs_build(const int32_t *nbr_map, int64_t nv, int32_t kv, int32_t num_chunks, const int32_t *chunk_row_off,
                        int32_t *pair_in, int32_t *pair_pos, int32_t *seg_off, int32_t *tile_start,
                        int32_t *tile_desc ,
                        void *workspace, size_t workspace_bytes, void *stream);
size_t gp_conv_chunk_plan_workspace_bytes(int64_t nv, int32_t granule_rows);
int gp_conv_chunk_plan(const int32_t *nbr_map, int64_t nv, int32_t kv, int32_t granule_rows, int32_t col_tiles,
                       int32_t target_tiles, int32_t max_chunks, int32_t *chunk_row_off, int32_t *n_chunks, void *workspace,
                       size_t workspace_bytes, void *stream);
int gp_conv_weights_split(const float *w, int32_t kv, int32_t cin, int32_t cout, float scale_pow2,
                          void *w_hi, void *w_lo, void *stream);
int gp_split_f16(const float *x, int64_t ld_x, int32_t d, int64_t n, void *hi, void *lo, int64_t ld_h,
                 void *stream);
int gp_pow2_scale(const float *x, int64_t ld_x, int32_t d, int64_t n, float *scale2, void *workspace,
                  size_t workspace_bytes, void *stream);
int gp_split_f16_scaled(const float *x, int64_t ld_x, int32_t d, int64_t n, void *hi, void *lo, int64_t ld_h,
                        const float *scale, float *row_inv_scale, const int32_t *dst_row, void *stream);
int gp_sparse_conv_f16x3(const float *x, int64_t ld_x, const void *x_hi, const void *x_lo, int64_t ld_xh,
                         const int32_t *pair_in, const int32_t *pair_pos,
                         const int32_t *seg_off, const int32_t *tile_start, const int32_t *tile_desc,
                         int32_t nseg, int64_t num_pairs, int64_t nv, int32_t kv,
                         const void *w_hi, const void *w_lo, int32_t cin, int32_t cout, float *partial,
                         const float *scale, const float *shift, const float *residual, int64_t ld_res,
                         int32_t relu, float *y, int64_t ld_y, void *y_hi, void *y_lo, int64_t ld_yh,
                         int32_t num_chunks, const int32_t *chunk_row_off_host, const int32_t *chunk_tile_off_host,
                         const int32_t *chunk_pair_off_host, const float *x_row_inv_scale, float *y_row_inv_scale,
                         const void *res_hi, const void *res_lo, int64_t ld_rh, const float *res_row_inv_scale, int32_t w_blocked,
                         int32_t plane_flags, void *stream);
int gp_conv_weights_split_blocked(const float *w, int32_t kv, int32_t cin, int32_t cout, float scale_pow2,
                                  void *w_hi, void *w_lo, int32_t transpose_flip, void *stream);
int gp_l2norm_rows(float *x, int64_t ld, int32_t d, int64_t n, void *stream);
int gp_embed_head_f16x3(const void *x_hi, const void *x_lo, int64_t ld_x, const float *x_row_inv_scale, const void *w_hi,
                        const void *w_lo, int64_t nv, int32_t cin, int32_t cout, float out_scale, int32_t l2_normalize,
                        float *y, int64_t ld_y, void *e_hi, void *e_lo, float plane_scale,
                        const int32_t *e_dst_row ,
                        void *stream);

int gp_rcb_order(const int32_t *coords, int64_t nv, int32_t chunk_rows, int32_t leaf_rows, int32_t *sigma, int32_t *rho, void *stream);
int gp_rows_renumber_i32(const int32_t *nbr, int64_t nv, int32_t k, const int32_t *sigma, const int32_t *rho, int32_t *out,
                         void *stream);

size_t gp_knn_workspace_bytes(int64_t nv);
int gp_knn_lattice(const void *grid, const int32_t *coords, const int32_t *ids, int64_t nv,
                   int32_t k, int32_t *nbr, void *workspace, size_t workspace_bytes, void *stream);
size_t gp_knn_batched_workspace_bytes(int64_t nv);
int gp_knn_batched(const uint64_t *keys_sorted, const int32_t *ids, int64_t nv, int32_t k, int32_t *nbr, int32_t *status,
                   void *workspace, size_t workspace_bytes, void *stream);

int gp_affinity_softmax(const float *e, int64_t ld_e, int32_t d, const int32_t *nbr, int32_t k,
                        int64_t nv, float sharpen, float *w, void *stream);
int gp_affinity_softmax_scatter(const float *e, int64_t ld_e, int32_t d, const int32_t *nbr, int32_t k, int64_t nv,
                                float sharpen, float *w, const int32_t *dst, void *wa_hi, void *wa_lo, void *stream);

int gp_pool_ell(const float *x, int64_t ld_x, const int32_t *nbr, const float *w, int32_t k,
                int64_t nv, int32_t d, float *y, int64_t ld_y, void *stream);

size_t gp_pool_transpose_workspace_bytes(int64_t nv, int32_t k);
int gp_pool_transpose_build(const int32_t *nbr, int64_t nv, int32_t k, int64_t *tr_off, int32_t *tr_slot, void *workspace,
                            size_t workspace_bytes, void *stream);
int gp_pool_ell_transpose(const float *g, int64_t ld_g, const int64_t *tr_off, const int32_t *tr_slot, const float *w, int32_t k,
                          int64_t nv, int32_t d, float *out, int64_t ld_out, void *stream);
int gp_pool_ell_wgrad(const float *g, int64_t ld_g, const float *x_prev, int64_t ld_x, const int32_t *nbr, int32_t k, int64_t nv,
                      int32_t d, float *dw, int32_t accumulate, void *stream);
size_t gp_affinity_softmax_backward_workspace_bytes(int64_t nv, int32_t k);
int gp_affinity_softmax_backward(const float *e_unit, int64_t ld_e, int32_t d, const int32_t *nbr, const float *w, const float *dw,
                                 int32_t k, int64_t nv, float sharpen, const int64_t *tr_off, const int32_t *tr_slot, float *de_unit,
                                 int64_t ld_de, void *workspace, size_t workspace_bytes, void *stream);
int gp_l2norm_rows_backward(const float *e_raw, int64_t ld_e, const float *de_unit, int64_t ld_du, int32_t d, int64_t n,
                            float *de_raw, int64_t ld_de, void *stream);

size_t gp_pool_tiles_workspace_bytes(int64_t nv, int32_t r);
int gp_pool_tiles_count(const int32_t *nbr, int64_t nv, int32_t k, int32_t r, int64_t *tile_off,
                        void *workspace, size_t workspace_bytes, void *stream);
int gp_pool_tiles_fill(const int32_t *nbr, const float *w, int64_t nv, int32_t k, int32_t r,
                       const int64_t *tile_off, int32_t *u_row, float *u_w, void *stream);
int gp_pool_tiles_apply(const float *x, int64_t ld_x, const int64_t *tile_off, const int32_t *u_row,
                        const float *u_w, int32_t r, int64_t nv, int32_t d, float *y, int64_t ld_y,
                        void *stream);

size_t gp_pool_mfma_workspace_bytes(int64_t nv, int32_t block_rows);
int gp_pool_mfma_count(const int32_t *nbr, int64_t nv, int32_t k, int32_t block_rows, int32_t min_steps,
                       int64_t *bu_off, int32_t *bu_n, void *workspace, size_t workspace_bytes, void *stream);
int gp_pool_mfma_fill(const int32_t *nbr, const float *w, int64_t nv, int32_t k, int32_t block_rows,
                      const int64_t *bu_off, const int32_t *bu_n, int64_t total_rows, int32_t *bu_row,
                      void *wa_hi, void *wa_lo, void *stream);
int gp_pool_mfma_apply(const void *x_hi, const void *x_lo, int64_t ld_x, const int64_t *bu_off,
                       const int32_t *bu_row, const void *wa_hi, const void *wa_lo, int64_t nv, int32_t d,
                       int32_t block_rows, void *y_hi, void *y_lo, int64_t ld_y, float *y_f32,
                       int64_t ld_yf, const float *out_scale, void *stream);
int gp_pool_mfma_apply_persistent(const void *x_hi, const void *x_lo, int64_t ld_x, const int64_t *bu_off,
                                  const int32_t *bu_row, const void *wa_hi, const void *wa_lo, int64_t nv,
                                  int32_t d, int32_t block_rows, int32_t min_steps, void *y_hi, void *y_lo,
                                  int64_t ld_y, float *y_f32, int64_t ld_yf, int64_t y_rows,
                                  const float *out_scale, uint32_t *queue, void *stream);

size_t gp_pool_cs_workspace_bytes(int64_t nv, int32_t rows_per_block);
int gp_pool_cs_count(const int32_t *nbr, int64_t nv, int32_t k, int32_t rows_per_block, int64_t *bu_off, int32_t *bu_n,
                     int64_t *max_union, void *workspace, size_t workspace_bytes, void *stream);
int gp_pool_cs_fill(const int32_t *nbr, const float *w, int64_t nv, int32_t k, int32_t rows_per_block, const int64_t *bu_off,
                    int64_t total_rows, int32_t max_union, int32_t *bu_row, uint32_t *bu_mask, void *wa_hi, void *wa_lo, void *stream);
int gp_pool_cs_structure(const int32_t *nbr, int64_t nv, int32_t k, int32_t rows_per_block, const int64_t *bu_off,
                         int64_t total_rows, int32_t max_union, int32_t *bu_row, uint32_t *bu_mask, void *wa_hi, void *wa_lo,
                         int32_t *dst, void *stream);
int gp_pool_cs_structure_valid(const int32_t *nbr, int64_t nv, int32_t k, int32_t rows_per_block, const int64_t *bu_off,
                               int64_t total_rows, int32_t max_union, int32_t *bu_row, uint32_t *bu_mask, uint32_t *bu_valid,
                               void *stream);
int gp_affinity_cs_fragments(const void *e_hi, const void *e_lo, int64_t nv, int32_t d, int32_t k, float sharpen,
                             const int64_t *bu_off, const int32_t *bu_row, const uint32_t *bu_mask, const uint32_t *bu_valid,
                             int32_t rows_per_block, void *wa_hi, void *wa_lo, void *stream);
int gp_pool_cs_apply(const void *x_hi, const void *x_lo, int64_t ld_x, const int64_t *bu_off, const int32_t *bu_row,
                     const uint32_t *bu_mask, const void *wa_hi, const void *wa_lo, int64_t nv, int32_t d,
                     int32_t rows_per_block, void *y_hi, void *y_lo, int64_t ld_y, float *y_f32, int64_t ld_yf,
                     const float *out_scale, void *stream);
int gp_pool_cs_deps(const int64_t *bu_off, const int32_t *bu_row, int64_t nv, int32_t rows_per_block, int32_t *dep,
                    int32_t *scratch, void *stream);
size_t gp_pool_cs_chain_flag_words(int64_t nv, int32_t rows_per_block);
size_t gp_pool_cs_chain_flag_words_d(int64_t nv, int32_t rows_per_block, int32_t d);
int gp_pool_cs_apply_chain(void *x_hi, void *x_lo, void *p_hi, void *p_lo, int64_t ld, const int64_t *bu_off,
                           const int32_t *bu_row, const uint32_t *bu_mask, const void *wa_hi, const void *wa_lo, int64_t nv,
                           int32_t d, int32_t rows_per_block, int32_t applications, float *y_f32, int64_t ld_yf,
                           const float *out_scale, const int32_t *dep, uint32_t *flags, uint32_t epoch, void *stream);

int gp_lift_dense_accum(const float *feat2d, int32_t d, int32_t height, int32_t width,
                        const int64_t *pt, const int64_t *x, const int64_t *y, int64_t n_v,
                        float *sum, int64_t ld_sum, float *cnt, void *stream);
int gp_lift_dense_bilinear_accum(const float *feat, int32_t d, int32_t h, int32_t w, int32_t out_h, int32_t out_w,
                                 const int64_t *pt, const int64_t *x, const int64_t *y, int64_t n_v,
                                 float *sum, int64_t ld_sum, float *cnt, void *stream);
int gp_lift_dense_finish(float *sum, int64_t ld_sum, int32_t d, const float *cnt, int64_t n,
                         uint8_t *seen, void *stream);
size_t gp_lift_masks_workspace_bytes(int32_t q, int32_t h, int32_t w);
int gp_lift_masks_view(const float *pred_masks, int32_t q, int32_t h, int32_t w,
                       const float *scores, const int32_t *tap_x0, const float *tap_wx,
                       const int32_t *tap_y0, const float *tap_wy, int32_t out_h, int32_t out_w,
                       const int64_t *x, const int64_t *y, int64_t n_v, int32_t *seg,
                       float *seg_logit, void *workspace, size_t workspace_bytes, void *stream);
size_t gp_lift_masks_views_workspace_bytes(int32_t nsrc, int32_t q, int32_t h, int32_t w, int64_t total, int64_t n,
                                           int64_t fill_cap);
int gp_lift_masks_views(const float *pred_masks, int32_t nsrc, int32_t q, int32_t h, int32_t w, const float *scores,
                        const int32_t *tap_x0, const float *tap_wx, const int32_t *tap_y0, const float *tap_wy,
                        int32_t out_h, int32_t out_w, const float *xyz, int64_t n, const int64_t *ent_pt,
                        const int64_t *ent_x, const int64_t *ent_y, const int32_t *ent_view, const int64_t *view_off,
                        const uint8_t *keep, int32_t nviews, int64_t total, int64_t fill_cap, int32_t *seg, int64_t *pv_start,
                        int32_t *pv_view, int32_t *pv_seg, void *workspace, size_t workspace_bytes, void *stream);
int gp_segment_tables(const float *mask_embed, int32_t q, int32_t d, const float *text_norm,
                      int32_t c, float logit_scale, float *f_seg, float *logit_seg, void *stream);
int gp_pv_count(const int64_t *pt, int64_t n_v, int64_t *cnt, void *stream);
size_t gp_scan_workspace_bytes(int64_t n);
int gp_exclusive_scan_i64(const int64_t *in, int64_t n, int64_t *out, void *workspace,
                          size_t workspace_bytes, void *stream);
int gp_pv_fill(const int64_t *pt, const int32_t *seg, int64_t n_v, int32_t view,
               const int64_t *pv_start, int32_t *cursor, int32_t *pv_view, int32_t *pv_seg,
               void *stream);
int gp_fuse_views_top3(const int64_t *pv_start, const int32_t *pv_view, const int32_t *pv_seg,
                       int64_t n, const float *f_seg, const float *logit_seg, int32_t q, int32_t d,
                       int32_t c, float *out, int64_t ld_out, uint8_t *seen, void *stream);
size_t gp_nn1_workspace_bytes(int64_t n_ref, int64_t n_query);
int gp_nn1_f64(const float *ref_xyz, int64_t n_ref, const float *query_xyz, int64_t n_query,
               int64_t *nn, void *workspace, size_t workspace_bytes, void *stream);
size_t gp_nn1_masked_workspace_bytes(int64_t n);
int gp_nn1_masked_f64(const float *xyz, int64_t n, const uint8_t *ref_mask, const uint8_t *query_mask,
                      int64_t *nn, void *workspace, size_t workspace_bytes, void *stream);
size_t gp_visible_lists_workspace_bytes(int64_t n);
int gp_visible_lists(const int64_t *mapping, int64_t n, int64_t *pt, int64_t *x, int64_t *y,
                     int64_t *count_dev, void *workspace, size_t workspace_bytes, void *stream);
size_t gp_views_visible_lists_workspace_bytes(int64_t n, int32_t nviews);
int gp_views_visible_lists(const double *coords, int64_t n, const double *params, const double *depth, int32_t nviews,
                           int32_t width, int32_t height, int32_t cut_bound, double vis_thres, int64_t min_visible,
                           int64_t val_keep, int64_t *ent_pt, int64_t *ent_x, int64_t *ent_y, int32_t *ent_view,
                           int64_t *view_off, uint8_t *keep, void *workspace, size_t workspace_bytes, void *stream);

int gp_classify_argmax(const float *feat, int64_t ld, int32_t d, int64_t n, const float *text_norm,
                       int32_t c, float logit_scale, int64_t *pred, uint8_t *zero_row, void *stream);
int gp_gather_rows_classify(const float *src, int64_t ld_src, int32_t d, const int64_t *index, int64_t n, const int32_t *row_map,
                            float *out, int64_t ld_out, const float *text_norm, int32_t c, float logit_scale, int64_t *pred,
                            uint8_t *zero_row, void *stream);
int gp_rows_argmax(const float *logits, int64_t ld, int32_t c, int64_t n, const float *feat, int64_t ld_f,
                   int32_t d, int64_t *pred, uint8_t *zero_row, void *stream);
int gp_iou_hist_i64(const int64_t *pred, const int64_t *target, int64_t n, int32_t num_classes,
                    const int64_t *ignore_ids_host, int32_t num_ignore, int64_t *counts,
                    void *stream);
size_t gp_nn1_batched_workspace_bytes(int64_t nv);
int gp_nn1_batched(const uint64_t *keys_sorted, const int32_t *ids, const uint8_t *ref_mask, const uint8_t *query_mask, int64_t nv,
                   int32_t axes, int32_t *nn, int32_t *status, void *workspace, size_t workspace_bytes, void *stream);
int gp_iou_hist_batched_i64(const int64_t *pred, const int32_t *coords, int64_t rows, const int64_t *target, const int64_t *index,
                            int64_t n, int32_t num_batches, int32_t num_classes, const int64_t *ignore_ids_host, int32_t num_ignore,
                            int64_t *counts, void *stream);
int32_t gp_segment_loss_col_step(void);
int gp_segment_loss_unit_rows(const float *y, int64_t ld_y, int32_t d, int64_t n, float *u, int64_t ld_u, int32_t d_pad, uint8_t *zero,
                              void *stream);
size_t gp_segment_loss_items_workspace_bytes(int64_t n, int64_t p);
int gp_segment_loss_items(const int32_t *coords, const uint8_t *zero, int64_t n, const int64_t *labels, const int64_t *index, int64_t p,
                          int32_t c, const int64_t *ignore_ids_host, int32_t num_ignore, int32_t reduction, uint8_t *row_valid,
                          int64_t *item_off, int32_t *item_id, int64_t *entry_cnt, float *entry_w, int64_t *status, void *workspace,
                          size_t workspace_bytes, void *stream);
int gp_segment_loss_rows(const float *z, int64_t ld_z, int64_t r, int32_t c, int32_t c_pad, const int32_t *coords, const uint8_t *row_valid,
                         const int64_t *item_off, const int32_t *item_id, const int64_t *labels, const float *entry_w, float *g,
                         int64_t ld_g, float *lse, double *term, void *stream);
size_t gp_segment_loss_reduce_workspace_bytes(int64_t n, int32_t num_entries);
int gp_segment_loss_reduce(const double *term, const int32_t *coords, int64_t n, const int64_t *entry_cnt, int32_t num_entries,
                           int32_t reduction, float *loss, float *per_entry, void *workspace, size_t workspace_bytes, void *stream);

size_t gp_col_stats_workspace_bytes(int64_t nv, int32_t c);
int gp_col_stats(const float *y, int64_t ld, int64_t nv, int32_t c, float *mean, float *var,
                 void *workspace, size_t workspace_bytes, void *stream);
int gp_bn_train_apply(const float *y, int64_t ld, int64_t nv, int32_t c, const float *mean, const float *var,
                      const float *gamma, const float *beta, float eps, const float *residual, int64_t ld_res,
                      int32_t relu, float *out, int64_t ld_out, void *out_hi, void *out_lo, int64_t ld_split,
                      float momentum, float *running_mean, float *running_var, void *stream);
size_t gp_bn_train_backward_workspace_bytes(int64_t nv, int32_t c);
int gp_bn_train_backward(const float *dout, int64_t ld_dout, const float *act, int64_t ld_act, const float *y,
                         int64_t ld_y, const float *mean, const float *var, float eps, const float *gamma, const float *beta_mask,
                         int64_t nv, int32_t c, float *dy, int64_t ld_dy, float *dz_out, int64_t ld_dz,
                         float *dgamma, float *dbeta, float *dy_scale2, void *dy_hi, void *dy_lo, int64_t ld_h,
                         void *workspace, size_t workspace_bytes, void *stream);
int gp_col_sums_f64(const float *y, int64_t ld, int64_t nv, int32_t c, const float *mean, double *out, void *workspace,
                    size_t workspace_bytes, void *stream);
int gp_bn_bwd_sums_f64(const float *dout, int64_t ld_dout, const float *act, int64_t ld_act, const float *y, int64_t ld_y,
                       const float *mean, const float *var, float eps, const float *gamma_mask, const float *beta_mask, int64_t nv, int32_t c,
                       double *sums, void *workspace, size_t workspace_bytes, void *stream);
int gp_bn_bwd_apply(const float *dout, int64_t ld_dout, const float *act, int64_t ld_act, const float *y, int64_t ld_y,
                    const float *mean, const float *var, float eps, const float *gamma, const float *beta_mask, const float *sums,
                    int64_t n_total, int64_t nv, int32_t c, float *dy, int64_t ld_dy, float *dz_out, int64_t ld_dz, float *dy_scale2,
                    void *stream);
size_t gp_infonce_workspace_bytes(int64_t num_samples, int32_t d);
int gp_infonce_fwd_bwd(const float *e, int64_t ld_e, int64_t nv, int32_t d, const int64_t *sample_to_voxel,
                       int64_t num_samples, const int64_t *point_to_batch, int64_t num_anchors,
                       int32_t num_negatives, float temperature, float *loss, float *de, int64_t ld_de,
                       void *workspace, size_t workspace_bytes, void *stream);
int gp_infonce_weighted_fwd_bwd(const float *e, int64_t ld_e, int64_t nv, int32_t d, const int64_t *sample_to_voxel,
                                int64_t num_samples, const int64_t *point_to_batch, int64_t num_anchors, int32_t num_negatives,
                                float temperature, const float *weights, float *loss, float *anchor_loss, float *de, int64_t ld_de,
                                void *workspace, size_t workspace_bytes, void *stream);
size_t gp_conv_wgrad_workspace_bytes(int64_t num_segments, int32_t cin_pad, int32_t cout);
int gp_conv_wgrad_f16x3(const void *x_hi, const void *x_lo, int64_t ld_x, const void *y_hi, const void *y_lo,
                        int64_t ld_y, const int32_t *pair_in, const int32_t *pair_out, const int32_t *segs,
                        int64_t num_segments, const int32_t *seg_off, int32_t kv, int32_t cin_pad, int32_t cin_out,
                        int32_t cout, const float *inv_scale, float *dw, void *workspace, size_t workspace_bytes,
                        void *stream);
int gp_adamw_step(float *param, const float *grad, float *exp_avg, float *exp_avg_sq, int64_t n, float lr,
                  float beta1, float beta2, float eps, float weight_decay, int64_t step, void *stream);
int gp_knn_points_f32(const float *xyz, int64_t n, const int64_t *queries, int64_t num_queries, int32_t k,
                      int64_t *out, int32_t *flag_dev, void *stream);
int gp_sampler_select(const float *sim, int64_t ld, int64_t num_anchors, int64_t n, const int64_t *anchor_idx, int32_t k,
                      int64_t *positive, int64_t *macro, void *stream);
int gp_sim_segments_f16x3(const void *hi, const void *lo, int64_t ld_h, int32_t d, const int32_t *anchor_row, const int32_t *seg_first,
                          const int32_t *seg_len, const int64_t *row_off, int64_t num_anchors, int64_t max_len, float *out,
                          void *stream);
int gp_sampler_select_segments(const float *sim, const int64_t *row_off, const int32_t *row_len, const int32_t *row_base,
                               int64_t num_anchors, int64_t max_len, const int64_t *anchor_idx, int32_t k, int64_t *positive,
                               int64_t *macro, void *stream);
int gp_sampler_micro_segments(const float *sim, const int64_t *row_off, const int32_t *seg_first, const int32_t *seg_len,
                              const int32_t *nbr, int64_t ld_nbr, int32_t k, const int64_t *positive, int64_t num_anchors,
                              int32_t num_micro, int64_t *micro, void *stream);
int gp_normalize_split_f16(const float *x, int64_t ld_x, int32_t d, int64_t n, int64_t n_pad, float eps, void *hi, void *lo,
                           int64_t ld_h, void *stream);

size_t gp_fused_decode_workspace_bytes(int64_t n, int64_t nv);
int gp_fused_decode(const uint8_t *mask_chunk, int64_t n, const uint8_t *row_keep, const void *feat,
                    int64_t feat_rows, int64_t row_bytes, const int64_t *vox_ind, int64_t nv, int32_t mode,
                    void *out, uint8_t *mask_out, int64_t *n_sel, void *workspace, size_t workspace_bytes,
                    void *stream);

int32_t gp_lift_batched_col_chunk(void);
int gp_lift_batched_transpose(const float *src, int32_t nviews, int32_t d, int64_t hw, float *dst, void *stream);
size_t gp_lift_batched_workspace_bytes(int64_t n, int32_t nviews);
int gp_lift_batched(const double *points, int64_t n, const float *feat, int32_t d, int32_t h, int32_t w,
                    const int64_t *view_entry, const double *w2c, const double *intrinsics, const double *depth,
                    int32_t nviews, int32_t height, int32_t width, int32_t bilinear, int32_t cut_bound, double vis_thres,
                    int64_t min_visible, int64_t max_visible, int32_t fill, float *out, int64_t ld_out, uint8_t *seen,
                    int32_t *count, int64_t *view_count, uint8_t *view_keep, int64_t *nn, int64_t *status,
                    void *workspace, size_t workspace_bytes, void *stream);

size_t gp_lift_masks_batched_lists_workspace_bytes(int64_t n, int32_t nviews);
int gp_lift_masks_batched_lists(const double *points, int64_t n, const int64_t *view_entry, const double *w2c,
                                const double *intrinsics, const double *depth, int32_t nviews, int32_t height, int32_t width,
                                int32_t cut_bound, double vis_thres, int64_t min_visible, int64_t max_visible, int64_t cap,
                                int64_t *ent_pt, int64_t *ent_x, int64_t *ent_y, int32_t *ent_view, int64_t *view_off,
                                int64_t *view_count, uint8_t *view_keep, int64_t *status, void *workspace,
                                size_t workspace_bytes, void *stream);
size_t gp_lift_masks_batched_workspace_bytes(int64_t n, int32_t nviews, int32_t q, int32_t h, int32_t w, int32_t out_h,
                                             int32_t out_w, int64_t total, int32_t words, int64_t fill_cap);
int gp_lift_masks_batched(const double *points, int64_t n, const int64_t *view_entry, int32_t nviews,
                          const float *pred_masks, int32_t q, int32_t h, int32_t w, const float *scores,
                          const int32_t *tap_x0, const float *tap_wx, const int32_t *tap_y0, const float *tap_wy,
                          int32_t out_h, int32_t out_w, const int64_t *ent_pt, const int64_t *ent_x, const int64_t *ent_y,
                          const int32_t *ent_view, const int64_t *view_off, const uint8_t *keep, int64_t total, int32_t words,
                          int64_t fill_cap, const float *f_seg, const float *logit_seg, int32_t d, int32_t c, int32_t fill,
                          float *out, int64_t ld_out, uint8_t *seen, int32_t *count, int64_t *nn, int32_t *seg, int64_t *status,
                          void *workspace, size_t workspace_bytes, void *stream);

#ifdef __cplusplus
}
#endif
#endif
```

Measured before the change: 46.77.

## Fuse voxel pooling with operand split, keep kNN candidates in registers, fill unseen during fusion

Three separate changes. First, a new voxel_rows kernel does the scatter-mean of 2D features and geometry, the per-row pow2 scaling and the f16 hi/lo interleaved split in a single pass. This replaces two scatter_mean_csr calls, the split_input pass and the pow2_scale pass. Second, the radius-1 kNN ring kernel keeps candidate rows and their squared distances packed in registers, so the selection pass reuses them instead of re-reading coordinates. Third, view fusion now computes seen/unseen masks first and writes each point's features from its nearest seen neighbour directly, which removes a gather, a torch.where and an arange. The cost is more register pressure in kNN and added code paths that depend on specific conditions.

```diff
diff --git a/geopurify_amd/_lib.py b/geopurify_amd/_lib.py
--- a/geopurify_amd/_lib.py
+++ b/geopurify_amd/_lib.py
@@ -48,6 +48,8 @@
                                        _P, _P, c_int64, _P, c_int32, c_int32, _P]),
     "gp_conv_weights_split_blocked": (c_int32, [_P, c_int32, c_int32, c_int32, c_float, _P, _P, c_int32, _P]),
     "gp_pow2_scale": (c_int32, [_P, c_int64, c_int32, c_int64, _P, _P, c_size_t, _P]),
+    "gp_voxel_rows_operands": (c_int32, [_P, c_int64, c_int32, _P, c_int64, c_int32, _P, _P, c_int64, _P, _P, c_int64, c_int32, _P, c_int64,
+                                         _P, _P, _P, c_size_t, _P]),
     "gp_split_f16_scaled": (c_int32, [_P, c_int64, c_int32, c_int64, _P, _P, c_int64, _P, _P, _P, _P]),
     "gp_rcb_order": (c_int32, [_P, c_int64, c_int32, c_int32, _P, _P, _P]),
     "gp_rows_renumber_i32": (c_int32, [_P, c_int64, c_int32, _P, _P, _P, _P]),
@@ -55,6 +57,7 @@
     "gp_embed_head_f16x3": (c_int32, [_P, _P, c_int64, _P, _P, _P, c_int64, c_int32, c_int32, c_float, c_int32, _P, c_int64, _P, _P, c_float, _P, _P]),
     "gp_knn_workspace_bytes": (c_size_t, [c_int64]),
     "gp_knn_lattice": (c_int32, [_P, _P, _P, c_int64, c_int32, _P, _P, c_size_t, _P]),
+    "gp_knn_lattice_two_pass": (c_int32, [_P, _P, _P, c_int64, c_int32, _P, _P, c_size_t, _P]),
     "gp_knn_batched_workspace_bytes": (c_size_t, [c_int64]),
     "gp_knn_batched": (c_int32, [_P, _P, c_int64, c_int32, _P, _P, _P, c_size_t, _P]),
     "gp_affinity_softmax": (c_int32, [_P, c_int64, c_int32, _P, c_int32, c_int64, c_float, _P, _P]),
@@ -103,6 +106,8 @@
     "gp_pv_fill": (c_int32, [_P, _P, c_int64, c_int32, _P, _P, _P, _P, _P]),
     "gp_segment_tables": (c_int32, [_P, c_int32, c_int32, _P, c_int32, c_float, _P, _P, _P]),
     "gp_fuse_views_top3": (c_int32, [_P, _P, _P, c_int64, _P, _P, c_int32, c_int32, c_int32, _P, c_int64, _P, _P]),
+    "gp_seen_masks": (c_int32, [_P, c_int64, _P, _P, _P]),
+    "gp_fuse_views_top3_fill": (c_int32, [_P, _P, _P, c_int64, _P, _P, c_int32, c_int32, c_int32, _P, _P, c_int64, _P]),
     "gp_nn1_workspace_bytes": (c_size_t, [c_int64, c_int64]),
     "gp_nn1_f64": (c_int32, [_P, c_int64, _P, c_int64, _P, _P, c_size_t, _P]),
     "gp_nn1_masked_workspace_bytes": (c_size_t, [c_int64]),
diff --git a/geopurify_amd/csrc/knn.hip b/geopurify_amd/csrc/knn.hip
--- a/geopurify_amd/csrc/knn.hip
+++ b/geopurify_amd/csrc/knn.hip
@@ -11,7 +11,10 @@
     static constexpr int HB = (B + 63) / 64 * 64;
 };
 
-template <int R, int WAVES>
+constexpr int KNN_KEEP = 32;
+constexpr int KNN_KEEP_ROW_BITS = 25;
+
+template <int R, int WAVES, bool KEEP = false>
 __global__ void __launch_bounds__(WAVES * 64)
 knn_ring_kernel(const void *grid, const int32_t *__restrict__ coords, const int32_t *__restrict__ ids, int64_t nv,
                 int k, int32_t *__restrict__ nbr, const int32_t *__restrict__ qlist,
@@ -67,7 +70,30 @@
         return cstart[lo] + (j - coff[lo]);
     };
 
-    for (int j0 = 0; j0 < total_c; j0 += 128) {
+    static_assert(!KEEP || KnnCfg<R>::B <= 127, "a kept candidate holds d^2 in 7 bits");
+    const bool kept = KEEP && total_c <= 64 * KNN_KEEP;
+    unsigned keep[KEEP ? KNN_KEEP : 1];
+    if constexpr (KEEP) {
+        if (kept) {
+#pragma unroll
+            for (int i = 0; i < KNN_KEEP; i += 2) {
+                if (i * 64 < total_c) {
+                    const int ja = i * 64 + lane, jb = ja + 64;
+                    const bool va = ja < total_c, vb = jb < total_c;
+                    const int64_t ra = va ? row_of(ja) : 0, rb = vb ? row_of(jb) : 0;
+                    const int ax = coords[ra * 3], ay = coords[ra * 3 + 1], az = coords[ra * 3 + 2];
+                    const int bx = coords[rb * 3], by = coords[rb * 3 + 1], bz = coords[rb * 3 + 2];
+                    const int da = (ax - qx) * (ax - qx) + (ay - qy) * (ay - qy) + (az - qz) * (az - qz);
+                    const int db = (bx - qx) * (bx - qx) + (by - qy) * (by - qy) + (bz - qz) * (bz - qz);
+                    if (va && da < B) atomicAdd(&hist[da], 1);
+                    if (vb && db < B) atomicAdd(&hist[db], 1);
+                    keep[i] = ((unsigned)(va ? min(da, 127) : 127) << KNN_KEEP_ROW_BITS) | (unsigned)ra;
+                    keep[i + 1] = ((unsigned)(vb ? min(db, 127) : 127) << KNN_KEEP_ROW_BITS) | (unsigned)rb;
+                }
+            }
+        }
+    }
+    for (int j0 = kept ? total_c : 0; j0 < total_c; j0 += 128) {
         const int ja = j0 + lane, jb = j0 + 64 + lane;
         const bool va = ja < total_c, vb = jb < total_c;
         const int64_t ra = va ? row_of(ja) : 0, rb = vb ? row_of(jb) : 0;
@@ -119,23 +145,32 @@
         return;
     }
 
-    for (int j0 = 0; j0 < total_c; j0 += 64) {
+    auto emit = [&](int64_t r, int d2) {
+        if (d2 < T) {
+            int id = ids ? ids[r] : (int)r;
+            int p = atomicAdd(&s_cnt[wv][0], 1);
+            s_selkey[wv][p] = ((unsigned long long)(unsigned)d2 << 32) | (unsigned)id;
+            s_selrow[wv][p] = (int)r;
+        } else if (d2 == T) {
+            int id = ids ? ids[r] : (int)r;
+            int p = atomicAdd(&s_cnt[wv][1], 1);
+            s_tieid[wv][p] = id;
+            s_tierow[wv][p] = (int)r;
+        }
+    };
+    if constexpr (KEEP) {
+        if (kept) {
+#pragma unroll
+            for (int i = 0; i < KNN_KEEP; ++i)
+                if (i * 64 < total_c) emit((int64_t)(keep[i] & ((1u << KNN_KEEP_ROW_BITS) - 1u)), (int)(keep[i] >> KNN_KEEP_ROW_BITS));
+        }
+    }
+    for (int j0 = kept ? total_c : 0; j0 < total_c; j0 += 64) {
         const int j = j0 + lane;
         if (j < total_c) {
             const int64_t r = row_of(j);
             int ex = coords[r * 3] - qx, ey = coords[r * 3 + 1] - qy, ez = coords[r * 3 + 2] - qz;
-            int d2 = ex * ex + ey * ey + ez * ez;
-            if (d2 < T) {
-                int id = ids ? ids[r] : (int)r;
-                int p = atomicAdd(&s_cnt[wv][0], 1);
-                s_selkey[wv][p] = ((unsigned long long)(unsigned)d2 << 32) | (unsigned)id;
-                s_selrow[wv][p] = (int)r;
-            } else if (d2 == T) {
-                int id = ids ? ids[r] : (int)r;
-                int p = atomicAdd(&s_cnt[wv][1], 1);
-                s_tieid[wv][p] = id;
-                s_tierow[wv][p] = (int)r;
-            }
+            emit(r, ex * ex + ey * ey + ez * ez);
         }
     }
     gp_wave_sync();
@@ -224,8 +259,8 @@
     return cv.off;
 }
 
-extern "C" int gp_knn_lattice(const void *grid, const int32_t *coords, const int32_t *ids, int64_t nv, int32_t k,
-                              int32_t *nbr, void *workspace, size_t workspace_bytes, void *stream_) {
+static int knn_lattice(bool read_once, const void *grid, const int32_t *coords, const int32_t *ids, int64_t nv, int32_t k,
+                       int32_t *nbr, void *workspace, size_t workspace_bytes, void *stream_) {
     GP_CHECK_ARG(grid && coords && nbr && workspace, "gp_knn_lattice: null argument");
     GP_CHECK_ARG(k >= 1 && k <= GP_KNN_MAX_K, "gp_knn_lattice: k=%d not in 1..%d", k, GP_KNN_MAX_K);
     GP_CHECK_ARG(nv > k, "gp_knn_lattice: need more than k voxels (nv=%lld, k=%d)", (long long)nv, k);
@@ -237,11 +272,25 @@
     hipStream_t s = gp_stream(stream_);
     zero2_kernel<<<1, 64, 0, s>>>(counts, counts + 1);
     constexpr int W1 = 4, W3 = 2;
-    knn_ring_kernel<1, W1><<<(int)((nv + W1 - 1) / W1), W1 * 64, 0, s>>>(grid, coords, ids, nv, k, nbr, nullptr, nullptr,
-                                                                      list_a, counts);
+    if (read_once && nv <= ((int64_t)1 << KNN_KEEP_ROW_BITS))
+        knn_ring_kernel<1, W1, true><<<(int)((nv + W1 - 1) / W1), W1 * 64, 0, s>>>(grid, coords, ids, nv, k, nbr, nullptr, nullptr,
+                                                                                list_a, counts);
+    else
+        knn_ring_kernel<1, W1><<<(int)((nv + W1 - 1) / W1), W1 * 64, 0, s>>>(grid, coords, ids, nv, k, nbr, nullptr, nullptr,
+                                                                          list_a, counts);
     knn_ring_kernel<3, W3><<<(int)((nv + W3 - 1) / W3), W3 * 64, 0, s>>>(grid, coords, ids, nv, k, nbr, list_a, counts,
                                                                       list_b, counts + 1);
     knn_exhaustive_kernel<<<1024, 256, 0, s>>>(coords, ids, nv, k, nbr, list_b, counts + 1);
     GP_CHECK_LAUNCH();
     return GP_OK;
 }
+
+extern "C" int gp_knn_lattice(const void *grid, const int32_t *coords, const int32_t *ids, int64_t nv, int32_t k,
+                              int32_t *nbr, void *workspace, size_t workspace_bytes, void *stream_) {
+    return knn_lattice(true, grid, coords, ids, nv, k, nbr, workspace, workspace_bytes, stream_);
+}
+
+extern "C" int gp_knn_lattice_two_pass(const void *grid, const int32_t *coords, const int32_t *ids, int64_t nv, int32_t k,
+                                       int32_t *nbr, void *workspace, size_t workspace_bytes, void *stream_) {
+    return knn_lattice(false, grid, coords, ids, nv, k, nbr, workspace, workspace_bytes, stream_);
+}
diff --git a/geopurify_amd/csrc/lift.hip b/geopurify_amd/csrc/lift.hip
--- a/geopurify_amd/csrc/lift.hip
+++ b/geopurify_amd/csrc/lift.hip
@@ -201,14 +201,28 @@
     pv_seg[s] = seg[i];
 }
 
+__global__ void seen_masks_kernel(const int64_t *__restrict__ start, int64_t n, uint8_t *__restrict__ seen, uint8_t *__restrict__ unseen) {
+    int64_t p = blockIdx.x * (int64_t)blockDim.x + threadIdx.x;
+    if (p >= n) return;
+    const bool has = start[p + 1] > start[p];
+    seen[p] = has ? 1 : 0;
+    unseen[p] = has ? 0 : 1;
+}
+
+template <bool FILL>
 __global__ void fuse_top3_kernel(const int64_t *__restrict__ start, const int32_t *__restrict__ pv_view,
                                  const int32_t *__restrict__ pv_seg, int64_t n, const float *__restrict__ fseg,
                                  const float *__restrict__ lseg, int Q, int d, int C, float *__restrict__ out,
-                                 int64_t ld_out, uint8_t *__restrict__ seen) {
+                                 int64_t ld_out, uint8_t *__restrict__ seen, const int64_t *__restrict__ nn) {
     int64_t p = (blockIdx.x * (int64_t)blockDim.x + threadIdx.x) >> 6;
     if (p >= n) return;
     int lane = gp_lane();
-    int64_t b = start[p], e = start[p + 1];
+    int64_t src = p;
+    if constexpr (FILL) {
+        const int64_t t = nn[p];
+        if (t >= 0 && t < n) src = t;
+    }
+    int64_t b = start[src], e = start[src + 1];
     int M = (int)(e - b);
     if (lane == 0 && seen) seen[p] = M > 0 ? 1 : 0;
     if (M == 0) {
@@ -489,8 +503,26 @@
                                   float *out, int64_t ld_out, uint8_t *seen, void *stream_) {
     GP_CHECK_ARG(pv_start && pv_view && pv_seg && f_seg && logit_seg && out && n > 0, "gp_fuse_views_top3: null/empty argument");
     GP_CHECK_ARG(d % 4 == 0 && ld_out % 4 == 0, "gp_fuse_views_top3: d and ld_out must be multiples of 4");
-    fuse_top3_kernel<<<(int)((n * 64 + 255) / 256), 256, 0, gp_stream(stream_)>>>(pv_start, pv_view, pv_seg, n, f_seg,
-                                                                                logit_seg, q, d, c, out, ld_out, seen);
-    GP_CHECK_LAUNCH();
-    return GP_OK;
-}
+    fuse_top3_kernel<false><<<(int)((n * 64 + 255) / 256), 256, 0, gp_stream(stream_)>>>(pv_start, pv_view, pv_seg, n, f_seg,
+                                                                                       logit_seg, q, d, c, out, ld_out, seen, nullptr);
+    GP_CHECK_LAUNCH();
+    return GP_OK;
+}
+
+extern "C" int gp_seen_masks(const int64_t *pv_start, int64_t n, uint8_t *seen, uint8_t *unseen, void *stream_) {
+    GP_CHECK_ARG(pv_start && seen && unseen && n > 0, "gp_seen_masks: null/empty argument");
+    seen_masks_kernel<<<(int)((n + 255) / 256), 256, 0, gp_stream(stream_)>>>(pv_start, n, seen, unseen);
+    GP_CHECK_LAUNCH();
+    return GP_OK;
+}
+
+extern "C" int gp_fuse_views_top3_fill(const int64_t *pv_start, const int32_t *pv_view, const int32_t *pv_seg, int64_t n,
+                                       const float *f_seg, const float *logit_seg, int32_t q, int32_t d, int32_t c,
+                                       const int64_t *nn, float *out, int64_t ld_out, void *stream_) {
+    GP_CHECK_ARG(pv_start && pv_view && pv_seg && f_seg && logit_seg && nn && out && n > 0, "gp_fuse_views_top3_fill: null/empty argument");
+    GP_CHECK_ARG(d % 4 == 0 && ld_out % 4 == 0, "gp_fuse_views_top3_fill: d and ld_out must be multiples of 4");
+    fuse_top3_kernel<true><<<(int)((n * 64 + 255) / 256), 256, 0, gp_stream(stream_)>>>(pv_start, pv_view, pv_seg, n, f_seg,
+                                                                                      logit_seg, q, d, c, out, ld_out, nullptr, nn);
+    GP_CHECK_LAUNCH();
+    return GP_OK;
+}
diff --git a/geopurify_amd/csrc/voxel_rows.hip b/geopurify_amd/csrc/voxel_rows.hip
--- /dev/null
+++ b/geopurify_amd/csrc/voxel_rows.hip
@@ -0,0 +1,109 @@
+#include "gp_common.h"
+#include "gp_gfx950.h"
+
+namespace {
+
+template <int NI>
+__global__ void voxel_rows_kernel(const float *__restrict__ f, int64_t ld_f, int d, const float *__restrict__ geo, int64_t ld_geo, int dg,
+                                  const int64_t *__restrict__ order, const int64_t *__restrict__ seg, int64_t nv,
+                                  const int32_t *__restrict__ row_map, float *__restrict__ x, int64_t ld_x, int cin_pad,
+                                  _Float16 *__restrict__ rows, int64_t ld_rows, float *__restrict__ row_inv, unsigned *__restrict__ amax_bits) {
+    __shared__ float s_m[4];
+    const int lane = gp_lane();
+    float gmax = 0.f;
+    for (int64_t v_ = (blockIdx.x * (int64_t)blockDim.x + threadIdx.x) >> 6; v_ < nv; v_ += ((int64_t)gridDim.x * blockDim.x) >> 6) {
+        const int64_t v = __builtin_amdgcn_readfirstlane((int)v_);
+        const int64_t b = seg[v], e = seg[v + 1];
+        const int64_t orow = row_map ? row_map[v] : v;
+        const float den = (float)(e - b < 1 ? 1 : e - b);
+        float acc[NI][4];
+#pragma unroll
+        for (int i = 0; i < NI; ++i)
+#pragma unroll
+            for (int k = 0; k < 4; ++k) acc[i][k] = 0.f;
+        for (int64_t j = b; j < e; ++j) {
+            const int64_t r = order[j];
+#pragma unroll
+            for (int i = 0; i < NI; ++i) {
+                const int c = lane * 4 + 256 * i;
+                if (c < d) {
+                    const float4 t = *reinterpret_cast<const float4 *>(f + r * ld_f + c);
+                    acc[i][0] += t.x; acc[i][1] += t.y; acc[i][2] += t.z; acc[i][3] += t.w;
+                } else if (c < d + dg) {
+#pragma unroll
+                    for (int k = 0; k < 4; ++k)
+                        if (c + k < d + dg) acc[i][k] += geo[r * ld_geo + (c + k - d)];
+                }
+            }
+        }
+        float rmax = 0.f;
+#pragma unroll
+        for (int i = 0; i < NI; ++i) {
+            const int c = lane * 4 + 256 * i;
+            if (c < cin_pad) {
+#pragma unroll
+                for (int k = 0; k < 4; ++k) acc[i][k] = acc[i][k] / den;
+                *reinterpret_cast<float4 *>(x + orow * ld_x + c) = make_float4(acc[i][0], acc[i][1], acc[i][2], acc[i][3]);
+                const float m = fmaxf(fmaxf(fabsf(acc[i][0]), fabsf(acc[i][1])), fmaxf(fabsf(acc[i][2]), fabsf(acc[i][3])));
+                rmax = fmaxf(rmax, m);
+                if (c < d) gmax = fmaxf(gmax, m);
+            }
+        }
+        const float s = gp_pow2_for(gp_wave_max(rmax));
+        if (lane == 0) row_inv[orow] = 1.f / s;
+#pragma unroll
+        for (int i = 0; i < NI; ++i) {
+            const int c = lane * 4 + 256 * i;
+            if (c < cin_pad) {
+                const float sv[4] = {acc[i][0] * s, acc[i][1] * s, acc[i][2] * s, acc[i][3] * s};
+                f16x4 h, l;
+                gp_split_f16<4>(sv, h, l);
+                _Float16 *ph = rows + orow * ld_rows + ((c >> 5) << 6) + (c & 31);
+                *reinterpret_cast<f16x4 *>(ph) = h;
+                *reinterpret_cast<f16x4 *>(ph + 32) = l;
+            }
+        }
+    }
+    if (amax_bits) {
+        gmax = gp_wave_max(gmax);
+        if (lane == 0) s_m[threadIdx.x >> 6] = gmax;
+        __syncthreads();
+        if (threadIdx.x == 0) atomicMax(amax_bits, __float_as_uint(fmaxf(fmaxf(s_m[0], s_m[1]), fmaxf(s_m[2], s_m[3]))));
+    }
+}
+
+__global__ void voxel_rows_scale_kernel(const unsigned *__restrict__ amax_bits, float *__restrict__ out2) {
+    const float s = gp_pow2_for(__uint_as_float(amax_bits[0]));
+    out2[0] = s;
+    out2[1] = 1.f / s;
+}
+
+}
+
+extern "C" int gp_voxel_rows_operands(const float *f, int64_t ld_f, int32_t d, const float *geo, int64_t ld_geo, int32_t dg,
+                                      const int64_t *order, const int64_t *seg_start, int64_t nv, const int32_t *row_map, float *x,
+                                      int64_t ld_x, int32_t cin_pad, void *rows, int64_t ld_rows, float *row_inv_scale, float *scale2,
+                                      void *workspace, size_t workspace_bytes, void *stream_) {
+    GP_CHECK_ARG(f && geo && order && seg_start && x && rows && row_inv_scale && nv > 0, "gp_voxel_rows_operands: null/empty argument");
+    GP_CHECK_ARG(d > 0 && d % 4 == 0 && dg > 0 && cin_pad >= d + dg && cin_pad % 32 == 0 && cin_pad <= 1024,
+                 "gp_voxel_rows_operands: d %% 4 == 0, cin_pad %% 32 == 0, d + dg <= cin_pad <= 1024");
+    GP_CHECK_ARG(ld_f >= d && ld_f % 4 == 0 && ld_geo >= dg && ld_x >= cin_pad && ld_x % 4 == 0 && ld_rows >= 2 * (int64_t)cin_pad && ld_rows % 4 == 0,
+                 "gp_voxel_rows_operands: ld_f and ld_x multiples of 4 that hold a row, ld_rows %% 4 == 0 and >= 2 cin_pad");
+    GP_CHECK_ARG((uintptr_t)f % 16 == 0 && (uintptr_t)x % 16 == 0 && (uintptr_t)rows % 8 == 0, "gp_voxel_rows_operands: f and x 16-byte, rows 8-byte aligned");
+    GP_CHECK_ARG(!scale2 || (workspace && workspace_bytes >= 4), "gp_voxel_rows_operands: scale2 needs a workspace of 4 bytes");
+    hipStream_t s = gp_stream(stream_);
+    unsigned *amax = scale2 ? static_cast<unsigned *>(workspace) : nullptr;
+    if (amax) GP_CHECK_HIP(hipMemsetAsync(amax, 0, 4, s));
+    const int64_t waves = nv < 16384 ? nv : 16384;
+    const unsigned blocks = (unsigned)((waves * 64 + 255) / 256);
+    _Float16 *r16 = static_cast<_Float16 *>(rows);
+    switch ((cin_pad + 255) / 256) {
+    case 1: voxel_rows_kernel<1><<<blocks, 256, 0, s>>>(f, ld_f, d, geo, ld_geo, dg, order, seg_start, nv, row_map, x, ld_x, cin_pad, r16, ld_rows, row_inv_scale, amax); break;
+    case 2: voxel_rows_kernel<2><<<blocks, 256, 0, s>>>(f, ld_f, d, geo, ld_geo, dg, order, seg_start, nv, row_map, x, ld_x, cin_pad, r16, ld_rows, row_inv_scale, amax); break;
+    case 3: voxel_rows_kernel<3><<<blocks, 256, 0, s>>>(f, ld_f, d, geo, ld_geo, dg, order, seg_start, nv, row_map, x, ld_x, cin_pad, r16, ld_rows, row_inv_scale, amax); break;
+    default: voxel_rows_kernel<4><<<blocks, 256, 0, s>>>(f, ld_f, d, geo, ld_geo, dg, order, seg_start, nv, row_map, x, ld_x, cin_pad, r16, ld_rows, row_inv_scale, amax); break;
+    }
+    if (scale2) voxel_rows_scale_kernel<<<1, 1, 0, s>>>(amax, scale2);
+    GP_CHECK_LAUNCH();
+    return GP_OK;
+}
diff --git a/geopurify_amd/ops.py b/geopurify_amd/ops.py
--- a/geopurify_amd/ops.py
+++ b/geopurify_amd/ops.py
@@ -244,6 +244,22 @@
                                   _ptr(row_map), _ptr(out), out.stride(0), int(col0), _stream()),
           "gp_scatter_mean_csr")
     return out
+
+
+def voxel_rows_operands(f, d, geo, dg, order, seg_start, nv, cin_pad, row_map=None, want_scale=True):
+    lib = _lib.load()
+    _chk(f, torch.float32, "f")
+    _chk(geo, torch.float32, "geo")
+    dev = f.device
+    X = torch.empty((nv, cin_pad), dtype=torch.float32, device=dev)
+    rows = torch.empty((nv, 2 * cin_pad), dtype=torch.float16, device=dev)
+    rinv = torch.empty(nv, dtype=torch.float32, device=dev)
+    sc = torch.empty(2, dtype=torch.float32, device=dev) if want_scale else None
+    ws = _ws(256, dev) if want_scale else None
+    check(lib.gp_voxel_rows_operands(_ptr(f), f.stride(0), int(d), _ptr(geo), geo.stride(0), int(dg), _ptr(order), _ptr(seg_start), int(nv),
+                                     _ptr(row_map), _ptr(X), X.stride(0), int(cin_pad), _ptr(rows), rows.stride(0), _ptr(rinv), _ptr(sc),
+                                     _ptr(ws), ws.numel() if ws is not None else 0, _stream()), "gp_voxel_rows_operands")
+    return X, (rows, None, rinv), sc
 
 
 def gather_rows(src, d, index, out=None, row_map=None):
@@ -525,14 +541,14 @@
     return (out, (eh, el)) if planes else out
 
 
-def knn_lattice(grid, coords_sorted, ids, k):
+def knn_lattice(grid, coords_sorted, ids, k, two_pass=False):
     lib = _lib.load()
     nv = coords_sorted.shape[0]
     dev = coords_sorted.device
     ws = _ws(lib.gp_knn_workspace_bytes(nv), dev)
     nbr = torch.empty((nv, k), dtype=torch.int32, device=dev)
-    check(lib.gp_knn_lattice(_ptr(grid.buf), _ptr(coords_sorted), _ptr(ids), nv, int(k), _ptr(nbr), _ptr(ws),
-                             ws.numel(), _stream()), "gp_knn_lattice")
+    fn, name = (lib.gp_knn_lattice_two_pass, "gp_knn_lattice_two_pass") if two_pass else (lib.gp_knn_lattice, "gp_knn_lattice")
+    check(fn(_ptr(grid.buf), _ptr(coords_sorted), _ptr(ids), nv, int(k), _ptr(nbr), _ptr(ws), ws.numel(), _stream()), name)
     return nbr
 
 
@@ -990,6 +1006,25 @@
     check(lib.gp_fuse_views_top3(_ptr(pv_start), _ptr(pv_view), _ptr(pv_seg), int(n), _ptr(f_seg), _ptr(logit_seg),
                                  Q, d, C, _ptr(out), out.stride(0), _ptr(seen), _stream()), "gp_fuse_views_top3")
     return seen
+
+
+def seen_masks(pv_start, n):
+    lib = _lib.load()
+    _chk(pv_start, torch.int64, "pv_start")
+    seen = torch.empty(n, dtype=torch.uint8, device=pv_start.device)
+    unseen = torch.empty(n, dtype=torch.uint8, device=pv_start.device)
+    check(lib.gp_seen_masks(_ptr(pv_start), int(n), _ptr(seen), _ptr(unseen), _stream()), "gp_seen_masks")
+    return seen, unseen
+
+
+def fuse_views_top3_fill(pv_start, pv_view, pv_seg, n, f_seg, logit_seg, nn, out):
+    lib = _lib.load()
+    V, Q, d = f_seg.shape
+    C = logit_seg.shape[2]
+    _chk(nn, torch.int64, "nn")
+    check(lib.gp_fuse_views_top3_fill(_ptr(pv_start), _ptr(pv_view), _ptr(pv_seg), int(n), _ptr(f_seg), _ptr(logit_seg),
+                                      Q, d, C, _ptr(nn), _ptr(out), out.stride(0), _stream()), "gp_fuse_views_top3_fill")
+    return out
 
 
 def nn1(ref_xyz, query_xyz):
diff --git a/geopurify_amd/pipeline.py b/geopurify_amd/pipeline.py
--- a/geopurify_amd/pipeline.py
+++ b/geopurify_amd/pipeline.py
@@ -94,6 +94,11 @@
         if not self.fast:
             return None
         return ops.split_f16(x, self.cin_pad, per_row=True, interleaved=self.residual_from_planes and self.interleaved_rows)
+
+    def one_pass_input(self, F, geo):
+        return (self.fast and self.residual_from_planes and self.interleaved_rows and self.cin_pad <= 1024 and F.shape[1] % 4 == 0
+                and F.dtype == torch.float32 and F.is_contiguous() and F.data_ptr() % 16 == 0
+                and geo.dtype == torch.float32 and geo.is_contiguous() and geo.shape[1] == self.cin - F.shape[1])
 
     def forward(self, x, nbr_map, pairs=None, x_split=None, mark=None, planes=False, plane_rows=None, raw=False):
         if raw and planes:
@@ -444,10 +449,9 @@
         dev = self.device
         N = batch.scene_coords.shape[0]
         F = torch.empty((N, D), dtype=torch.float32, device=dev)
-        seen = ops.fuse_views_top3(start, pvv, pvs, N, f_seg, l_seg, F)
-        nn = ops.nn1_masked(batch.scene_coords, seen, 1 - seen)
-        src = torch.where(nn >= 0, nn, torch.arange(N, device=dev))
-        F = ops.gather_rows(F, D, src)
+        seen, unseen = ops.seen_masks(start, N)
+        nn = ops.nn1_masked(batch.scene_coords, seen, unseen)
+        ops.fuse_views_top3_fill(start, pvv, pvs, N, f_seg, l_seg, nn, F)
         return F, text, logit_scale
 
     def lift_dense(self, batch: SceneBatch, vlm: DenseFeatureVLM):
@@ -493,10 +497,16 @@
             segc = torch.zeros(Nv + 1, dtype=torch.int64, device=dev)
             segc[1:] = torch.bincount(batch.scene_inds_reconstruct, minlength=Nv).cumsum(0)
             batch.order, batch.seg_start = order, segc
-        X = torch.zeros((Nv, st.cin_pad), dtype=torch.float32, device=dev)
-        ops.scatter_mean_csr(F, D, batch.order, batch.seg_start, Nv, X, col0=0, row_map=rank)
-        ops.scatter_mean_csr(batch.scene_gauss_features, GEO_DIM, batch.order, batch.seg_start, Nv, X, col0=D,
-                             row_map=rank)
+        family = self._pool_family(D)
+        xs = sc = None
+        if st.one_pass_input(F, batch.scene_gauss_features):
+            X, xs, sc = ops.voxel_rows_operands(F, D, batch.scene_gauss_features, GEO_DIM, batch.order, batch.seg_start, Nv, st.cin_pad,
+                                                row_map=rank, want_scale=family in ("cs", "chain"))
+        else:
+            X = torch.zeros((Nv, st.cin_pad), dtype=torch.float32, device=dev)
+            ops.scatter_mean_csr(F, D, batch.order, batch.seg_start, Nv, X, col0=0, row_map=rank)
+            ops.scatter_mean_csr(batch.scene_gauss_features, GEO_DIM, batch.order, batch.seg_start, Nv, X, col0=D,
+                                 row_map=rank)
         mark("scatter_mean")
         if batch.extent is not None:
             grid = ops.grid_build(cs, [0, 0, 0], batch.extent)
@@ -508,10 +518,10 @@
         nbr = ops.knn_lattice(grid, cs, perm, self.K)
         mark("kNN")
         state = {"X": X, "rank": rank, "nbr_map": nbr_map, "pairs": pairs, "nbr": nbr, "Nv": Nv, "D": D, "pool": None,
-                 "xs": st.split_input(X)}
-        family = self._pool_family(D)
+                 "xs": xs if xs is not None else st.split_input(X)}
         if family in ("cs", "chain"):
-            sc = ops.pow2_scale(X, D)
+            if sc is None:
+                sc = ops.pow2_scale(X, D)
             how = self.pool_structure_ahead
             if how and self.affinity_mfma and self.K <= 96 and self.student is not None and self.student.embed == 128:
                 how = "valid"
diff --git a/include/geopurify_hip.h b/include/geopurify_hip.h
--- a/include/geopurify_hip.h
+++ b/include/geopurify_hip.h
@@ -85,6 +85,10 @@
                   size_t workspace_bytes, void *stream);
 int gp_split_f16_scaled(const float *x, int64_t ld_x, int32_t d, int64_t n, void *hi, void *lo, int64_t ld_h,
                         const float *scale, float *row_inv_scale, const int32_t *dst_row, void *stream);
+int gp_voxel_rows_operands(const float *f, int64_t ld_f, int32_t d, const float *geo, int64_t ld_geo, int32_t dg,
+                           const int64_t *order, const int64_t *seg_start, int64_t nv, const int32_t *row_map, float *x,
+                           int64_t ld_x, int32_t cin_pad, void *rows, int64_t ld_rows, float *row_inv_scale, float *scale2,
+                           void *workspace, size_t workspace_bytes, void *stream);
 int gp_sparse_conv_f16x3(const float *x, int64_t ld_x, const void *x_hi, const void *x_lo, int64_t ld_xh,
                          const int32_t *pair_in, const int32_t *pair_pos,
                          const int32_t *seg_off, const int32_t *tile_start, const int32_t *tile_desc,
@@ -112,6 +116,8 @@
 size_t gp_knn_workspace_bytes(int64_t nv);
 int gp_knn_lattice(const void *grid, const int32_t *coords, const int32_t *ids, int64_t nv,
                    int32_t k, int32_t *nbr, void *workspace, size_t workspace_bytes, void *stream);
+int gp_knn_lattice_two_pass(const void *grid, const int32_t *coords, const int32_t *ids, int64_t nv,
+                            int32_t k, int32_t *nbr, void *workspace, size_t workspace_bytes, void *stream);
 size_t gp_knn_batched_workspace_bytes(int64_t nv);
 int gp_knn_batched(const uint64_t *keys_sorted, const int32_t *ids, int64_t nv, int32_t k, int32_t *nbr, int32_t *status,
                    void *workspace, size_t workspace_bytes, void *stream);
@@ -224,6 +230,10 @@
 int gp_fuse_views_top3(const int64_t *pv_start, const int32_t *pv_view, const int32_t *pv_seg,
                        int64_t n, const float *f_seg, const float *logit_seg, int32_t q, int32_t d,
                        int32_t c, float *out, int64_t ld_out, uint8_t *seen, void *stream);
+int gp_seen_masks(const int64_t *pv_start, int64_t n, uint8_t *seen, uint8_t *unseen, void *stream);
+int gp_fuse_views_top3_fill(const int64_t *pv_start, const int32_t *pv_view, const int32_t *pv_seg,
+                            int64_t n, const float *f_seg, const float *logit_seg, int32_t q, int32_t d,
+                            int32_t c, const int64_t *nn, float *out, int64_t ld_out, void *stream);
 size_t gp_nn1_workspace_bytes(int64_t n_ref, int64_t n_query);
 int gp_nn1_f64(const float *ref_xyz, int64_t n_ref, const float *query_xyz, int64_t n_query,
                int64_t *nn, void *workspace, size_t workspace_bytes, void *stream);
```

Measured after the change: 47.42 (median of 6 runs). 1.01x the previous value.
